# jvasilakes/disentanglement-vae

Measured on NVIDIA B200. Metric: train_tokens_per_sec, higher is better.
Workload: dtype f32

## Files before the change

disentanglement-vae_b200/_lib.py:

```python
import ctypes as C
import os

_HERE = os.path.dirname(os.path.abspath(__file__))
LIB_PATH = os.path.join(_HERE, "libdvae_b200.so")

MAX_SPACES = 8
HEADS_NSCALARS = 3 + 3 * MAX_SPACES


class DvaeError(RuntimeError):
    pass


_p = C.c_void_p
_i = C.c_int
_l = C.c_int64
_f = C.c_float
_u32 = C.c_uint32
_pp = C.POINTER(C.c_void_p)
_ip = C.POINTER(C.c_int)

SIGNATURES = {
    "dvae_last_error_string": (C.c_char_p, []),
    "dvae_version": (_i, []),
    "dvae_launch_count": (_l, []),
    "dvae_weight_planes_floats": (_l, [_i, _i, _i]),
    "dvae_weight_planes_register": (_i, [_p, _i, _i, _p, _p]),
    "dvae_weight_planes_refresh": (_i, [_p]),
    "dvae_weight_planes_refresh_ex": (_i, [_i, _i, _p]),
    "dvae_weight_planes_enable": (_i, [_i]),
    "dvae_weight_planes_clear": (_i, []),
    "dvae_defer_joins": (_i, [_i]),
    "dvae_join_side_streams": (_i, [_p]),
    "dvae_linear": (_i, [_p, _l, _i, _p, _l, _i, _p, _l, _i, _i, _i, _p, _p, _f, _i, _p]),
    "dvae_tc_linear": (_i, [_p, _l, _i, _p, _l, _i, _p, _l, _i, _i, _i, _p, _p, _f, _i, _i, _p]),
    "dvae_tc16_linear": (_i, [_p, _l, _i, _p, _l, _i, _p, _l, _i, _i, _i, _p, _p, _f, _i, _f, _f, _p, _p, _p]),
    "dvae_colsum": (_i, [_p, _l, _i, _i, _p, _f, _p]),
    "dvae_randn": (_i, [_p, _l, _p, _u32, _p]),
    "dvae_embedding_fwd": (_i, [_p, _i, _p, _l, _l, _i, _i, _f, _p, _u32, _l, _i, _p, _p]),
    "dvae_embedding_bwd": (_i, [_p, _i, _p, _l, _l, _i, _i, _f, _p, _u32, _l, _i, _p, _p]),
    "dvae_bow_encoder_fwd": (_i, [_p, _i, _p, _l, _l, _i, _i, _f, _p, _u32, _p, _l, _p, _p]),
    "dvae_bow_encoder_bwd": (_i, [_p, _l, _p, _i, _p, _l, _l, _i, _i, _f, _p, _u32, _p, _p]),
    "dvae_dropout": (_i, [_p, _l, _l, _i, _f, _p, _u32, _p, _l, _l, _p]),
    "dvae_lstm_step": (_i, [_p, _l, _i, _i, _i, _i, _i, _p, _p, _p, _p, _p, _p, _l, _p, _p, _p, _p, _p]),
    "dvae_vocab_sample_step": (_i, [_p, _l, _i, _i, _i, _p, _p, _p, _u32, _p, _l, _p, _p]),
    "dvae_vocab_sample_step_ex": (_i, [_p, _l, _i, _i, _i, _p, _p, _p, _u32, _p, _l, _p, _p, _p]),
    "dvae_vocab_w_planes_floats": (_l, [_i, _i]),
    "dvae_vocab_w_planes": (_i, [_p, _i, _i, _p, _p]),
    "dvae_vocab_sample_step_planes": (_i, [_p, _l, _i, _i, _i, _p, _p, _p, _p, _u32, _p, _l, _p, _p, _p]),
    "dvae_recount_lengths": (_i, [_p, _l, _l, _i, _i, _l, _l, _l, _p, _p]),
    "dvae_bleu_counts": (_i, [_p, _l, _i, _p, _l, _i, _i, _l, _p, _p]),
    "dvae_bleu_score": (_i, [_p, _p, _p]),
    "dvae_lstm_state_ws_floats": (_l, [_i, _i, _i]),
    "dvae_lstm_seq_fwd": (_i, [_p, _l, _i, _i, _i, _i, _i, _pp, _pp, _pp, _pp, _p, _p, _l, _l, _p, _p, _l, _p, _p,
                               _l, _l, _p, _p, _p, _p]),
    "dvae_lstm_input_proj": (_i, [_p, _l, _i, _i, _i, _i, _i, _pp, _pp, _pp, _p, _p]),
    "dvae_lstm_seq_fwd_ex": (_i, [_p, _l, _i, _i, _i, _i, _i, _pp, _pp, _pp, _pp, _p, _p, _l, _l, _p, _p, _l, _p, _p,
                                  _l, _l, _p, _p, _p, _i, _p]),
    "dvae_lstm_seq_bwd": (_i, [_p, _l, _i, _i, _i, _i, _i, _pp, _pp, _p, _p, _l, _l, _p, _p, _l, _p, _p, _p, _l,
                               _p, _p, _l, _l, _p, _l, _pp, _pp, _pp, _pp, _p, _p, _l, _l, _p, _p]),
    "dvae_lstm_bwd_planes_ws_floats": (_l, [_i, _i, _i, _i, _i]),
    "dvae_lstm_seq_bwd_ex": (_i, [_p, _l, _i, _i, _i, _i, _i, _pp, _pp, _p, _p, _l, _l, _p, _p, _l, _p, _p, _p, _l,
                                  _p, _p, _l, _l, _p, _l, _pp, _pp, _pp, _pp, _p, _p, _l, _l, _p, _p, _p]),
    "dvae_counter_increment": (_i, [_p, _p]),
    "dvae_fork_after": (_i, [_i, _p, _p, C.POINTER(C.c_void_p)]),
    "dvae_nvls_barrier_words": (_l, []),
    "dvae_nvls_all_reduce": (_i, [_p, _l, _pp, _i, _i, _p, C.c_uint32, C.c_uint32, _i, C.c_uint64, _p, _p]),
    "dvae_p2p_all_reduce": (_i, [_pp, _l, _pp, _i, _i, _p, C.c_uint32, C.c_uint32, _i, C.c_uint64, _p, _p]),
    "dvae_flag_signal": (_i, [_p, _p, _i, _p, _p]),
    "dvae_flag_wait": (_i, [_p, _p, _p]),
    "dvae_flag_signal_value": (_i, [_p, C.c_uint32, _p]),
    "dvae_flag_wait_value": (_i, [_p, C.c_uint32, _p]),
    "dvae_heads_ws_floats": (_l, [_i, _i]),
    "dvae_latent_heads_fwd": (_i, [_p, _i, _i, _i, _ip, _ip, _p, _p, _p, _p, _p, _p, _p, _p, _p, _i, _p, _p, _p,
                                   _p, _p, _p, _p, _p]),
    "dvae_heads_bwd_ws_floats": (_l, [_i, _i, _i]),
    "dvae_latent_heads_bwd": (_i, [_p, _i, _i, _i, _ip, _ip, _p, _p, _p, _p, _p, _p, _i, _p, _p, _p, _p, _p, _p,
                                   _p, _p, _p, _p, _p, _p, _p, _p, _p, _p, _p, _p, _p]),
    "dvae_dsc_loss": (_i, [_p, _p, _i, _i, _ip, _ip, _p, _p, _p, _p]),
    "dvae_vocab_ce_ws_floats": (_l, [_i, _i, _i]),
    "dvae_vocab_ce_fwd": (_i, [_p, _l, _i, _i, _i, _i, _p, _p, _p, _l, _p, _i, _p, _p, _p, _p, _p, _p]),
    "dvae_vocab_split_w": (_i, [_p, _i, _i, _i, _p, _p]),
    "dvae_vocab_ce_fwd_ex": (_i, [_p, _l, _i, _i, _i, _i, _p, _p, _p, _l, _p, _i, _p, _p, _p, _p, _p, _i, _p]),
    "dvae_vocab_ce_partials": (_i, [_p, _l, _i, _i, _i, _i, _p, _p, _p, _l, _p, _i, _p, _p]),
    "dvae_vocab_ce_bwd_ws_floats": (_l, [_i, _i, _i]),
    "dvae_vocab_ce_bwd": (_i, [_p, _l, _i, _i, _i, _i, _p, _p, _p, _l, _p, _p, _p, _p, _l, _p, _p, _p, _p, _p]),
    "dvae_entropy_loss": (_i, [_p, _i, _i, _p, _p, _p, _p]),
    "dvae_club_mi": (_i, [_p, _p, _p, _i, _i, _p, _p, _p, _p, _p, _p, _p]),
    "dvae_club_nll": (_i, [_p, _p, _p, _i, _i, _p, _p, _p, _p, _p]),
    "dvae_act_bwd": (_i, [_p, _p, _p, _l, _i, _p]),
    "dvae_relu": (_i, [_p, _l, _p]),
    "dvae_grad_sumsq": (_i, [_p, _l, _p, _p, _p]),
    "dvae_clip_adam": (_i, [_p, _p, _p, _p, _l, _p, _f, _f, _p, _i, _p]),
}

_lib = None
planes_owner = None


def load():
    global _lib
    if _lib is not None:
        return _lib
    if not os.path.exists(LIB_PATH):
        raise DvaeError(
            f"{LIB_PATH} not found: build it with `python -c 'import __graft_entry__ as g; g.build()'` "
            "(nvcc, sm_100a).  There is no CPU or PyTorch fallback for this path.")
    lib = C.CDLL(LIB_PATH)
    for name, (res, args) in SIGNATURES.items():
        try:
            fn = getattr(lib, name)
        except AttributeError as e:
            raise DvaeError(f"{LIB_PATH} does not export {name}") from e
        fn.restype = res
        fn.argtypes = args
    _lib = lib
    return lib


def check(rc, what):
    if rc != 0:
        msg = load().dvae_last_error_string()
        raise DvaeError(f"{what} failed ({rc}): {msg.decode() if msg else ''}")


def ptr(t):
    return None if t is None else t.data_ptr()


def ptr_array(tensors):
    arr = (C.c_void_p * max(len(tensors), 1))()
    for i, t in enumerate(tensors):
        arr[i] = None if t is None else t.data_ptr()
    return arr


def int_array(vals):
    arr = (C.c_int * max(len(vals), 1))()
    for i, v in enumerate(vals):
        arr[i] = int(v)
    return arr


def stream_ptr():
    import torch
    return torch.cuda.current_stream().cuda_stream


def launch_count():
    return int(load().dvae_launch_count())
```

disentanglement-vae_b200/csrc/common.cuh:

```cuda
#pragma once
#include <cuda_runtime.h>
#include <stdint.h>
#include <stdio.h>

#include "../../include/dvae_b200.h"

namespace dvae {

void set_error(const char* fmt, ...);
void count_launch(int n = 1);

#define DVAE_REQUIRE(cond, ...)            \
  do {                                     \
    if (!(cond)) {                         \
      ::dvae::set_error(__VA_ARGS__);      \
      return DVAE_EINVAL;                  \
    }                                      \
  } while (0)

#define DVAE_CUDA(call)                                                                  \
  do {                                                                                   \
    cudaError_t e__ = (call);                                                            \
    if (e__ != cudaSuccess) {                                                            \
      ::dvae::set_error("%s failed at %s:%d: %s", #call, __FILE__, __LINE__,             \
                        cudaGetErrorString(e__));                                        \
      return DVAE_ECUDA;                                                                 \
    }                                                                                    \
  } while (0)

#define DVAE_LAUNCH_CHECK()                                                              \
  do {                                                                                   \
    ::dvae::count_launch();                                                              \
    cudaError_t e__ = cudaGetLastError();                                                \
    if (e__ != cudaSuccess) {                                                            \
      ::dvae::set_error("kernel launch failed at %s:%d: %s", __FILE__, __LINE__,         \
                        cudaGetErrorString(e__));                                        \
      return DVAE_ECUDA;                                                                 \
    }                                                                                    \
  } while (0)

static inline int ceil_div(int64_t a, int64_t b) { return (int)((a + b - 1) / b); }

class Fork {
 public:
  explicit Fork(cudaStream_t main);
  cudaStream_t side(int i);
  int join();
  int join_or_defer();
  int mark(int i);
  int wait_mark();
  int chain(int from, int to);
 private:
  cudaStream_t main_;
  bool used_[3] = {false, false, false};
  bool marked_ = false;
  bool ok_;
};

bool defer_joins_enabled();

bool force_simt_gemm();

struct GemmHints {
  const uint32_t* a_amax_bits = nullptr;
  const uint32_t* b_amax_bits = nullptr;
  int a_amax_n = 1, b_amax_n = 1;
  float a_scale = 1.f, b_scale = 1.f;
  bool a_wide = false, b_wide = false;
  const void* b_planes = nullptr;
  int b_tile0 = 0, b_kb0 = 0, b_kbtot = 0;
  int max_ctas = 0;
  bool atomic_out = false;
  bool c_zeroed = false;
  int concurrency = 1;
};
int linear_impl_ex(const float* A, int64_t lda, int trans_a, const float* B, int64_t ldb, int trans_b, float* C,
                   int64_t ldc, int M, int N, int K, const float* bias, const float* bias2, float beta, int act,
                   const GemmHints& hints, cudaStream_t st);

namespace tc {
bool tc_linear_supported(const float* A, int64_t lda, const float* B, int64_t ldb, int M, int N, int K);
int tc_linear_impl(const float* A, int64_t lda, int trans_a, const float* B, int64_t ldb, int trans_b, float* C, int64_t ldc,
                   int M, int N, int K, const float* bias, const float* bias2, float beta, int act, int passes,
                   cudaStream_t st);
int tc_ce_partials(const float* h, int64_t ldh, int N, int B, int H, int V, const float* w, const float* bias,
                   const int64_t* targets, int64_t tgt_stride_b, const int64_t* lengths, int tiles_per_split, int nsplit,
                   float* part, int* part_idx, const uint64_t* gumbel_seed, uint32_t gumbel_salt, cudaStream_t st);
int tc_softmax_grad(const float* h, int64_t ldh, int N, int B, int H, int v0, int vc, const float* w, const float* bias,
                    const int64_t* targets, int64_t tgt_stride_b, const int64_t* lengths, const float* lse,
                    const float* grad_scale, float* P, int64_t ldp, cudaStream_t st);
}

struct Philox {
  static constexpr uint32_t kM0 = 0xD2511F53u, kM1 = 0xCD9E8D57u, kW0 = 0x9E3779B9u, kW1 = 0xBB67AE85u;
  __host__ __device__ static inline void round(uint32_t (&c)[4], uint32_t k0, uint32_t k1) {
#ifdef __CUDA_ARCH__
    uint32_t hi0 = __umulhi(kM0, c[0]), hi1 = __umulhi(kM1, c[2]);
#else
    uint32_t hi0 = (uint32_t)(((uint64_t)kM0 * c[0]) >> 32), hi1 = (uint32_t)(((uint64_t)kM1 * c[2]) >> 32);
#endif
    uint32_t lo0 = kM0 * c[0], lo1 = kM1 * c[2];
    uint32_t n0 = hi1 ^ c[1] ^ k0, n1 = lo1, n2 = hi0 ^ c[3] ^ k1, n3 = lo0;
    c[0] = n0; c[1] = n1; c[2] = n2; c[3] = n3;
  }
  __host__ __device__ static inline void gen(uint64_t seed, uint32_t salt, uint64_t ctr, uint32_t (&out)[4]) {
    uint32_t c[4] = {(uint32_t)ctr, (uint32_t)(ctr >> 32), salt, 0x5eedu};
    uint32_t k0 = (uint32_t)seed, k1 = (uint32_t)(seed >> 32);
#pragma unroll
    for (int i = 0; i < 10; ++i) {
      round(c, k0, k1);
      k0 += kW0;
      k1 += kW1;
    }
    out[0] = c[0]; out[1] = c[1]; out[2] = c[2]; out[3] = c[3];
  }
};

__device__ __forceinline__ void dropout_scale4(uint64_t seed, uint32_t salt, uint64_t idx4, float p,
                                               float inv_keep, float (&s)[4]) {
  uint32_t r[4];
  Philox::gen(seed, salt, idx4, r);
#pragma unroll
  for (int i = 0; i < 4; ++i) s[i] = ((float)r[i] * 2.3283064365386963e-10f >= p) ? inv_keep : 0.f;
}

__device__ __forceinline__ void gumbel4(uint64_t seed, uint32_t salt, int row, int col, int ncol4, float (&g)[4]) {
  uint32_t r[4];
  Philox::gen(seed, salt, (uint64_t)row * ncol4 + (col >> 2), r);
#pragma unroll
  for (int i = 0; i < 4; ++i) {
    const float u = ((float)(r[i] >> 8) + 0.5f) * (1.f / 16777216.f);
    g[i] = -logf(-logf(u));
  }
}

__device__ __forceinline__ float warp_sum(float v) {
#pragma unroll
  for (int o = 16; o > 0; o >>= 1) v += __shfl_xor_sync(0xffffffffu, v, o);
  return v;
}

__device__ __forceinline__ float sigmoidf_(float x) { return 1.f / (1.f + expf(-x)); }

}
```

disentanglement-vae_b200/csrc/embed_optim.cu:

```cuda
#include "common.cuh"

namespace dvae {

constexpr int kSMs = 148;

__global__ void embedding_fwd_kernel(const float* __restrict__ emb, int E, const int64_t* __restrict__ tokens,
                                     int64_t sb, int64_t st_, int T, int B, float p, const uint64_t* seed_dev,
                                     uint32_t salt, int64_t first_token, int t0, float* __restrict__ x) {
  const int64_t total4 = (int64_t)T * B * ((E + 3) / 4);
  const uint64_t seed = (p > 0.f && seed_dev) ? *seed_dev : 0;
  const float inv_keep = p > 0.f ? 1.f / (1.f - p) : 1.f;
  const int e4n = (E + 3) / 4;
  for (int64_t i = (int64_t)blockIdx.x * blockDim.x + threadIdx.x; i < total4; i += (int64_t)gridDim.x * blockDim.x) {
    const int64_t row = i / e4n + (int64_t)t0 * B;
    const int e0 = (int)(i % e4n) * 4;
    const int t = (int)(row / B), b = (int)(row % B);
    const int64_t tok = (t == 0 && first_token >= 0) ? first_token : tokens[b * sb + t * st_];
    const float* src = emb + tok * E + e0;
    float s[4] = {1.f, 1.f, 1.f, 1.f};
    if (p > 0.f && seed_dev) dropout_scale4(seed, salt, (uint64_t)(row * e4n + e0 / 4), p, inv_keep, s);
    float* dst = x + row * E + e0;
#pragma unroll
    for (int j = 0; j < 4; ++j)
      if (e0 + j < E) dst[j] = src[j] * s[j];
// ... 30 lines not shown
                                   float* __restrict__ ctx, int64_t ldctx, int32_t* __restrict__ argmax) {
  const int e4n = (E + 3) / 4;
  const int64_t total = (int64_t)B * e4n;
  const uint64_t seed = (p > 0.f && seed_dev) ? *seed_dev : 0;
  const float inv_keep = p > 0.f ? 1.f / (1.f - p) : 1.f;
  for (int64_t i = (int64_t)blockIdx.x * blockDim.x + threadIdx.x; i < total; i += (int64_t)gridDim.x * blockDim.x) {
    const int b = (int)(i / e4n), e0 = (int)(i % e4n) * 4;
    float best[4] = {-INFINITY, -INFINITY, -INFINITY, -INFINITY};
    int arg[4] = {0, 0, 0, 0};
    for (int t = 0; t < T; ++t) {
      const int64_t tok = tokens[b * sb + t * st_];
      float s[4] = {1.f, 1.f, 1.f, 1.f};
      if (p > 0.f && seed_dev) dropout_scale4(seed, salt, (uint64_t)(((int64_t)t * B + b) * e4n + e0 / 4), p, inv_keep, s);
#pragma unroll
      for (int j = 0; j < 4; ++j)
        if (e0 + j < E) {
          const float v = emb[tok * E + e0 + j] * s[j];
          if (v > best[j]) { best[j] = v; arg[j] = t; }
        }
    }
#pragma unroll
    for (int j = 0; j < 4; ++j)
      if (e0 + j < E) {
        ctx[(int64_t)b * ldctx + e0 + j] = best[j];
        argmax[(int64_t)b * E + e0 + j] = arg[j];
      }
  }
}

__global__ void bow_max_bwd_kernel(const float* __restrict__ d_ctx, int64_t ldd, const int32_t* __restrict__ argmax, int E,
                                   const int64_t* __restrict__ tokens, int64_t sb, int64_t st_, int T, int B, float p,
                                   const uint64_t* seed_dev, uint32_t salt, float* __restrict__ d_emb) {
  const int e4n = (E + 3) / 4;
  const int64_t total = (int64_t)B * E;
  const uint64_t seed = (p > 0.f && seed_dev) ? *seed_dev : 0;
  const float inv_keep = p > 0.f ? 1.f / (1.f - p) : 1.f;
  for (int64_t i = (int64_t)blockIdx.x * blockDim.x + threadIdx.x; i < total; i += (int64_t)gridDim.x * blockDim.x) {
    const int b = (int)(i / E), e = (int)(i % E);
    const int t = argmax[i];
    float s[4] = {1.f, 1.f, 1.f, 1.f};
    if (p > 0.f && seed_dev) dropout_scale4(seed, salt, (uint64_t)(((int64_t)t * B + b) * e4n + e / 4), p, inv_keep, s);
    const float v = d_ctx[(int64_t)b * ldd + e] * s[e & 3];
    if (v != 0.f) atomicAdd(d_emb + tokens[b * sb + t * st_] * E + e, v);
  }
}

__global__ void dropout_kernel(const float* __restrict__ x, int64_t ldx, int64_t rows, int width, float p,
                               const uint64_t* seed_dev, uint32_t salt, float* __restrict__ y, int64_t ldy, int64_t row0) {
  const int w4n = (width + 3) / 4;
  const int64_t total4 = rows * w4n;
  const uint64_t seed = (p > 0.f && seed_dev) ? *seed_dev : 0;
  const float inv_keep = p > 0.f ? 1.f / (1.f - p) : 1.f;
  for (int64_t i = (int64_t)blockIdx.x * blockDim.x + threadIdx.x; i < total4; i += (int64_t)gridDim.x * blockDim.x) {
    const int64_t row = i / w4n + row0;
    const int c0 = (int)(i % w4n) * 4;
    float s[4] = {1.f, 1.f, 1.f, 1.f};
    if (p > 0.f && seed_dev) dropout_scale4(seed, salt, (uint64_t)(row * w4n + c0 / 4), p, inv_keep, s);
#pragma unroll
    for (int j = 0; j < 4; ++j)
      if (c0 + j < width) y[row * ldy + c0 + j] = x[row * ldx + c0 + j] * s[j];
  }
}

__global__ void randn_kernel(float* __restrict__ out, int64_t n, const uint64_t* seed_dev, uint32_t salt) {
  const uint64_t seed = *seed_dev;
  const int64_t n4 = (n + 3) / 4;
  for (int64_t i = (int64_t)blockIdx.x * blockDim.x + threadIdx.x; i < n4; i += (int64_t)gridDim.x * blockDim.x) {
    uint32_t r[4];
    Philox::gen(seed, salt, (uint64_t)i, r);
    float u0 = ((float)r[0] + 1.f) * 2.3283064365386963e-10f, u1 = (float)r[1] * 2.3283064365386963e-10f;
    float u2 = ((float)r[2] + 1.f) * 2.3283064365386963e-10f, u3 = (float)r[3] * 2.3283064365386963e-10f;
    float a = sqrtf(-2.f * logf(u0)), b = sqrtf(-2.f * logf(u2));
    float s0, c0, s1, c1;
    sincospif(2.f * u1, &s0, &c0);
    sincospif(2.f * u3, &s1, &c1);
    float v[4] = {a * c0, a * s0, b * c1, b * s1};
#pragma unroll
    for (int j = 0; j < 4; ++j)
      if (i * 4 + j < n) out[i * 4 + j] = v[j];
  }
}

constexpr int kRedBlocks = 1024;

__global__ void __launch_bounds__(256) sumsq_kernel(const float* __restrict__ g, int64_t n, float* __restrict__ sumsq,
                                                    float* __restrict__ ws) {
  __shared__ float red[8];
  __shared__ int is_last;
  float acc = 0.f;
  const int64_t n4 = n / 4;
  const float4* g4 = reinterpret_cast<const float4*>(g);
  for (int64_t i = (int64_t)blockIdx.x * blockDim.x + threadIdx.x; i < n4; i += (int64_t)gridDim.x * blockDim.x) {
    float4 v = g4[i];
    acc = fmaf(v.x, v.x, acc); acc = fmaf(v.y, v.y, acc); acc = fmaf(v.z, v.z, acc); acc = fmaf(v.w, v.w, acc);
  }
  if (blockIdx.x == 0)
    for (int64_t i = n4 * 4 + threadIdx.x; i < n; i += blockDim.x) acc = fmaf(g[i], g[i], acc);
  acc = warp_sum(acc);
  if ((threadIdx.x & 31) == 0) red[threadIdx.x >> 5] = acc;
  __syncthreads();
  if (threadIdx.x == 0) {
    float t = 0.f;
    for (int i = 0; i < 8; ++i) t += red[i];
    ws[blockIdx.x] = t;
    __threadfence();
    unsigned int* counter = reinterpret_cast<unsigned int*>(ws + kRedBlocks);
    is_last = atomicAdd(counter, 1u) == gridDim.x - 1;
  }
  __syncthreads();
  if (is_last) {
    __threadfence();
    double t = 0.0;
    for (int i = threadIdx.x; i < (int)gridDim.x; i += blockDim.x) t += (double)((volatile float*)ws)[i];
    __shared__ double dred[256];
    dred[threadIdx.x] = t;
    __syncthreads();
    for (int o = 128; o > 0; o >>= 1) {
      if ((int)threadIdx.x < o) dred[threadIdx.x] += dred[threadIdx.x + o];
      __syncthreads();
    }
    if (threadIdx.x == 0) {
      sumsq[0] = (float)dred[0];
      *reinterpret_cast<unsigned int*>(ws + kRedBlocks) = 0u;
    }
  }
}

__global__ void __launch_bounds__(256) clip_adam_kernel(float* __restrict__ p, float* __restrict__ g,
                                                        float* __restrict__ m, float* __restrict__ v, int64_t n,
                                                        const float* __restrict__ sumsq, float max_norm,
                                                        float grad_scale, const float* __restrict__ hyper,
                                                        int zero_grad) {
  const float lr = hyper[0], b1 = hyper[1], b2 = hyper[2], eps = hyper[3], step = hyper[4];
  float coef = grad_scale;
  if (sumsq) {
    const float norm = sqrtf(sumsq[0]) * fabsf(grad_scale);
    coef *= fminf(1.f, max_norm / (norm + 1e-6f));
  }
  const float bc1 = 1.f - powf(b1, step), bc2 = 1.f - powf(b2, step);
  const float step_size = lr / bc1, inv_bc2_sqrt = 1.f / sqrtf(bc2);
  auto update = [&](float& pi, float& gi_io, float& mi_io, float& vi_io) {
    const float gi = gi_io * coef;
    const float mi = fmaf(b1, mi_io, (1.f - b1) * gi);
    const float vi = fmaf(b2, vi_io, (1.f - b2) * gi * gi);
    mi_io = mi; vi_io = vi;
    pi -= step_size * mi / (sqrtf(vi) * inv_bc2_sqrt + eps);
    gi_io = zero_grad ? 0.f : gi;
  };
  const bool vec = (((uintptr_t)p | (uintptr_t)g | (uintptr_t)m | (uintptr_t)v) & 15) == 0;
  const int64_t n4 = vec ? n / 4 : 0;
  float4* p4 = reinterpret_cast<float4*>(p); float4* g4 = reinterpret_cast<float4*>(g);
  float4* m4 = reinterpret_cast<float4*>(m); float4* v4 = reinterpret_cast<float4*>(v);
  const int64_t stride = (int64_t)gridDim.x * blockDim.x;
  for (int64_t i = (int64_t)blockIdx.x * blockDim.x + threadIdx.x; i < n4; i += 2 * stride) {
    const int64_t j = i + stride;
    const bool two = j < n4;
    float4 pa = p4[i], ga = g4[i], ma = m4[i], va = v4[i];
    float4 pb, gb, mb, vb;
    if (two) { pb = p4[j]; gb = g4[j]; mb = m4[j]; vb = v4[j]; }
    update(pa.x, ga.x, ma.x, va.x); update(pa.y, ga.y, ma.y, va.y); update(pa.z, ga.z, ma.z, va.z); update(pa.w, ga.w, ma.w, va.w);
    p4[i] = pa; g4[i] = ga; m4[i] = ma; v4[i] = va;
    if (two) {
      update(pb.x, gb.x, mb.x, vb.x); update(pb.y, gb.y, mb.y, vb.y); update(pb.z, gb.z, mb.z, vb.z); update(pb.w, gb.w, mb.w, vb.w);
      p4[j] = pb; g4[j] = gb; m4[j] = mb; v4[j] = vb;
    }
  }
  for (int64_t i = n4 * 4 + (int64_t)blockIdx.x * blockDim.x + threadIdx.x; i < n; i += stride) update(p[i], g[i], m[i], v[i]);
}

}

using namespace dvae;

static int ew_grid(int64_t work) {
  int64_t blocks = (work + 255) / 256;
  int64_t cap = (int64_t)kSMs * 8;
  return (int)(blocks < 1 ? 1 : (blocks > cap ? cap : blocks));
}

extern "C" int dvae_embedding_fwd(const float* emb, int E, const int64_t* tokens, int64_t sb, int64_t st_, int T,
                                  int B, float p, const uint64_t* seed_dev, uint32_t salt, int64_t first_token, int t0, float* x, void* stream) {
  DVAE_REQUIRE(emb && tokens && x && E > 0 && T > 0 && B > 0 && p >= 0.f && p < 1.f, "dvae_embedding_fwd: bad argument");
  embedding_fwd_kernel<<<ew_grid((int64_t)T * B * ((E + 3) / 4)), 256, 0, (cudaStream_t)stream>>>(emb, E, tokens, sb, st_, T, B, p, seed_dev, salt, first_token, t0, x);
  DVAE_LAUNCH_CHECK();
  return DVAE_OK;
}

extern "C" int dvae_embedding_bwd(const float* d_x, int E, const int64_t* tokens, int64_t sb, int64_t st_, int T,
                                  int B, float p, const uint64_t* seed_dev, uint32_t salt, int64_t first_token, int t0, float* d_emb, void* stream) {
  DVAE_REQUIRE(d_x && tokens && d_emb && E > 0 && T > 0 && B > 0 && p >= 0.f && p < 1.f, "dvae_embedding_bwd: bad argument");
  embedding_bwd_kernel<<<ew_grid((int64_t)T * B * ((E + 3) / 4)), 256, 0, (cudaStream_t)stream>>>(d_x, E, tokens, sb, st_, T, B, p, seed_dev, salt, first_token, t0, d_emb);
  DVAE_LAUNCH_CHECK();
  return DVAE_OK;
}

extern "C" int dvae_bow_encoder_fwd(const float* emb, int E, const int64_t* tokens, int64_t sb, int64_t st_, int T, int B, float p,
                                    const uint64_t* seed_dev, uint32_t salt, float* ctx, int64_t ldctx, int32_t* argmax, void* stream) {
  DVAE_REQUIRE(emb && tokens && ctx && argmax && E > 0 && T > 0 && B > 0 && p >= 0.f && p < 1.f, "dvae_bow_encoder_fwd: bad argument");
  bow_max_fwd_kernel<<<ew_grid((int64_t)B * ((E + 3) / 4)), 256, 0, (cudaStream_t)stream>>>(emb, E, tokens, sb, st_, T, B, p, seed_dev, salt, ctx, ldctx, argmax);
  DVAE_LAUNCH_CHECK();
  return DVAE_OK;
}

extern "C" int dvae_bow_encoder_bwd(const float* d_ctx, int64_t ldd, const int32_t* argmax, int E, const int64_t* tokens, int64_t sb,
                                    int64_t st_, int T, int B, float p, const uint64_t* seed_dev, uint32_t salt, float* d_emb, void* stream) {
  DVAE_REQUIRE(d_ctx && argmax && tokens && d_emb && E > 0 && T > 0 && B > 0 && p >= 0.f && p < 1.f, "dvae_bow_encoder_bwd: bad argument");
  bow_max_bwd_kernel<<<ew_grid((int64_t)B * E), 256, 0, (cudaStream_t)stream>>>(d_ctx, ldd, argmax, E, tokens, sb, st_, T, B, p, seed_dev, salt, d_emb);
  DVAE_LAUNCH_CHECK();
  return DVAE_OK;
}

extern "C" int dvae_dropout(const float* x, int64_t ldx, int64_t rows, int width, float p, const uint64_t* seed_dev,
                            uint32_t salt, float* y, int64_t ldy, int64_t row0, void* stream) {
  DVAE_REQUIRE(x && y && rows > 0 && width > 0 && p >= 0.f && p < 1.f, "dvae_dropout: bad argument");
  dropout_kernel<<<ew_grid(rows * ((width + 3) / 4)), 256, 0, (cudaStream_t)stream>>>(x, ldx, rows, width, p, seed_dev, salt, y, ldy, row0);
  DVAE_LAUNCH_CHECK();
  return DVAE_OK;
}

extern "C" int dvae_randn(float* out, int64_t n, const uint64_t* seed_dev, uint32_t salt, void* stream) {
  DVAE_REQUIRE(out && seed_dev && n > 0, "dvae_randn: bad argument");
  randn_kernel<<<ew_grid((n + 3) / 4), 256, 0, (cudaStream_t)stream>>>(out, n, seed_dev, salt);
  DVAE_LAUNCH_CHECK();
  return DVAE_OK;
}

extern "C" int dvae_grad_sumsq(const float* g, int64_t n, float* sumsq, float* ws, void* stream) {
  DVAE_REQUIRE(g && sumsq && ws && n > 0, "dvae_grad_sumsq: bad argument");
  DVAE_REQUIRE((reinterpret_cast<uintptr_t>(g) & 15) == 0, "dvae_grad_sumsq: gradient buffer must be 16-byte aligned");
  int blocks = ew_grid(n / 4 + 1);
  if (blocks > kRedBlocks) blocks = kRedBlocks;
  sumsq_kernel<<<blocks, 256, 0, (cudaStream_t)stream>>>(g, n, sumsq, ws);
  DVAE_LAUNCH_CHECK();
  return DVAE_OK;
}

extern "C" int dvae_clip_adam(float* p, float* g, float* m, float* v, int64_t n, const float* sumsq, float max_norm,
                              float grad_scale, const float* hyper_dev, int zero_grad, void* stream) {
  DVAE_REQUIRE(p && g && m && v && hyper_dev && n > 0, "dvae_clip_adam: bad argument");
  clip_adam_kernel<<<ew_grid((n + 7) / 8), 256, 0, (cudaStream_t)stream>>>(p, g, m, v, n, sumsq, max_norm, grad_scale, hyper_dev, zero_grad);
  DVAE_LAUNCH_CHECK();
  return DVAE_OK;
}

namespace dvae {
__global__ void recount_lengths_kernel(const int64_t* __restrict__ tokens, int64_t sb, int64_t st_, int B, int T, int64_t eos,
                                       int64_t pad, int64_t min_len, int64_t* __restrict__ lengths_out) {
  const int warp = (blockIdx.x * blockDim.x + threadIdx.x) >> 5, lane = threadIdx.x & 31;
  if (warp >= B) return;
  int n = 0;
  for (int t = lane; t < T; t += 32) {
    const int64_t tok = tokens[warp * sb + t * st_];
    n += (tok == eos || tok == pad) ? 1 : 0;
  }
#pragma unroll
  for (int o = 16; o > 0; o >>= 1) n += __shfl_xor_sync(0xffffffffu, n, o);
  if (lane == 0) {
    const int64_t len = (int64_t)T - n;
    lengths_out[warp] = len < min_len ? min_len : len;
  }
}
}

extern "C" int dvae_recount_lengths(const int64_t* tokens, int64_t tok_stride_b, int64_t tok_stride_t, int B, int T,
                                    int64_t eos, int64_t pad, int64_t min_len, int64_t* lengths_out, void* stream) {
  DVAE_REQUIRE(tokens && lengths_out && B > 0 && T > 0, "dvae_recount_lengths: bad argument");
  const int threads = 128, blocks = dvae::ceil_div((int64_t)B * 32, threads);
  dvae::recount_lengths_kernel<<<blocks, threads, 0, (cudaStream_t)stream>>>(tokens, tok_stride_b, tok_stride_t, B, T, eos, pad,
                                                                            min_len, lengths_out);
  DVAE_LAUNCH_CHECK();
  return DVAE_OK;
}
```

disentanglement-vae_b200/csrc/linear.cu:

```cuda
#include "gemm_simt.cuh"
#include "tc_gemm16.cuh"

namespace dvae {

template <class G>
__global__ void __launch_bounds__(G::NT) linear_kernel(const float* __restrict__ A, int64_t lda,
                                                        const float* __restrict__ B, int64_t ldb,
                                                        float* __restrict__ C, int64_t ldc, int M, int N, int K,
                                                        const float* __restrict__ bias,
                                                        const float* __restrict__ bias2, float beta, int act,
                                                        int k_per_split) {
  __shared__ __align__(16) float smem[G::SMEM_FLOATS];
  const int m0 = blockIdx.y * G::BM, n0 = blockIdx.x * G::BN;
  const int kb = blockIdx.z * k_per_split, ke = min(K, kb + k_per_split);
  float acc[G::TM][G::TN];
#pragma unroll
  for (int i = 0; i < G::TM; ++i)
#pragma unroll
    for (int j = 0; j < G::TN; ++j) acc[i][j] = 0.f;
  G::run(A, lda, m0, M, B, ldb, n0, N, kb, ke, K, smem, acc);
  const int ty = threadIdx.x / G::TX, tx = threadIdx.x % G::TX;
  const bool split = gridDim.z > 1;
#pragma unroll
  for (int i = 0; i < G::TM; ++i) {
    int m = m0 + G::row_of(ty, i);
    if (m >= M) continue;
#pragma unroll
    for (int j = 0; j < G::TN; ++j) {
      int n = n0 + G::col_of(tx, j);
      if (n >= N) continue;
      float v = acc[i][j];
      float* c = C + (int64_t)m * ldc + n;
      if (split) {
        if (blockIdx.z == 0) {
          if (bias) v += bias[n];
          if (bias2) v += bias2[n];
        }
        atomicAdd(c, v);
      } else {
        if (bias) v += bias[n];
        if (bias2) v += bias2[n];
        if (act == 1) v = tanhf(v);
        if (beta != 0.f) v += beta * (*c);
        *c = v;
      }
    }
  }
}

using GBig_NT = GemmTile<128, 128, 16, 8, 8, true, true>;
using GBig_NN = GemmTile<128, 128, 16, 8, 8, true, false>;
using GBig_TN = GemmTile<128, 128, 16, 8, 8, false, false>;
using GBig_TT = GemmTile<128, 128, 16, 8, 8, false, true>;
using GSm_NT = GemmTile<64, 64, 16, 4, 4, true, true>;
using GSm_NN = GemmTile<64, 64, 16, 4, 4, true, false>;
using GSm_TN = GemmTile<64, 64, 16, 4, 4, false, false>;
using GSm_TT = GemmTile<64, 64, 16, 4, 4, false, true>;

template <class G>
static int launch_linear(const float* A, int64_t lda, const float* B, int64_t ldb, float* C, int64_t ldc, int M,
                         int N, int K, const float* bias, const float* bias2, float beta, int act, int splits,
                         cudaStream_t st) {
  int k_per_split = ceil_div(ceil_div(K, splits), G::BK) * G::BK;
  splits = ceil_div(K, k_per_split);
  dim3 grid(ceil_div(N, G::BN), ceil_div(M, G::BM), splits);
  linear_kernel<G><<<grid, G::NT, 0, st>>>(A, lda, B, ldb, C, ldc, M, N, K, bias, bias2, beta, act, k_per_split);
  DVAE_LAUNCH_CHECK();
  return DVAE_OK;
}

__global__ void scale_rows_kernel(float* C, int64_t ldc, int M, int N, float beta) {
  int64_t i = (int64_t)blockIdx.x * blockDim.x + threadIdx.x;
  if (i >= (int64_t)M * N) return;
  float* c = C + (i / N) * ldc + (i % N);
  *c = beta == 0.f ? 0.f : *c * beta;
}

int linear_impl(const float* A, int64_t lda, int trans_a, const float* B, int64_t ldb, int trans_b, float* C,
                int64_t ldc, int M, int N, int K, const float* bias, const float* bias2, float beta, int act,
                cudaStream_t st) {
  return linear_impl_ex(A, lda, trans_a, B, ldb, trans_b, C, ldc, M, N, K, bias, bias2, beta, act, GemmHints(), st);
}

int linear_impl_ex(const float* A, int64_t lda, int trans_a, const float* B, int64_t ldb, int trans_b, float* C,
                   int64_t ldc, int M, int N, int K, const float* bias, const float* bias2, float beta, int act,
                   const GemmHints& hints, cudaStream_t st) {
  DVAE_REQUIRE(A && B && C, "dvae_linear: null pointer");
  DVAE_REQUIRE(M > 0 && N > 0 && K > 0, "dvae_linear: non-positive size M=%d N=%d K=%d", M, N, K);
  DVAE_REQUIRE(act == 0 || act == 1, "dvae_linear: unknown activation %d", act);
  static const double tc_min_mnk = [] {
    const char* e = getenv("DVAE_TC_MIN_LOG2_MNK");
    return (double)(1ll << (e ? atoi(e) : 24));
  }();
  if (!force_simt_gemm() && M >= 64 && N >= 64 && K >= 32 && (double)M * N * K >= tc_min_mnk) {
    const bool unscaled_wide = (hints.a_wide && !hints.a_amax_bits) || (hints.b_wide && !hints.b_amax_bits);
    if (!unscaled_wide && tc16::supported(A, lda, trans_a, B, ldb, trans_b, M, N, K))
      return tc16::linear(A, lda, trans_a, B, ldb, trans_b, C, ldc, M, N, K, bias, bias2, beta, act, hints, st);
    if (tc::tc_linear_supported(A, lda, B, ldb, M, N, K))
      return tc::tc_linear_impl(A, lda, trans_a, B, ldb, trans_b, C, ldc, M, N, K, bias, bias2, beta, act, 3, st);
  }
  const int kSMs = 148;
  int64_t big_tiles = (int64_t)ceil_div(M, 128) * ceil_div(N, 128);
  int64_t small_tiles = (int64_t)ceil_div(M, 64) * ceil_div(N, 64);
  bool big = big_tiles >= kSMs;
  int splits = 1;
  if (!big && small_tiles < kSMs / 2 && K >= 512 && act == 0) {
    { int64_t want = (kSMs + small_tiles - 1) / small_tiles, cap = K / 128; splits = (int)(want < cap ? want : cap); }
    if (splits < 1) splits = 1;
  }
  if (splits > 1) {
    if (beta != 1.f) {
      int64_t n = (int64_t)M * N;
      scale_rows_kernel<<<ceil_div(n, 256), 256, 0, st>>>(C, ldc, M, N, beta);
      DVAE_LAUNCH_CHECK();
    }
  }
#define DVAE_DISPATCH(GB, GS)                                                                                    \
  return big ? launch_linear<GB>(A, lda, B, ldb, C, ldc, M, N, K, bias, bias2, beta, act, 1, st)                 \
             : launch_linear<GS>(A, lda, B, ldb, C, ldc, M, N, K, bias, bias2, beta, act, splits, st)
  if (!trans_a && !trans_b) { DVAE_DISPATCH(GBig_NT, GSm_NT); }
  if (!trans_a && trans_b) { DVAE_DISPATCH(GBig_NN, GSm_NN); }
  if (trans_a && trans_b) { DVAE_DISPATCH(GBig_TN, GSm_TN); }
  DVAE_DISPATCH(GBig_TT, GSm_TT);
#undef DVAE_DISPATCH
}

__global__ void colsum_kernel(const float* __restrict__ X, int64_t ldx, int M, int N, float* __restrict__ out,
                              int rows_per_block) {
  __shared__ float red[8][33];
  const int n = blockIdx.x * 32 + threadIdx.x;
  const int m0 = blockIdx.y * rows_per_block, m1 = min(M, m0 + rows_per_block);
  float s0 = 0.f, s1 = 0.f;
  if (n < N) {
    int m = m0 + threadIdx.y;
    for (; m + 8 < m1; m += 16) { s0 += X[(int64_t)m * ldx + n]; s1 += X[(int64_t)(m + 8) * ldx + n]; }
    if (m < m1) s0 += X[(int64_t)m * ldx + n];
  }
  red[threadIdx.y][threadIdx.x] = s0 + s1;
  __syncthreads();
  if (threadIdx.y == 0 && n < N) {
    float t = 0.f;
#pragma unroll
    for (int i = 0; i < 8; ++i) t += red[i][threadIdx.x];
    atomicAdd(out + n, t);
  }
}

__global__ void scale_vec_kernel(float* out, int N, float beta) {
  int i = blockIdx.x * blockDim.x + threadIdx.x;
  if (i < N) out[i] *= beta;
}

int colsum_impl(const float* X, int64_t ldx, int M, int N, float* out, float beta, cudaStream_t st) {
  DVAE_REQUIRE(X && out && M > 0 && N > 0, "dvae_colsum: bad argument");
  if (beta == 0.f) {
    DVAE_CUDA(cudaMemsetAsync(out, 0, sizeof(float) * N, st));
  } else if (beta != 1.f) {
    scale_vec_kernel<<<ceil_div(N, 256), 256, 0, st>>>(out, N, beta);
    DVAE_LAUNCH_CHECK();
  }
  const int col_blocks = ceil_div(N, 32);
  int row_blocks = ceil_div(2 * 148, col_blocks);
  if (row_blocks > ceil_div(M, 64)) row_blocks = ceil_div(M, 64);
  if (row_blocks < 1) row_blocks = 1;
  const int rows_per_block = ceil_div(M, row_blocks);
  colsum_kernel<<<dim3(col_blocks, ceil_div(M, rows_per_block)), dim3(32, 8), 0, st>>>(X, ldx, M, N, out, rows_per_block);
  DVAE_LAUNCH_CHECK();
  return DVAE_OK;
}

}

extern "C" int dvae_linear(const float* A, int64_t lda, int trans_a, const float* B, int64_t ldb, int trans_b,
                           float* C, int64_t ldc, int M, int N, int K, const float* bias, const float* bias2,
                           float beta, int act, void* stream) {
  dvae::GemmHints hints;
  hints.a_wide = hints.b_wide = true;
  return dvae::linear_impl_ex(A, lda, trans_a, B, ldb, trans_b, C, ldc, M, N, K, bias, bias2, beta, act, hints,
                           (cudaStream_t)stream);
// ... 6 lines not shown
```

disentanglement-vae_b200/csrc/lstm.cu:

```cuda
#include <stdlib.h>

#include <cstring>

#include "common.cuh"
#include "lstm_persist.cuh"
#include "tc_gemm16.cuh"

namespace dvae {

int linear_impl(const float* A, int64_t lda, int trans_a, const float* B, int64_t ldb, int trans_b, float* C,
                int64_t ldc, int M, int N, int K, const float* bias, const float* bias2, float beta, int act,
                cudaStream_t st);
int colsum_impl(const float* X, int64_t ldx, int M, int N, float* out, float beta, cudaStream_t st);

__global__ void copy_state_kernel(const float* __restrict__ src, int64_t lds, int64_t dirs, float* __restrict__ dst,
                                  int64_t ldd, int64_t dird, int D, int B, int H) {
  int64_t i = (int64_t)blockIdx.x * blockDim.x + threadIdx.x;
  if (i >= (int64_t)D * B * H) return;
  int u = i % H, b = (i / H) % B, d = i / ((int64_t)H * B);
  dst[d * dird + b * ldd + u] = src ? src[d * dirs + b * lds + u] : 0.f;
}

__global__ void transpose_kernel(const float* __restrict__ in, float* __restrict__ out, int R, int C) {
  __shared__ float tile[32][33];
// ... 211 lines not shown
int lstm_input_proj_impl(const float* x, int64_t ldx, int T, int B, int I, int H, int D, const float* const* w_ih,
                         const float* const* b_ih, const float* const* b_hh, float* gates, cudaStream_t st) {
  DVAE_REQUIRE(x && gates && w_ih, "dvae_lstm_input_proj: null pointer");
  DVAE_REQUIRE(T > 0 && B > 0 && I > 0 && H > 0 && (D == 1 || D == 2), "dvae_lstm_input_proj: bad shape T=%d B=%d I=%d H=%d D=%d", T, B, I, H, D);
  const int64_t slab = (int64_t)T * B * 4 * H;
  Fork fork(st);
  GemmHints gh;
  gh.concurrency = D;
  for (int d = 0; d < D; ++d) {
    int rc = linear_impl_ex(x, ldx, 0, w_ih[d], I, 0, gates + d * slab, 4 * H, T * B, 4 * H, I, b_ih ? b_ih[d] : nullptr,
                            b_hh ? b_hh[d] : nullptr, 0.f, 0, gh, d == 0 ? st : fork.side(0));
    if (rc) return rc;
  }
  return fork.join();
}

int lstm_seq_fwd_impl(const float* x, int64_t ldx, int T, int B, int I, int H, int D, const float* const* w_ih,
                      const float* const* w_hh, const float* const* b_ih, const float* const* b_hh,
                      const float* h0, const float* c0, int64_t ld0, int64_t dir0, const int64_t* lengths,
                      float* hs, int64_t ldhs, float* hn, float* cn, int64_t ldn, int64_t dirn, float* gates,
                      float* cs, float* ws, bool gates_ready, cudaStream_t st) {
  DVAE_REQUIRE(x && hs && gates && cs && ws && w_ih && w_hh, "dvae_lstm_seq_fwd: null pointer");
  DVAE_REQUIRE(T > 0 && B > 0 && I > 0 && H > 0 && (D == 1 || D == 2), "dvae_lstm_seq_fwd: bad shape T=%d B=%d I=%d H=%d D=%d", T, B, I, H, D);
  DVAE_REQUIRE(!(lengths && h0), "dvae_lstm_seq_fwd: length-masked layers start from the zero state");
  const int64_t sf = (int64_t)D * B * H;
  if (!gates_ready) {
    int rc = lstm_input_proj_impl(x, ldx, T, B, I, H, D, w_ih, b_ih, b_hh, gates, st);
    if (rc) return rc;
  }
  {
    const void* ptrs[] = {x, w_hh[0], w_hh[D - 1], h0, c0, hs, hn, cn, gates, cs, ws};
    const int64_t lds[] = {ld0, dir0, ldhs, ldn, dirn};
    if (!force_step_path() && persist_supported(B, H, D, ptrs, 11, lds, 5)) {
      PersistFwdArgs a;
      a.w_hh[0] = w_hh[0]; a.w_hh[1] = w_hh[D - 1];
      a.gates = gates; a.cs = cs; a.hs = hs; a.ldhs = ldhs; a.h0 = h0; a.c0 = c0; a.ld0 = ld0; a.dir0 = dir0;
      a.hstate = ws; a.hn = hn; a.cn = cn; a.ldn = ldn; a.dirn = dirn; a.lengths = lengths;
      a.T = T; a.B = B; a.D = D; a.n_slices = ceil_div(B, 16); a.d_off = 0;
      a.dbg = nullptr;
      if (const char* e = getenv("DVAE_LSTM_DBG")) a.dbg = reinterpret_cast<unsigned long long*>(strtoull(e, nullptr, 0));
      return persist_fwd(H, a, st);
    }
    if (!force_step_path() && planes_lstm_supported(B, H, D, ptrs, 11, lds, 5) && resident_lstm_supported(B, H))
      return resident_lstm_fwd(T, B, H, D, w_hh, h0, c0, ld0, dir0, lengths, hs, ldhs, hn, cn, ldn, dirn, gates, cs,
                               ws + planes_ws_offset(B, H, D), st);
    if (!force_step_path() && planes_lstm_supported(B, H, D, ptrs, 11, lds, 5))
      return planes_lstm_fwd(T, B, H, D, w_hh, h0, c0, ld0, dir0, lengths, hs, ldhs, hn, cn, ldn, dirn, gates, cs, ws,
                             ws + planes_ws_offset(B, H, D), st);
  }
  float* hbuf[2] = {ws, ws + 2 * sf};
  float* cbuf[2] = {ws + sf, ws + 3 * sf};
  const int nthr = 256, nblk = ceil_div(sf, nthr);
  copy_state_kernel<<<nblk, nthr, 0, st>>>(h0, ld0, dir0, hbuf[0], H, (int64_t)B * H, D, B, H);
  DVAE_LAUNCH_CHECK();
  copy_state_kernel<<<nblk, nthr, 0, st>>>(c0, ld0, dir0, cbuf[0], H, (int64_t)B * H, D, B, H);
  DVAE_LAUNCH_CHECK();
  FwdStepArgs a;
  for (int d = 0; d < 2; ++d) a.w_hh[d] = w_hh[d < D ? d : 0];
  a.gates = gates; a.cs = cs; a.hs = hs; a.ldhs = ldhs; a.lengths = lengths; a.T = T; a.B = B; a.H = H;
  dim3 grid(ceil_div(H, 16), ceil_div(B, kStepRows), D);
  for (int s = 0; s < T; ++s) {
    a.s = s;
    a.h_in = hbuf[s & 1]; a.c_in = cbuf[s & 1]; a.h_out = hbuf[(s + 1) & 1]; a.c_out = cbuf[(s + 1) & 1];
    lstm_step_fwd_kernel<<<grid, kStepThreads, 0, st>>>(a);
    DVAE_LAUNCH_CHECK();
  }
  if (hn) {
    copy_state_kernel<<<nblk, nthr, 0, st>>>(hbuf[T & 1], H, (int64_t)B * H, hn, ldn, dirn, D, B, H);
    DVAE_LAUNCH_CHECK();
  }
  if (cn) {
    copy_state_kernel<<<nblk, nthr, 0, st>>>(cbuf[T & 1], H, (int64_t)B * H, cn, ldn, dirn, D, B, H);
    DVAE_LAUNCH_CHECK();
  }
  return DVAE_OK;
}

int lstm_seq_bwd_impl(const float* x, int64_t ldx, int T, int B, int I, int H, int D, const float* const* w_ih,
                      const float* const* w_hh, const float* h0, const float* c0, int64_t ld0, int64_t dir0,
                      const int64_t* lengths, const float* hs, int64_t ldhs, float* gates, const float* cs,
                      const float* d_hs, int64_t lddhs, const float* d_hn, const float* d_cn, int64_t ldn,
                      int64_t dirn, float* d_x, int64_t lddx, float* const* d_w_ih, float* const* d_w_hh,
                      float* const* d_b_ih, float* const* d_b_hh, float* d_h0, float* d_c0, int64_t ldd0,
                      int64_t dird0, float* ws, float* planes_ws, cudaStream_t st) {
  DVAE_REQUIRE(x && hs && gates && cs && ws && w_ih && w_hh, "dvae_lstm_seq_bwd: null pointer");
  DVAE_REQUIRE(T > 0 && B > 0 && I > 0 && H > 0 && (D == 1 || D == 2), "dvae_lstm_seq_bwd: bad shape");
  DVAE_REQUIRE(!(lengths && h0), "dvae_lstm_seq_bwd: length-masked layers start from the zero state");
  const int64_t slab = (int64_t)T * B * 4 * H, sf = (int64_t)D * B * H;
  bool persisted = false;
  uint32_t* amax = nullptr;
  int amax_n = 1;
  bool dx_zeroed = false;
  {
    const void* ptrs[] = {w_hh[0], w_hh[D - 1], c0, gates, cs, d_hs, d_hn, d_cn, d_h0, d_c0};
    const int64_t lds[] = {ld0, dir0, lddhs, ldn, dirn, ldd0, dird0};
    if (!force_step_path() && persist_supported(B, H, D, ptrs, 10, lds, 7)) {
      PersistBwdArgs a;
      a.w_hh[0] = w_hh[0]; a.w_hh[1] = w_hh[D - 1];
      a.gates = gates; a.cs = cs; a.c0 = c0; a.ld0 = ld0; a.dir0 = dir0; a.d_hs = d_hs; a.lddhs = lddhs;
      a.d_hn = d_hn; a.d_cn = d_cn; a.ldn = ldn; a.dirn = dirn; a.d_h0 = d_h0; a.d_c0 = d_c0; a.ldd0 = ldd0;
      a.dird0 = dird0; a.lengths = lengths; a.T = T; a.B = B; a.D = D; a.n_slices = ceil_div(B, 16); a.d_off = 0;
      a.amax_out = nullptr;
      a.zero_buf = nullptr; a.zero_n4 = 0;
      if (tc_lstm_supported(H)) {
        static thread_local unsigned slot = 0;
        amax = reinterpret_cast<uint32_t*>(ws + state_floats(B, H, D) + 4LL * D * H * H) + amax_slot_entries(B, D) * (slot++ & 7);
        a.amax_out = amax;
        amax_n = tc_lstm_bwd_ctas(B, D);
        if (d_x && lddx == I && (((uintptr_t)d_x) & 15) == 0 && ((int64_t)T * B * I) % 4 == 0 && d_x != d_hs) {
          a.zero_buf = d_x; a.zero_n4 = (int64_t)T * B * I / 4;
          dx_zeroed = true;
        }
      }
      int rc = persist_bwd(H, a, st);
      if (rc) return rc;
      persisted = true;
    } else {
      const void* ptrs2[] = {w_hh[0], w_hh[D - 1], c0, gates, cs, d_hs, d_hn, d_cn, d_h0, d_c0, ws};
      if (!force_step_path() && planes_lstm_supported(B, H, D, ptrs2, 11, lds, 7)) {
        static thread_local unsigned slot2 = 0;
        amax = reinterpret_cast<uint32_t*>(ws + state_floats(B, H, D) + 4LL * D * H * H) + amax_slot_entries(B, D) * (slot2++ & 7);
        amax_n = D;
        int rc = planes_lstm_bwd(T, B, H, D, w_hh, c0, ld0, dir0, lengths, gates, cs, d_hs, lddhs, d_hn, d_cn, ldn, dirn, d_h0,
                                 d_c0, ldd0, dird0, ws, ws + 4 * sf, ws + planes_ws_offset(B, H, D), amax, st);
        if (rc) return rc;
        persisted = true;
      }
    }
  }
  float* carry[2] = {ws, ws + 2 * sf};
  float* dcb[2] = {ws + sf, ws + 3 * sf};
  float* wt = ws + 4 * sf;
  for (int d = 0; d < D && !persisted; ++d) {
    transpose_kernel<<<dim3(ceil_div(H, 32), ceil_div(4 * H, 32)), dim3(32, 8), 0, st>>>(w_hh[d], wt + (int64_t)d * 4 * H * H, 4 * H, H);
    DVAE_LAUNCH_CHECK();
  }
  const int nthr = 256, nblk = ceil_div(sf, nthr);
  if (!persisted) {
    copy_state_kernel<<<nblk, nthr, 0, st>>>(d_hn, ldn, dirn, carry[0], H, (int64_t)B * H, D, B, H);
    DVAE_LAUNCH_CHECK();
    copy_state_kernel<<<nblk, nthr, 0, st>>>(d_cn, ldn, dirn, dcb[0], H, (int64_t)B * H, D, B, H);
    DVAE_LAUNCH_CHECK();
  }
  BwdStepArgs a;
  for (int d = 0; d < 2; ++d) a.w_hh_t[d] = wt + (int64_t)(d < D ? d : 0) * 4 * H * H;
  a.gates = gates; a.cs = cs; a.c0 = c0; a.ld0 = ld0; a.dir0 = dir0; a.d_hs = d_hs; a.lddhs = lddhs;
  a.d_h0 = d_h0; a.d_c0 = d_c0; a.ldd0 = ldd0; a.dird0 = dird0; a.lengths = lengths; a.T = T; a.B = B; a.H = H;
  dim3 grid(ceil_div(H, 32), ceil_div(B, kStepRows), D);
  const int nsteps = persisted ? 0 : T + ((d_h0 || d_c0) ? 1 : 0);
  for (int s = 0; s < nsteps; ++s) {
    a.s = s; a.final_ = (s == T);
    a.carry_in = carry[s & 1]; a.dc_in = dcb[s & 1]; a.carry_out = carry[(s + 1) & 1]; a.dc_out = dcb[(s + 1) & 1];
    if (a.final_) {
    }
    lstm_step_bwd_kernel<<<grid, kStepThreads, 0, st>>>(a);
    DVAE_LAUNCH_CHECK();
  }
  GemmHints gh;
  gh.a_wide = true;
  gh.a_amax_bits = amax;
  gh.a_amax_n = amax_n;
  GemmHints gh_bg = gh;
  {
    static const int cap = [] { const char* e = getenv("DVAE_DW_MAX_CTAS"); return e ? atoi(e) : 48; }();
    gh_bg.max_ctas = (defer_joins_enabled() && tc_lstm_supported(H)) ? cap : 0;
  }
  Fork fork(st);
  const bool dx_pair = d_x && D == 2 && dx_zeroed && !force_simt_gemm() && tc_lstm_supported(H) &&
                       !(getenv("DVAE_DX_PAIR") && getenv("DVAE_DX_PAIR")[0] == '0');
  if (dx_pair) {
    GemmHints ghx = gh;
    ghx.c_zeroed = true; ghx.atomic_out = true; ghx.concurrency = 2;
    int rc = linear_impl_ex(gates + slab, 4 * H, 0, w_ih[1], I, 1, d_x, lddx, T * B, I, 4 * H, nullptr, nullptr, 1.f, 0, ghx, fork.side(2));
    if (rc) return rc;
    if ((rc = fork.mark(2))) return rc;
  }
  const int TB = T * B, KBt = ceil_div(TB, 32);
  const char* dwp_env = getenv("DVAE_DW_PLANES");
  const bool dwp_on = dwp_env ? dwp_env[0] != '0' : (int64_t)4 * H * (I > H ? I : H) * TB >= ((int64_t)1 << 32);
  const bool dw_planes = planes_ws && amax && !force_simt_gemm() && tc16::enabled() && TB >= 128 &&
                         (reinterpret_cast<uintptr_t>(planes_ws) & 15) == 0 && dwp_on;
  const bool hh_planes = dw_planes && T > 1 && B % 32 == 0;
  float *xT = planes_ws, *dGt[2] = {nullptr, nullptr}, *hsT[2] = {nullptr, nullptr};
  if (dw_planes) {
    float* q = xT + tc16::plane_floats(I, TB);
    for (int d = 0; d < D; ++d) { dGt[d] = q; q += tc16::plane_floats(4 * H, TB); }
    for (int d = 0; d < D; ++d) { hsT[d] = q; q += tc16::plane_floats(H, TB); }
    tc16::PlaneTable tab;
    tab.n = 0;
    if (d_w_ih) tab.e[tab.n++] = tc16::PlaneTable::Entry{x, TB, I, nullptr, xT, ldx, nullptr, 0};
    for (int d = 0; d < D; ++d) {
      tab.e[tab.n++] = tc16::PlaneTable::Entry{gates + d * slab, TB, 4 * H, nullptr, dGt[d], 4 * H, amax, amax_n};
      if (hh_planes && d_w_hh) tab.e[tab.n++] = tc16::PlaneTable::Entry{hs + d * H, TB, H, nullptr, hsT[d], ldhs, nullptr, 0};
    }
    int rc = tc16::weight_planes_launch(tab, fork.side(0));
    if (rc) return rc;
    if ((rc = fork.chain(0, 1))) return rc;
  }
  for (int d = 0; d < D; ++d) {
    const float* dG = gates + d * slab;
    int rc;
    if (d_x && !(dx_pair && d == 1)) {
      GemmHints ghx = gh;
      ghx.c_zeroed = dx_zeroed;
      if (dx_pair) { ghx.atomic_out = true; ghx.concurrency = 2; }
      rc = linear_impl_ex(dG, 4 * H, 0, w_ih[d], I, 1, d_x, lddx, T * B, I, 4 * H, nullptr, nullptr, (d == 0 && !dx_pair) ? 0.f : 1.f, 0, ghx, st);
      if (rc) return rc;
      if (dx_pair && (rc = fork.wait_mark())) return rc;
    }
    if (d_w_ih && d_w_ih[d]) {
      if (dw_planes)
        rc = tc16::linear_planes(dGt[d], xT, d_w_ih[d], I, 4 * H, I, TB, nullptr, 0.f, 0, 1.f, 1.f, nullptr, false, 16, fork.side(0), 0, 0,
                                 gh_bg.max_ctas, 0, 0, amax, amax_n);
      else
        rc = linear_impl_ex(dG, 4 * H, 1, x, ldx, 1, d_w_ih[d], I, 4 * H, I, T * B, nullptr, nullptr, 0.f, 0, gh_bg, fork.side(0));
      if (rc) return rc;
    }
    if (d_w_hh && d_w_hh[d]) {
      cudaStream_t s1 = fork.side(1);
      bool wrote = false;
      if (T > 1) {
        const float* dGs = d == 0 ? dG + (int64_t)B * 4 * H : dG;
        const float* hp = d == 0 ? hs + d * H : hs + (int64_t)B * ldhs + d * H;
        if (hh_planes)
          rc = tc16::linear_planes(dGt[d], hsT[d], d_w_hh[d], H, 4 * H, H, (T - 1) * B, nullptr, 0.f, 0, 1.f, 1.f, nullptr, false, 16, s1,
                                   d == 0 ? 0 : B / 32, KBt, gh_bg.max_ctas, d == 0 ? B / 32 : 0, KBt, amax, amax_n);
        else
          rc = linear_impl_ex(dGs, 4 * H, 1, hp, ldhs, 1, d_w_hh[d], H, 4 * H, H, (T - 1) * B, nullptr, nullptr, 0.f, 0, gh_bg, s1);
        if (rc) return rc;
        wrote = true;
      }
      if (h0) {
        const float* dG0 = d == 0 ? dG : dG + (int64_t)(T - 1) * B * 4 * H;
        rc = linear_impl_ex(dG0, 4 * H, 1, h0 + d * dir0, ld0, 1, d_w_hh[d], H, 4 * H, H, B, nullptr, nullptr, wrote ? 1.f : 0.f, 0, gh_bg, s1);
        if (rc) return rc;
        wrote = true;
      }
      if (!wrote) DVAE_CUDA(cudaMemsetAsync(d_w_hh[d], 0, sizeof(float) * 4 * H * H, s1));
    }
    cudaStream_t s2 = fork.side(2);
    if (d_b_ih && d_b_ih[d]) {
      rc = colsum_impl(dG, 4 * H, T * B, 4 * H, d_b_ih[d], 0.f, s2);
      if (rc) return rc;
      if (d_b_hh && d_b_hh[d]) DVAE_CUDA(cudaMemcpyAsync(d_b_hh[d], d_b_ih[d], sizeof(float) * 4 * H, cudaMemcpyDeviceToDevice, s2));
    } else if (d_b_hh && d_b_hh[d]) {
      rc = colsum_impl(dG, 4 * H, T * B, 4 * H, d_b_hh[d], 0.f, s2);
      if (rc) return rc;
    }
  }
  {
    int rc = fork.join_or_defer();
    if (rc) return rc;
  }
  return DVAE_OK;
}

__global__ void lstm_cell_step_kernel(float* __restrict__ gates_t, const float* __restrict__ c_prev, int64_t ldc, float* __restrict__ cs_t,
                                      float* __restrict__ hs_t, int B, int H) {
  const int HQ = H / 4, idx = blockIdx.x * blockDim.x + threadIdx.x;
  if (idx >= B * HQ) return;
  const int b = idx / HQ, u0 = (idx % HQ) * 4;
  float* g = gates_t + (int64_t)b * 4 * H + u0;
  float4 gi = *reinterpret_cast<float4*>(g), gf = *reinterpret_cast<float4*>(g + H), gg = *reinterpret_cast<float4*>(g + 2 * H),
         go = *reinterpret_cast<float4*>(g + 3 * H);
  float4 c = c_prev ? *reinterpret_cast<const float4*>(c_prev + (int64_t)b * ldc + u0) : make_float4(0.f, 0.f, 0.f, 0.f), h;
#define DVAE_CELL(x)                                                                  \
  gi.x = sigmoidf_(gi.x); gf.x = sigmoidf_(gf.x); gg.x = tanhf(gg.x); go.x = sigmoidf_(go.x); \
  c.x = fmaf(gf.x, c.x, gi.x * gg.x); h.x = go.x * tanhf(c.x);
  DVAE_CELL(x) DVAE_CELL(y) DVAE_CELL(z) DVAE_CELL(w)
#undef DVAE_CELL
  *reinterpret_cast<float4*>(g) = gi; *reinterpret_cast<float4*>(g + H) = gf; *reinterpret_cast<float4*>(g + 2 * H) = gg;
  *reinterpret_cast<float4*>(g + 3 * H) = go;
  *reinterpret_cast<float4*>(cs_t + (int64_t)b * H + u0) = c;
  *reinterpret_cast<float4*>(hs_t + (int64_t)b * H + u0) = h;
}

int lstm_step_impl(const float* x, int64_t ldx, int t, int T, int B, int I, int H, const float* w_ih, const float* w_hh,
                   const float* b_ih, const float* b_hh, const float* h0, const float* c0, int64_t ld0, float* hs,
                   float* gates, float* cs, float* ws, cudaStream_t st) {
  DVAE_REQUIRE(x && w_ih && w_hh && hs && gates && cs && ws, "dvae_lstm_step: null pointer");
  DVAE_REQUIRE(t >= 0 && t < T && B > 0 && I > 0 && H > 0, "dvae_lstm_step: bad shape");
  int rc = linear_impl(x + (int64_t)t * B * ldx, ldx, 0, w_ih, I, 0, gates + (int64_t)t * B * 4 * H, 4 * H, B, 4 * H, I, b_ih, b_hh,
                       0.f, 0, st);
  if (rc) return rc;
  const int64_t sf = (int64_t)B * H;
  {
    const void* ptrs[] = {x, w_hh, h0, c0, hs, gates, cs};
    bool aligned = H % 4 == 0 && ld0 % 4 == 0;
    for (const void* q : ptrs) aligned = aligned && ((reinterpret_cast<uintptr_t>(q) & 15) == 0);
    const char* e = getenv("DVAE_LSTM_IMPL");
    if (aligned && B >= 256 && H >= 64 && !force_simt_gemm() && !(e && !strcmp(e, "step"))) {
      float* gates_t = gates + (int64_t)t * B * 4 * H;
      const float* h_prev = t == 0 ? h0 : hs + (int64_t)(t - 1) * sf;
      const float* c_prev = t == 0 ? c0 : cs + (int64_t)(t - 1) * sf;
      if (h_prev && (rc = linear_impl(h_prev, t == 0 ? ld0 : H, 0, w_hh, H, 0, gates_t, 4 * H, B, 4 * H, H, nullptr, nullptr, 1.f, 0, st)))
        return rc;
      lstm_cell_step_kernel<<<ceil_div((int64_t)B * (H / 4), 256), 256, 0, st>>>(gates_t, c_prev, t == 0 ? ld0 : H, cs + (int64_t)t * sf,
                                                                               hs + (int64_t)t * sf, B, H);
      DVAE_LAUNCH_CHECK();
      return DVAE_OK;
    }
  }
  const float *h_in, *c_in;
  if (t == 0) {
    const int nthr = 256, nblk = ceil_div(sf, nthr);
    copy_state_kernel<<<nblk, nthr, 0, st>>>(h0, ld0, 0, ws, H, sf, 1, B, H);
    DVAE_LAUNCH_CHECK();
    copy_state_kernel<<<nblk, nthr, 0, st>>>(c0, ld0, 0, ws + sf, H, sf, 1, B, H);
    DVAE_LAUNCH_CHECK();
    h_in = ws; c_in = ws + sf;
  } else {
    h_in = hs + (int64_t)(t - 1) * sf; c_in = cs + (int64_t)(t - 1) * sf;
  }
  FwdStepArgs a;
  a.w_hh[0] = w_hh; a.w_hh[1] = w_hh;
  a.gates = gates; a.cs = cs; a.hs = hs; a.ldhs = H; a.lengths = nullptr; a.T = T; a.B = B; a.H = H; a.s = t;
  a.h_in = h_in; a.c_in = c_in; a.h_out = ws + 2 * sf; a.c_out = ws + 3 * sf;
  lstm_step_fwd_kernel<<<dim3(ceil_div(H, 16), ceil_div(B, kStepRows), 1), kStepThreads, 0, st>>>(a);
  DVAE_LAUNCH_CHECK();
  return DVAE_OK;
}

}

extern "C" int dvae_lstm_step(const float* x, int64_t ldx, int t, int T, int B, int I, int H, const float* w_ih,
                              const float* w_hh, const float* b_ih, const float* b_hh, const float* h0, const float* c0,
                              int64_t ld0, float* hs, float* gates, float* cs, float* state_ws, void* stream) {
  return dvae::lstm_step_impl(x, ldx, t, T, B, I, H, w_ih, w_hh, b_ih, b_hh, h0, c0, ld0, hs, gates, cs, state_ws,
                              (cudaStream_t)stream);
}

extern "C" int64_t dvae_lstm_state_ws_floats(int B, int H, int D) {
  return dvae::planes_ws_offset(B, H, D) + dvae::planes_lstm_ws_floats(B, H, D);
}

extern "C" int dvae_lstm_seq_fwd(const float* x, int64_t ldx, int T, int B, int I, int H, int D,
                                 const float* const* w_ih, const float* const* w_hh, const float* const* b_ih,
                                 const float* const* b_hh, const float* h0, const float* c0, int64_t ld0,
                                 int64_t dir0, const int64_t* lengths, float* hs, int64_t ldhs, float* hn,
                                 float* cn, int64_t ldn, int64_t dirn, float* gates, float* cs, float* state_ws,
                                 void* stream) {
  return dvae::lstm_seq_fwd_impl(x, ldx, T, B, I, H, D, w_ih, w_hh, b_ih, b_hh, h0, c0, ld0, dir0, lengths, hs,
                                 ldhs, hn, cn, ldn, dirn, gates, cs, state_ws, false, (cudaStream_t)stream);
}

extern "C" int dvae_lstm_input_proj(const float* x, int64_t ldx, int T, int B, int I, int H, int D,
                                    const float* const* w_ih, const float* const* b_ih, const float* const* b_hh,
                                    float* gates, void* stream) {
  return dvae::lstm_input_proj_impl(x, ldx, T, B, I, H, D, w_ih, b_ih, b_hh, gates, (cudaStream_t)stream);
}

extern "C" int dvae_lstm_seq_fwd_ex(const float* x, int64_t ldx, int T, int B, int I, int H, int D,
                                    const float* const* w_ih, const float* const* w_hh, const float* const* b_ih,
                                    const float* const* b_hh, const float* h0, const float* c0, int64_t ld0,
                                    int64_t dir0, const int64_t* lengths, float* hs, int64_t ldhs, float* hn,
                                    float* cn, int64_t ldn, int64_t dirn, float* gates, float* cs, float* state_ws,
                                    int flags, void* stream) {
  return dvae::lstm_seq_fwd_impl(x, ldx, T, B, I, H, D, w_ih, w_hh, b_ih, b_hh, h0, c0, ld0, dir0, lengths, hs,
                                 ldhs, hn, cn, ldn, dirn, gates, cs, state_ws, (flags & 1) != 0, (cudaStream_t)stream);
}

extern "C" int dvae_lstm_seq_bwd(const float* x, int64_t ldx, int T, int B, int I, int H, int D,
                                 const float* const* w_ih, const float* const* w_hh, const float* h0,
                                 const float* c0, int64_t ld0, int64_t dir0, const int64_t* lengths,
                                 const float* hs, int64_t ldhs, float* gates, const float* cs, const float* d_hs,
                                 int64_t lddhs, const float* d_hn, const float* d_cn, int64_t ldn, int64_t dirn,
                                 float* d_x, int64_t lddx, float* const* d_w_ih, float* const* d_w_hh,
                                 float* const* d_b_ih, float* const* d_b_hh, float* d_h0, float* d_c0,
                                 int64_t ldd0, int64_t dird0, float* state_ws, void* stream) {
  return dvae::lstm_seq_bwd_impl(x, ldx, T, B, I, H, D, w_ih, w_hh, h0, c0, ld0, dir0, lengths, hs, ldhs, gates, cs,
                                 d_hs, lddhs, d_hn, d_cn, ldn, dirn, d_x, lddx, d_w_ih, d_w_hh, d_b_ih, d_b_hh,
                                 d_h0, d_c0, ldd0, dird0, state_ws, nullptr, (cudaStream_t)stream);
}

extern "C" int64_t dvae_lstm_bwd_planes_ws_floats(int T, int B, int I, int H, int D) {
  const int TB = T * B;
  return dvae::tc16::plane_floats(I, TB) + (int64_t)D * (dvae::tc16::plane_floats(4 * H, TB) + dvae::tc16::plane_floats(H, TB));
}

extern "C" int dvae_lstm_seq_bwd_ex(const float* x, int64_t ldx, int T, int B, int I, int H, int D,
                                    const float* const* w_ih, const float* const* w_hh, const float* h0,
                                    const float* c0, int64_t ld0, int64_t dir0, const int64_t* lengths,
                                    const float* hs, int64_t ldhs, float* gates, const float* cs, const float* d_hs,
                                    int64_t lddhs, const float* d_hn, const float* d_cn, int64_t ldn, int64_t dirn,
                                    float* d_x, int64_t lddx, float* const* d_w_ih, float* const* d_w_hh,
                                    float* const* d_b_ih, float* const* d_b_hh, float* d_h0, float* d_c0,
                                    int64_t ldd0, int64_t dird0, float* state_ws, float* planes_ws, void* stream) {
  return dvae::lstm_seq_bwd_impl(x, ldx, T, B, I, H, D, w_ih, w_hh, h0, c0, ld0, dir0, lengths, hs, ldhs, gates, cs,
                                 d_hs, lddhs, d_hn, d_cn, ldn, dirn, d_x, lddx, d_w_ih, d_w_hh, d_b_ih, d_b_hh,
                                 d_h0, d_c0, ldd0, dird0, state_ws, planes_ws, (cudaStream_t)stream);
}
```

disentanglement-vae_b200/csrc/tc_gemm16.cu:

```cuda
#include <cuda_fp16.h>
#include <stdlib.h>
#include <string.h>

#include "tc_gemm.cuh"
#include "tc_gemm16.cuh"
#include "tc_planes.cuh"

namespace dvae {
namespace tc16 {

using namespace tc;

constexpr int BM = 128, BN = 128, BK = 32;
constexpr int STAGES = 6, MAX_STAGES = 14;
constexpr int RAW_TILE = BM * BK * 4;
constexpr int STAGE_BYTES = 2 * RAW_TILE;
constexpr int PS_PLANE = BM * BK * 2, PS_TILE = 2 * PS_PLANE;
constexpr int PS_LBO = 128, PS_SBO = 512;
static_assert(PS_TILE == RAW_TILE, "in-place conversion: fp16 hi + lo planes occupy exactly the landed fp32 tile");
constexpr int EPI_WARPS = 8, MMA_WARP = 4, TMA_WARP = 5, PROD_WARP0 = 6, PROD_WARPS = 16, EPI2_WARP0 = PROD_WARP0 + PROD_WARPS;
constexpr int NUM_THREADS = (EPI2_WARP0 + 4) * 32;
constexpr int CONV_BARRIER = 1;
constexpr int EPI_SCRATCH_BYTES = 8 * 32 * 32 * 4;
#ifndef DVAE_AS_KB
// ... 81 lines not shown
__device__ __forceinline__ uint32_t cluster_rank() {
  uint32_t r;
  asm volatile("mov.u32 %0, %%cluster_ctarank;" : "=r"(r));
  return r;
}
__device__ __forceinline__ void cluster_sync_all() {
  asm volatile("barrier.cluster.arrive.release.aligned;\n\tbarrier.cluster.wait.acquire.aligned;" ::: "memory");
}
__device__ __forceinline__ void bulk_load_multicast(uint32_t smem_dst, const void* src, uint32_t bytes, uint64_t* bar, uint16_t mask) {
  asm volatile("cp.async.bulk.shared::cluster.global.mbarrier::complete_tx::bytes.multicast::cluster [%0], [%1], %2, [%3], %4;" ::"r"(smem_dst),
               "l"(src), "r"(bytes), "r"(smem_u32(bar)), "h"(mask)
               : "memory");
}
__device__ __forceinline__ void tc_commit_multicast(uint64_t* bar, uint16_t mask) {
  asm volatile("tcgen05.commit.cta_group::1.mbarrier::arrive::one.shared::cluster.multicast::cluster.b64 [%0], %1;" ::"r"(smem_u32(bar)),
               "h"(mask)
               : "memory");
}

__device__ __forceinline__ void bulk_load(uint32_t smem_dst, const void* src, uint32_t bytes, uint64_t* bar) {
  asm volatile("cp.async.bulk.shared::cluster.global.mbarrier::complete_tx::bytes [%0], [%1], %2, [%3];" ::"r"(smem_dst), "l"(src),
               "r"(bytes), "r"(smem_u32(bar))
               : "memory");
}

__global__ void split_planes_kernel(const float* __restrict__ X, int64_t ld, int R, int K, float scale, float lo_scale,
                                    uint8_t* __restrict__ planes) {
  const int KB = (K + BK - 1) / BK, KC = KB * (BK / 8), RP = (R + BM - 1) / BM * BM;
  const int64_t total = (int64_t)RP * KC;
  for (int64_t i = (int64_t)blockIdx.x * blockDim.x + threadIdx.x; i < total; i += (int64_t)gridDim.x * blockDim.x) {
    const int kc = (int)(i % KC), r = (int)(i / KC);
    float v[8];
#pragma unroll
    for (int e = 0; e < 8; ++e) v[e] = (r < R && kc * 8 + e < K) ? __ldg(X + (int64_t)r * ld + kc * 8 + e) : 0.f;
    uint4 h, l;
    h.x = pack_hi_lo(v[0], v[1], scale, l.x, lo_scale); h.y = pack_hi_lo(v[2], v[3], scale, l.y, lo_scale);
    h.z = pack_hi_lo(v[4], v[5], scale, l.z, lo_scale); h.w = pack_hi_lo(v[6], v[7], scale, l.w, lo_scale);
    const int64_t off = ((int64_t)(r >> 7) * KB + (kc >> 2)) * (2 * PS_PLANE) + ((r & 127) >> 3) * PS_SBO + (kc & 3) * PS_LBO + (r & 7) * 16;
    *reinterpret_cast<uint4*>(planes + off) = h;
    *reinterpret_cast<uint4*>(planes + off + PS_PLANE) = l;
  }
}

__global__ void weight_planes_kernel(PlaneTable tab) {
  const PlaneTable::Entry e = tab.e[blockIdx.y >> 1];
  const int tr = blockIdx.y & 1;
  uint8_t* out = reinterpret_cast<uint8_t*>(tr ? e.planes_t : e.planes);
  if (!out) return;
  const int R = tr ? e.C : e.R, K = tr ? e.R : e.C;
  const int64_t ld = e.ld ? e.ld : e.C;
  const float sc = scale_from_amax(e.amax, e.amax_n, 1.f);
  const int KB = (K + BK - 1) / BK, KC = KB * (BK / 8), RP = (R + BM - 1) / BM * BM;
  const int64_t total = (int64_t)RP * KC;
  for (int64_t i = (int64_t)blockIdx.x * blockDim.x + threadIdx.x; i < total; i += (int64_t)gridDim.x * blockDim.x) {
    int kc, r;
    if (!tr) { kc = (int)(i % KC); r = (int)(i / KC); }
    else { r = (int)(i % RP); kc = (int)(i / RP); }
    float v[8];
#pragma unroll
    for (int j = 0; j < 8; ++j) {
      const int k = kc * 8 + j;
      v[j] = (r < R && k < K) ? __ldg(tr ? e.w + (int64_t)k * ld + r : e.w + (int64_t)r * ld + k) : 0.f;
    }
    uint4 h, l;
    h.x = pack_hi_lo(v[0], v[1], sc, l.x); h.y = pack_hi_lo(v[2], v[3], sc, l.y);
    h.z = pack_hi_lo(v[4], v[5], sc, l.z); h.w = pack_hi_lo(v[6], v[7], sc, l.w);
    const int64_t off = ((int64_t)(r >> 7) * KB + (kc >> 2)) * (2 * PS_PLANE) + ((r & 127) >> 3) * PS_SBO + (kc & 3) * PS_LBO + (r & 7) * 16;
    *reinterpret_cast<uint4*>(out + off) = h;
    *reinterpret_cast<uint4*>(out + off + PS_PLANE) = l;
  }
}

int weight_planes_launch(const PlaneTable& tab, cudaStream_t st) {
  if (tab.n <= 0) return DVAE_OK;
  int64_t most = 1;
  for (int i = 0; i < tab.n; ++i) most = max(most, (int64_t)tab.e[i].R * tab.e[i].C / 8);
  int bx = ceil_div(most, 256 * 4);
  bx = bx < 8 ? 8 : (bx > 4 * 148 ? 4 * 148 : bx);
  weight_planes_kernel<<<dim3(bx, 2 * tab.n), 256, 0, st>>>(tab);
  DVAE_LAUNCH_CHECK();
  return DVAE_OK;
}

__global__ void __launch_bounds__(NUM_THREADS, 1)
tc16_gemm_kernel(const __grid_constant__ CUtensorMap tmA, const __grid_constant__ CUtensorMap tmB, Params p) {
  extern __shared__ __align__(1024) uint8_t smem[];
  if (p.skip_flag && *p.skip_flag) return;
  uint64_t* bars = reinterpret_cast<uint64_t*>(smem + OFF_BAR);
  uint64_t* full = bars;
  uint64_t* empty = bars + MAX_STAGES;
  uint64_t* raw_full = bars + 2 * MAX_STAGES;
  uint64_t* tmem_full = raw_full + MAX_STAGES;
  uint64_t* tmem_empty = tmem_full + 2;
  uint64_t* a_full = tmem_empty + 2;
  uint32_t* tmem_slot = reinterpret_cast<uint32_t*>(a_full + 1);

  const int tid = threadIdx.x, warp = tid >> 5, lane = tid & 31;
  const bool wide_epi = p.presplit && p.mode != 0;
  const uint32_t csize = p.mcast ? cluster_size() : 1, crank = p.mcast ? cluster_rank() : 0;
  const uint16_t cmask = (uint16_t)((1u << csize) - 1);
  const bool conv_as_epi = wide_epi && warp >= PROD_WARP0 && warp < PROD_WARP0 + EPI_WARPS;
  asm volatile("griddepcontrol.launch_dependents;" ::: "memory");
  if (tid == 0) DBG16(0);
  if (p.zero_buf) {
    float4* z4 = reinterpret_cast<float4*>(p.zero_buf);
    const int64_t nblk = (int64_t)gridDim.x * gridDim.y * gridDim.z;
    const int64_t blk = ((int64_t)blockIdx.z * gridDim.y + blockIdx.y) * gridDim.x + blockIdx.x;
    for (int64_t i = blk * NUM_THREADS + tid; i < p.zero_n4; i += nblk * NUM_THREADS) z4[i] = make_float4(0.f, 0.f, 0.f, 0.f);
    if (p.zero_buf2) {
      float4* y4 = reinterpret_cast<float4*>(p.zero_buf2);
      for (int64_t i = blk * NUM_THREADS + tid; i < p.zero2_n4; i += nblk * NUM_THREADS) y4[i] = make_float4(0.f, 0.f, 0.f, 0.f);
    }
  }
  const int m0 = blockIdx.x * BM;
  const int nt0 = blockIdx.y * p.tiles_per_cta;
  const int n_tiles = (p.N + BN - 1) / BN;
  const int nt1 = min(n_tiles, nt0 + p.tiles_per_cta);
  const int nkb_total = (p.K + BK - 1) / BK;
  const int kb0 = blockIdx.z * p.kb_per_split;
  const int nkb = max(0, min(nkb_total, kb0 + p.kb_per_split) - kb0);
  const int b_tile0 = p.b_row0 / BN;

  if (tid == 0) {
    if (smem_u32(smem) & 1023) {
      printf("dvae tc16_gemm: dynamic shared memory base is not 1024-byte aligned\n");
      __trap();
    }
    for (int s = 0; s < MAX_STAGES; ++s) {
      mbar_init(&full[s], p.presplit ? 1 : PROD_WARPS / 2 + (p.b_presplit ? 1 : 0));
      mbar_init(&empty[s], p.mcast ? csize : 1);
      mbar_init(&raw_full[s], 1);
    }
    for (int a = 0; a < 2; ++a) {
      mbar_init(&tmem_full[a], 1);
      mbar_init(&tmem_empty[a], wide_epi ? 2 * EPI_WARPS : EPI_WARPS);
    }
    mbar_init(a_full, 2 * EPI_WARPS);
    fence_barrier_init();
  }
  if (warp == TMA_WARP && lane == 0 && !p.presplit) {
    tma_prefetch_desc(&tmA);
    tma_prefetch_desc(&tmB);
  }
  const bool a_stat = p.presplit && !p.no_astat && nkb_total <= AS_MAX_KB && gridDim.z == 1;
  const int nstages = a_stat ? (p.mode == 1 ? AS_STAGES_NOSCRATCH : AS_STAGES) : STAGES;
  const uint32_t stage_bytes = a_stat ? AS_STAGE_BYTES : STAGE_BYTES;
  const int a_blk = min((int)blockIdx.x, (p.M + BM - 1) / BM - 1);
  if (warp == MMA_WARP) tmem_alloc(tmem_slot, TMEM_COLS);
  tc_fence_before();
  __syncthreads();
  if (p.mcast) cluster_sync_all();
  tc_fence_after();
  const uint32_t tmem_base = *tmem_slot;
  const uint32_t smem_u = smem_u32(smem);

  if (warp == TMA_WARP) {
    if (DVAE_TC16_FLAG(16)) {
    } else if (lane == 0 && a_stat) {
      const uint8_t* b_planes = reinterpret_cast<const uint8_t*>(p.b_planes);
      int stage = 0, phase = 0;
      for (int nt = nt0; nt < nt1; ++nt) {
        for (int kb = 0; kb < nkb; kb += AS_KB_PER_STAGE) {
          DVAE_TC16_MARK(nt == nt0 + 1 && kb < 8, 32 + 2 * kb);
          if (!DVAE_TC16_FLAG(8)) mbar_wait(&empty[stage], phase ^ 1);
          else mbar_wait(&full[stage], phase ^ 1);
          DVAE_TC16_MARK(nt == nt0 + 1 && kb < 8, 33 + 2 * kb);
// ... 281 lines not shown
              float tv[16], ssum = 0.f;
#pragma unroll
              for (int k = 0; k < 16; ++k) {
                const int r = rg * 16 + k;
                tv[k] = lds32(sc + (r * 16 + (cc ^ ((r >> 1) & 15))) * 4);
                ssum += tv[k];
              }
              ssum += __shfl_xor_sync(0xffffffffu, ssum, 16);
              if (colw < p.N) {
                if (rg == 0 && p.p_colsum) atomicAdd(p.p_colsum + colw, ssum);
                const float lo8[8] = {tv[0], tv[1], tv[2], tv[3], tv[4], tv[5], tv[6], tv[7]};
                const float hi8[8] = {tv[8], tv[9], tv[10], tv[11], tv[12], tv[13], tv[14], tv[15]};
                if (r0 + rg * 16 < p.p_kb_t * BK) store_plane_chunk(p.p_planes_t, colw, r0 + rg * 16, p.p_kb_t, lo8, p.p_scale);
                if (r0 + rg * 16 + 8 < p.p_kb_t * BK) store_plane_chunk(p.p_planes_t, colw, r0 + rg * 16 + 8, p.p_kb_t, hi8, p.p_scale);
              }
              __syncwarp();
              continue;
            }
            const int colw = col0 + hh * 16 + (lane & 15);
            float* cp = p.C + (int64_t)(r0 + (lane >> 4)) * p.ldc + colw;
            if (colw < p.N) {
#pragma unroll
              for (int k = 0; k < 16; ++k) {
                const float val = lds32(sc + ((2 * k + (lane >> 4)) * 16 + ((lane & 15) ^ k)) * 4);
                if (2 * k + (lane >> 4) < nr) cp[(int64_t)(2 * k) * p.ldc] = val;
              }
            }
            __syncwarp();
          }
          DVAE_TC16_MARK(tid == 0 && tile == 2, 105);
          continue;
        }
        if (p.mode != 1) {
          const uint32_t sc = smem_u + OFF_SCRATCH + ew * (32 * 32 * 4);
          DVAE_TC16_MARK(tid == 0 && tile == 2, 104 + 3 * (c - c_lo));
#pragma unroll
          for (int hh = 0; hh < 2; ++hh) {
            float v[16], w[16];
            tmem_ld16_pair(ta + hh * 16, ta + 128 + hh * 16, v, w);
            float x[16];
#pragma unroll
            for (int j = 0; j < 16; ++j) x[j] = fmaf(w[j], kLoInv, v[j]) * oscale;
            if (p.mode == 2) {
              float bv[16];
#pragma unroll
              for (int q = 0; q < 4; ++q) {
                const uint4 t = lds128(sbias_u + ((c - c_lo) * 32 + hh * 16 + 4 * q) * 4);
                bv[4 * q] = __uint_as_float(t.x); bv[4 * q + 1] = __uint_as_float(t.y);
                bv[4 * q + 2] = __uint_as_float(t.z); bv[4 * q + 3] = __uint_as_float(t.w);
              }
              const bool dead = row_scale == 0.f;
#pragma unroll
              for (int j = 0; j < 16; ++j) {
                const int col = col0 + hh * 16 + j;
                const float e = ex2_ftz(fmaf(x[j] + bv[j], kLog2e, row_nlse2));
                x[j] = (dead || col >= p.N) ? 0.f : (e - (col == tgt ? 1.f : 0.f)) * row_scale;
              }
            }
#pragma unroll
            for (int j = 0; j < 16; ++j) sts32(sc + (lane * 32 + ((hh * 16 + j) ^ lane)) * 4, x[j]);
          }
          DVAE_TC16_MARK(tid == 0 && tile == 2, 105 + 3 * (c - c_lo));
          __syncwarp();
          const int col = col0 + lane;
          const int r0 = m0 + quarter * 32;
          const int nr = min(32, p.M - r0);
          if (col < p.N && nr > 0) {
            const bool split = gridDim.z > 1 || p.atomic_out;
            float badd = 0.f;
            if (p.mode == 0 && (!split || blockIdx.z == 0)) {
              if (p.bias) badd += __ldg(p.bias + col);
              if (p.bias2) badd += __ldg(p.bias2 + col);
            }
            float* cp = p.C + (int64_t)r0 * p.ldc + col;
            const int64_t ldc = p.ldc;
            auto chunk_at = [&](int rr) { return lds32(sc + (uint32_t)(rr * 32 + (lane ^ rr)) * 4); };
            if (p.mode == 2 || (!split && p.act == 0 && p.beta == 0.f)) {
              if (nr == 32) {
#pragma unroll
                for (int rr = 0; rr < 32; ++rr) cp[rr * ldc] = chunk_at(rr) + badd;
              } else {
                for (int rr = 0; rr < nr; ++rr) cp[rr * ldc] = chunk_at(rr) + badd;
              }
            } else if (split) {
              for (int rr = 0; rr < nr; ++rr) atomicAdd(cp + rr * ldc, chunk_at(rr) + badd);
            } else {
              const float beta = p.beta;
              const bool do_tanh = p.act == 1;
              if (nr == 32 && beta != 0.f) {
#pragma unroll 1
                for (int r8 = 0; r8 < 32; r8 += 8) {
                  float old[8];
#pragma unroll
                  for (int rr = 0; rr < 8; ++rr) old[rr] = cp[(r8 + rr) * ldc];
#pragma unroll
                  for (int rr = 0; rr < 8; ++rr) {
                    float x = chunk_at(r8 + rr) + badd;
                    if (do_tanh) x = tanhf(x);
                    cp[(r8 + rr) * ldc] = fmaf(beta, old[rr], x);
                  }
                }
              } else {
                for (int rr = 0; rr < nr; ++rr) {
                  float x = chunk_at(rr) + badd;
                  if (do_tanh) x = tanhf(x);
                  if (beta != 0.f) x = fmaf(beta, cp[rr * ldc], x);
                  cp[rr * ldc] = x;
                }
              }
            }
          }
          DVAE_TC16_MARK(tid == 0 && tile == 2, 106 + 3 * (c - c_lo));
          __syncwarp();
          continue;
        }
        const bool sample = p.gumbel_seed != nullptr;
        const uint64_t gseed = sample ? *p.gumbel_seed : 0;
#pragma unroll
        for (int hh = 0; hh < 2; ++hh) {
          float v[16], w[16];
          DVAE_TC16_MARK(tid == 0 && tile == 2, 98 + 3 * hh);
          if (a_stat) {
            tmem_ld16(ta + hh * 16, v);
#pragma unroll
            for (int j = 0; j < 16; ++j) w[j] = 0.f;
          } else {
            tmem_ld16_pair(ta + hh * 16, ta + 128 + hh * 16, v, w);
          }
          DVAE_TC16_MARK(tid == 0 && tile == 2, 99 + 3 * hh);
          if (!row_ok) continue;
          const int base = col0 + hh * 16;
          float x[16], xs[16];
          {
            const uint32_t ba = sbias_u + ((c - c_lo) * 32 + hh * 16) * 4;
            float bv[16];
#pragma unroll
            for (int q = 0; q < 4; ++q) {
              const uint4 t = lds128(ba + q * 16);
              bv[4 * q] = __uint_as_float(t.x); bv[4 * q + 1] = __uint_as_float(t.y);
              bv[4 * q + 2] = __uint_as_float(t.z); bv[4 * q + 3] = __uint_as_float(t.w);
            }
#pragma unroll
            for (int j = 0; j < 16; ++j) x[j] = fmaf(fmaf(w[j], kLoInv, v[j]), oscale, bv[j]);
            if (base + 16 > p.N) {
#pragma unroll
              for (int j = 0; j < 16; ++j)
                if (base + j >= p.N) x[j] = -INFINITY;
            }
          }
          if (sample) {
#pragma unroll
            for (int j4 = 0; j4 < 16; j4 += 4) {
              float g[4];
              gumbel4(gseed, p.gumbel_salt, row, base + j4, (p.N + 3) >> 2, g);
#pragma unroll
              for (int jj = 0; jj < 4; ++jj) xs[j4 + jj] = x[j4 + jj] + g[jj];
            }
          } else {
#pragma unroll
            for (int j = 0; j < 16; ++j) xs[j] = x[j];
          }
          float m8[8], m4[4];
#pragma unroll
          for (int j = 0; j < 8; ++j) m8[j] = fmaxf(xs[2 * j], xs[2 * j + 1]);
#pragma unroll
          for (int j = 0; j < 4; ++j) m4[j] = fmaxf(m8[2 * j], m8[2 * j + 1]);
// ... 82 lines not shown
  CUresult r = fn(m, CU_TENSOR_MAP_DATA_TYPE_FLOAT32, 2, const_cast<float*>(base), dims, strides, box, estr,
                  CU_TENSOR_MAP_INTERLEAVE_NONE, mn_major ? CU_TENSOR_MAP_SWIZZLE_NONE : CU_TENSOR_MAP_SWIZZLE_128B,
                  CU_TENSOR_MAP_L2_PROMOTION_L2_128B, CU_TENSOR_MAP_FLOAT_OOB_FILL_NONE);
  DVAE_REQUIRE(r == CUDA_SUCCESS, "tc16_gemm: cuTensorMapEncodeTiled failed (%d) rows=%d K=%d ld=%lld", (int)r, rows, K, (long long)ld);
  return DVAE_OK;
}

int64_t plane_floats(int R, int K) { return (int64_t)ceil_div(R, BM) * BM * ceil_div(K, BK) * BK; }

bool presplit_enabled() {
  const char* e = getenv("DVAE_VOCAB_PRESPLIT");
  return !(e && e[0] == '0');
}

bool single_acc_planes(int K) { return ceil_div(K, BK) <= AS_MAX_KB; }

int split_planes(const float* X, int64_t ld, int R, int K, float scale, void* planes, cudaStream_t st, bool force_dual) {
  const bool single = !force_dual && single_acc_planes(K);
  const float lo_scale = single ? 1.f : kLoScale;
  if (single) scale *= kSingleScale;
  DVAE_REQUIRE(X && planes && R > 0 && K > 0, "tc16 split_planes: bad argument");
  const int64_t work = (int64_t)ceil_div(R, BM) * BM * ceil_div(K, BK) * (BK / 8);
  int blocks = ceil_div(work, 256);
  if (blocks > 148 * 8) blocks = 148 * 8;
  split_planes_kernel<<<blocks, 256, 0, st>>>(X, ld, R, K, scale, lo_scale, reinterpret_cast<uint8_t*>(planes));
  DVAE_LAUNCH_CHECK();
  return DVAE_OK;
}

static int launch(const Params& p_in, dim3 grid, cudaStream_t st) {
  Params p = p_in;
  if (p.dbg)
    if (const char* e = getenv("DVAE_TC_DBG_MODE"))
      if (atoi(e) != p.mode) p.dbg = nullptr;
  static bool ready = false;
  if (!ready) {
    DVAE_CUDA(cudaFuncSetAttribute(tc16_gemm_kernel, cudaFuncAttributeMaxDynamicSharedMemorySize, SMEM_BYTES));
    ready = true;
  }
  CUtensorMap ma, mb;
  int rc;
  if (p.presplit) {
    memset(&ma, 0, sizeof(ma));
    memset(&mb, 0, sizeof(mb));
  } else {
    if ((rc = make_map(&ma, p.A, p.lda, p.a_mn, p.M, p.K))) return rc;
    if (p.b_presplit) memset(&mb, 0, sizeof(mb));
    else if ((rc = make_map(&mb, p.Bm, p.ldb, p.b_mn, p.N, p.K))) return rc;
  }
  const char* mc_env = getenv("DVAE_TC16_MCAST");
  const bool mcast_on = mc_env && mc_env[0] == '1';
  if (mcast_on && p.presplit && ceil_div(p.K, BK) <= AS_MAX_KB && grid.z == 1 && grid.x >= 2) {
    p.mcast = 1;
    grid.x = (grid.x + 1) / 2 * 2;
    cudaLaunchConfig_t cfg = {};
    cfg.gridDim = grid; cfg.blockDim = dim3(NUM_THREADS); cfg.dynamicSmemBytes = SMEM_BYTES; cfg.stream = st;
    cudaLaunchAttribute attr[1];
    attr[0].id = cudaLaunchAttributeClusterDimension;
    attr[0].val.clusterDim.x = 2; attr[0].val.clusterDim.y = 1; attr[0].val.clusterDim.z = 1;
    cfg.attrs = attr; cfg.numAttrs = 1;
    DVAE_CUDA(cudaLaunchKernelEx(&cfg, tc16_gemm_kernel, ma, mb, p));
    DVAE_LAUNCH_CHECK();
    return DVAE_OK;
  }
  tc16_gemm_kernel<<<grid, NUM_THREADS, SMEM_BYTES, st>>>(ma, mb, p);
  DVAE_LAUNCH_CHECK();
  return DVAE_OK;
}

__global__ void tc16_scale_rows_kernel(float* C, int64_t ldc, int M, int N, float beta) {
  int64_t i = (int64_t)blockIdx.x * blockDim.x + threadIdx.x;
  if (i >= (int64_t)M * N) return;
  float* c = C + (i / N) * ldc + (i % N);
  *c = beta == 0.f ? 0.f : *c * beta;
}

static void apply_hints(Params& p, const GemmHints& h) {
  if (const char* e = getenv("DVAE_TC_DBG")) p.dbg = reinterpret_cast<unsigned long long*>(strtoull(e, nullptr, 0));
  if (const char* e = getenv("DVAE_TC_SKIP_EPILOGUE")) p.dbg_skip_epilogue = atoi(e);
  p.a_amax = h.a_amax_bits; p.b_amax = h.b_amax_bits; p.a_amax_n = h.a_amax_n; p.b_amax_n = h.b_amax_n;
  p.a_scale = h.a_scale; p.b_scale = h.b_scale;
  p.alpha = 1.f; p.alpha_dev = nullptr;
  p.atomic_out = h.atomic_out ? 1 : 0;
}

int linear(const float* A, int64_t lda, int trans_a, const float* B, int64_t ldb, int trans_b, float* C, int64_t ldc, int M,
           int N, int K, const float* bias, const float* bias2, float beta, int act, const GemmHints& hints, cudaStream_t st) {
  Params p = {};
  p.A = A; p.lda = lda; p.Bm = B; p.ldb = ldb;
  p.M = M; p.N = N; p.K = K; p.a_mn = trans_a ? 1 : 0; p.b_mn = trans_b ? 1 : 0; p.tiles_per_cta = 1;
  p.C = C; p.ldc = ldc; p.bias = bias; p.bias2 = bias2; p.beta = beta; p.act = act; p.mode = 0;
  apply_hints(p, hints);
  PlaneHit hit;
  if (hints.b_planes) {
    p.b_presplit = 1; p.b_planes = hints.b_planes; p.b_row0 = hints.b_tile0 * BN; p.b_kb0 = hints.b_kb0; p.b_kbtot = hints.b_kbtot;
  } else if (!hints.b_amax_bits && hints.b_scale == 1.f && find_weight_planes(B, ldb, trans_b, N, K, &hit)) {
    p.b_presplit = 1; p.b_planes = hit.planes; p.b_row0 = hit.tile0 * BN; p.b_kb0 = hit.kb0; p.b_kbtot = hit.kbtot;
  }
  const int tiles = ceil_div(M, BM) * ceil_div(N, BN), nkb = ceil_div(K, BK);
  int splits = 1;
  if (act == 0 && nkb >= 16) {
    const float t_kb = p.b_presplit ? 0.33f + 0.15f * p.a_mn : 0.5f + 0.2f * (p.a_mn + p.b_mn);
    float best = 1e30f;
    for (int s2 = 1; s2 <= 16 && s2 <= nkb / 4; ++s2) {
      const int kbs = ceil_div(nkb, s2), se = ceil_div(nkb, kbs);
      if (se != s2) continue;
      if (hints.max_ctas > 0 && s2 > 1 && tiles * se > hints.max_ctas) break;
      const int waves = ceil_div(tiles * se, 148);
      const float t = waves * (kbs * t_kb + (se > 1 ? 6.f : 4.f)) + (se > 1 ? 2.f : 0.f);
      if (t < best * 0.95f) { best = t; splits = se; }
    }
  }
  if (const char* e = getenv("DVAE_TC16_SPLITS_BIG_MN"))
    if (p.a_mn && p.b_mn && tiles >= 64 && act == 0) splits = atoi(e);
  p.kb_per_split = ceil_div(nkb, splits);
  splits = ceil_div(nkb, p.kb_per_split);
  if (splits > 1 && beta != 1.f && !(beta == 0.f && hints.c_zeroed)) {
    if (beta == 0.f && ldc == N) {
      DVAE_CUDA(cudaMemsetAsync(C, 0, sizeof(float) * (size_t)M * N, st));
    } else {
      tc16_scale_rows_kernel<<<ceil_div((int64_t)M * N, 256), 256, 0, st>>>(C, ldc, M, N, beta);
      DVAE_LAUNCH_CHECK();
    }
  }
  const int conc = hints.concurrency > 1 ? hints.concurrency : 1;
  const int sm_budget = hints.max_ctas > 0 ? hints.max_ctas : 148;
  if (splits == 1 && tiles * conc > sm_budget && ceil_div(N, BN) >= 2) {
    int tpc = ceil_div(tiles * conc, sm_budget);
    if (tpc < 2) tpc = 2;
    if (tpc > ceil_div(N, BN)) tpc = ceil_div(N, BN);
    p.tiles_per_cta = tpc;
  }
  return launch(p, dim3(ceil_div(M, BM), ceil_div(ceil_div(N, BN), p.tiles_per_cta), splits), st);
}

int linear_planes(const void* a_planes, const void* b_planes, float* C, int64_t ldc, int M, int N, int K, const float* bias,
                  float beta, int act, float a_scale, float b_scale, const float* c_row_scale, bool c_zeroed, int max_splits,
                  cudaStream_t st, int b_kb0, int b_kbtot, int max_ctas, int a_kb0, int a_kbtot, const uint32_t* a_amax, int a_amax_n) {
  DVAE_REQUIRE(a_planes && b_planes && C && M > 0 && N > 0 && K > 0, "tc16 linear_planes: bad argument");
  Params p = {};
  p.presplit = 1; p.no_astat = 1; p.a_planes = a_planes; p.b_planes = b_planes; p.a_rows = M; p.b_rows = N;
  p.M = M; p.N = N; p.K = K; p.tiles_per_cta = 1; p.C = C; p.ldc = ldc; p.bias = bias; p.beta = beta; p.act = act; p.mode = 0;
  apply_hints(p, GemmHints());
  p.a_scale = a_scale; p.b_scale = b_scale; p.c_row_scale = c_row_scale;
  p.b_kb0 = b_kb0; p.b_kbtot = b_kbtot;
  p.a_kb0 = a_kb0; p.a_kbtot = a_kbtot;
  if (a_amax) { p.a_amax = a_amax; p.a_amax_n = a_amax_n; }
  const int tiles = ceil_div(M, BM) * ceil_div(N, BN), nkb = ceil_div(K, BK);
  int splits = 1;
  if (act == 0 && nkb >= 8) {
    const float t_kb = 0.27f;
    float best = 1e30f;
    for (int s2 = 1; s2 <= max_splits && s2 <= nkb / 4; ++s2) {
      const int kbs = ceil_div(nkb, s2), se = ceil_div(nkb, kbs);
      if (se != s2) continue;
      if (max_ctas > 0 && s2 > 1 && tiles * se > max_ctas) break;
      const int waves = ceil_div(tiles * se, 148);
      const float t = waves * (kbs * t_kb + (se > 1 ? 5.f : 4.f)) + (se > 1 ? 1.5f : 0.f);
      if (t < best * 0.95f) { best = t; splits = se; }
    }
  }
  p.kb_per_split = ceil_div(nkb, splits);
  splits = ceil_div(nkb, p.kb_per_split);
  if (splits > 1 && beta != 1.f && !(beta == 0.f && c_zeroed)) {
    if (beta == 0.f && ldc == N) {
      DVAE_CUDA(cudaMemsetAsync(C, 0, sizeof(float) * (size_t)M * N, st));
// ... 75 lines not shown
```

disentanglement-vae_b200/csrc/tc_gemm16.cuh:

```cuda
#pragma once
#include "common.cuh"

namespace dvae {
namespace tc16 {

struct Params {
  const float* A; int64_t lda;
  const float* Bm; int64_t ldb;
  int M, N, K;
  int a_mn, b_mn;
  int tiles_per_cta;
  float* C; int64_t ldc;
  const float* bias; const float* bias2;
  float beta; int act;
  int mode;
  int kb_per_split;
  const uint32_t* a_amax; const uint32_t* b_amax; float a_scale, b_scale; int a_amax_n, b_amax_n;
  float alpha; const float* alpha_dev;
  const int64_t* targets; int64_t tgt_stride_b; const int64_t* lengths; int B;
  float* part; int* part_idx;
  const float* lse; const float* grad_scale; int v0;
  const uint64_t* gumbel_seed; uint32_t gumbel_salt;
  float* zero_buf; int64_t zero_n4;
  float* zero_buf2; int64_t zero2_n4;
  int mcast;
  int a_kbtot; int a_kb0;
  int b_presplit; int b_kbtot; int b_kb0;
  int atomic_out;
  int no_astat;
  const float* c_row_scale;
  int presplit; int b_row0;
  const void* a_planes; const void* b_planes; int a_rows, b_rows;
  uint8_t* p_planes_a; uint8_t* p_planes_t; float* p_colsum; float p_scale; int p_kb_a, p_kb_t;
  const int* skip_flag;
  int dbg_skip_epilogue;
  unsigned long long* dbg;
};

bool enabled();
bool shape_ok(const float* A, int64_t lda, int trans_a, const float* B, int64_t ldb, int trans_b, int M, int N, int K);
bool supported(const float* A, int64_t lda, int trans_a, const float* B, int64_t ldb, int trans_b, int M, int N, int K);
int linear(const float* A, int64_t lda, int trans_a, const float* B, int64_t ldb, int trans_b, float* C, int64_t ldc, int M,
           int N, int K, const float* bias, const float* bias2, float beta, int act, const GemmHints& hints, cudaStream_t st);
int64_t plane_floats(int R, int K);
int split_planes(const float* X, int64_t ld, int R, int K, float scale, void* planes, cudaStream_t st, bool force_dual = false);
int linear_planes(const void* a_planes, const void* b_planes, float* C, int64_t ldc, int M, int N, int K, const float* bias,
                  float beta, int act, float a_scale, float b_scale, const float* c_row_scale, bool c_zeroed, int max_splits,
                  cudaStream_t st, int b_kb0 = 0, int b_kbtot = 0, int max_ctas = 0, int a_kb0 = 0, int a_kbtot = 0,
                  const uint32_t* a_amax = nullptr, int a_amax_n = 1);
constexpr int kMaxPlaneEntries = 24;
struct PlaneTable {
  struct Entry { const float* w; int R, C; void* planes; void* planes_t; int64_t ld; const uint32_t* amax; int amax_n; };
  Entry e[kMaxPlaneEntries];
  int n;
};
int weight_planes_launch(const PlaneTable& tab, cudaStream_t st);
struct PlaneHit { const void* planes; int tile0, kb0, kbtot; };
bool find_weight_planes(const float* B, int64_t ldb, int trans_b, int N, int K, PlaneHit* hit);
bool presplit_enabled();
int ce_partials(const float* h, int64_t ldh, int N, int B, int H, int V, const float* w, const float* bias,
                const int64_t* targets, int64_t tgt_stride_b, const int64_t* lengths, int tiles_per_split, int nsplit,
                float* part, int* part_idx, const uint64_t* gumbel_seed, uint32_t gumbel_salt, const void* h_planes,
                const void* w_planes, const int* skip_flag, cudaStream_t st);
int softmax_grad(const float* h, int64_t ldh, int N, int B, int H, int V, int v0, int vc, const float* w, const float* bias,
                 const int64_t* targets, int64_t tgt_stride_b, const int64_t* lengths, const float* lse,
                 const float* grad_scale, float* P, int64_t ldp, const void* h_planes, const void* w_planes, float* zero_buf,
                 int64_t zero_n4, float* zero_buf2, int64_t zero2_n4, cudaStream_t st, void* p_planes_a = nullptr,
                 void* p_planes_t = nullptr, float* p_colsum = nullptr, float p_scale = 1.f);

}
}
```

disentanglement-vae_b200/engine.py:

```python
import os
import random

import torch
import torch.distributed as dist

from . import _lib
from ._lib import ptr, check
from .plan import StepPlan
from .losses import get_cyclic_kl_weight
from .dist import all_reduce_views_


def d_bow(plan):
    return bool(plan.d.bow)


class TrainEngine:
    NSLOT = max(3, int(os.environ.get("DVAE_ENGINE_SLOTS", "4")))

    def __init__(self, model, params, B, T, lr=None, total_steps=None, use_graph=True, max_norm=5.0,
                 process_group=None, seed=None, teacher_forcing_prob=None):
        model._require_cuda()
        self.model, self.params, self.B, self.T = model, params, B, T
        self.lib = _lib.load()
        self.device = model._flat.device
        self.plan = StepPlan(model, B, T, self.device)
        self.d = d = self.plan.d
        self.world = dist.get_world_size(process_group) if (dist.is_available() and dist.is_initialized()) else 1
        self.rank = dist.get_rank(process_group) if self.world > 1 else 0
        self.pg = process_group
        self.max_norm = max_norm
        self.lr = float(params["learn_rate"] if lr is None else lr)
        self.total_steps = total_steps
        self.lambdas = params["lambdas"]
        if total_steps is None and any(v == "cyclic" for v in self.lambdas.values()):
            raise ValueError("a \"cyclic\" lambda needs total_steps (= epochs * len(dataloader), run.py:215-216)")
        self.tf_prob = float(params.get("teacher_forcing_prob", 1.0) if teacher_forcing_prob is None else teacher_forcing_prob)
        self.sampled = self.tf_prob < 1.0
        self.aux = bool(len(model.adversaries) or len(model.mi_estimators))
        if self.aux and self.world > 1:
            raise NotImplementedError("adversarial_loss / mi_loss models train on one GPU through the engine (their private "
                                      "optimizers are not all-reduced)")
        self.n = model._flat_numel
        f32 = dict(device=self.device, dtype=torch.float32)
        self.flat = model._flat[:self.n]
        self.use_graph = use_graph
        self._nvls = None
        if self.world > 1 and use_graph and not self.aux and os.environ.get("DVAE_DP_NVLS", "1") != "0":
            self._setup_nvls()
        if self._nvls is None:
            self.grad = torch.zeros(self.n, **f32)
        self.m = torch.zeros(self.n, **f32)
        self.v = torch.zeros(self.n, **f32)
        self.G = model.grad_views(self.grad)
        named = dict(model.named_parameters())
        for n in model._layout:
            named[n].grad = self.G[n]
        self.n_dsc = max(sum(1 for o in d.dsc_out if o > 0), 1)
        self.hyper = torch.zeros(8, **f32)
        self.kl_w = torch.zeros(max(d.S, 1), **f32)
        self.sumsq = torch.zeros(1, **f32)
        self.red_ws = torch.zeros(1032, **f32)
        T1 = max(T - 1, 1)
        lay, off = {}, 0
        for name, nbytes in (("inputs", B * T * 8), ("lengths", B * 8), ("seed", 8), ("labels", self.n_dsc * B * 4),
                             ("scal", (8 + max(d.S, 1)) * 4), ("coins", T1 * 4)):
            lay[name] = (off, nbytes)
            off = (off + nbytes + 15) // 16 * 16
        self._stage_bytes, self._stage_lay = off, lay
        self.d_stage = torch.zeros(off, device=self.device, dtype=torch.uint8)

        def view(buf, name, dtype, *shape):
            o, n = lay[name]
            return buf[o:o + n].view(dtype).view(*shape)
        self.inputs = view(self.d_stage, "inputs", torch.int64, B, T)
        self.lengths = view(self.d_stage, "lengths", torch.int64, B)
        self.labels = view(self.d_stage, "labels", torch.float32, self.n_dsc, B)
        self.d_scal = view(self.d_stage, "scal", torch.float32, 8 + max(d.S, 1))
        self.coins = view(self.d_stage, "coins", torch.int32, T1)
        self.coins.fill_(1)
        self.plan.seed_dev = view(self.d_stage, "seed", torch.int64, 1)
        self.preds = torch.zeros(B, T, device=self.device, dtype=torch.int64) if self.sampled else None
        ns = self.NSLOT
        self.h_stage = torch.zeros(ns, off, dtype=torch.uint8).pin_memory()
        self.h_outs = torch.zeros(ns, self.plan.out.numel(), dtype=torch.float32).pin_memory()
        self._hv = [{k: view(self.h_stage[i], k, dt, *shp).numpy() for k, dt, shp in
                     (("inputs", torch.int64, (B, T)), ("lengths", torch.int64, (B,)), ("seed", torch.int64, (1,)),
                      ("labels", torch.float32, (self.n_dsc, B)), ("scal", torch.float32, (8 + max(d.S, 1),)),
                      ("coins", torch.int32, (T1,)))} for i in range(ns)]
        for hv in self._hv:
            hv["coins"][:] = 1
            hv["lengths"][:] = 1
        self.h_out = self.h_outs[0]
        self._slot_ev = [None] * ns
        self._slot = -1
        self.step_idx = 0
        self.adam_step = 0
        base = int(params.get("random_seed", 10)) if seed is None else int(seed)
        if seed is None:
            base += 7919 * self.rank
        self._gen = torch.Generator().manual_seed(base)
        self._pyrand = random.Random(base)
        self._eval_gen = torch.Generator().manual_seed(base + 0x5EED)
        self._eval_pyrand = random.Random(base + 0x5EED)
        self._eval = None
        self.use_graph = use_graph and not self.aux
        self._graphs = None
        self._buckets = None
        self._comm = None
        self._flag_mode = False
        self._dp_step = 0
        self._dp_ctr = torch.zeros(1, dtype=torch.int32, device=self.device)
        self._dp_flags = torch.zeros(8, dtype=torch.int32, device=self.device)
        self._side = None
        self.label_names = [n for n, o in zip(d.space_names, d.dsc_out) if o > 0]
        self.last_aux = {}
        self.fixed_eps = None
        self._wplanes, self._plane_token = [], object()
        if os.environ.get("DVAE_WEIGHT_PLANES", "1") != "0" and not d.bow:
            self._alloc_weight_planes()

    def _alloc_weight_planes(self):
        lib, P = self.lib, self.model._P
        names = [n for n in P if (".recurrent.weight_ih_" in n)]
        todo = [(n, True, True) for n in names] + [("decoder.linear.weight", False, True)]
        for n, normal, transposed in todo:
            w = P[n]
            R, C = w.shape
            if R * C < (1 << 14) or (w.data_ptr() & 15):
                continue
            mk = lambda tr: torch.empty(lib.dvae_weight_planes_floats(R, C, tr), device=self.device, dtype=torch.float32)
            self._wplanes.append((w, mk(0) if normal else None, mk(1) if transposed else None))

    def _register_weight_planes(self):
        if not self._wplanes or _lib.planes_owner is self._plane_token:
            return
        check(self.lib.dvae_weight_planes_clear(), "dvae_weight_planes_clear")
        for w, pl, plt in self._wplanes:
            check(self.lib.dvae_weight_planes_register(ptr(w), w.size(0), w.size(1), ptr(pl), ptr(plt)), "dvae_weight_planes_register")
        _lib.planes_owner = self._plane_token

    def _forward(self, fork_ok=True, train=True, sampled=None, preds=None):
        pl, P, m = self.plan, self.model._P, self.model
        sampled = self.sampled if sampled is None else sampled
        preds = self.preds if preds is None else preds
        n_pl = len(self._wplanes)
        n_ih = sum(1 for w, a, b in self._wplanes if a is not None)
        if n_pl:
            check(self.lib.dvae_weight_planes_refresh_ex(0, n_ih, _lib.stream_ptr()), "dvae_weight_planes_refresh")
        self.hyper[:5].copy_(self.d_scal[:5])
        self.kl_w.copy_(self.d_scal[8:8 + self.kl_w.numel()])
        if self.fixed_eps is not None:
            pl.eps.copy_(self.fixed_eps)
        else:
            pl.randn_eps()
        cur = torch.cuda.current_stream()
        hoist = fork_ok and os.environ.get("DVAE_HOIST", "1") != "0" and not d_bow(pl) and not sampled
        refresh_wt = n_pl > n_ih and train
        fork_prep = None
        if hoist:
            if self._side is None:
                self._side = torch.cuda.Stream(device=self.device)

            def fork_prep():
                self._side.wait_stream(cur)
                with torch.cuda.stream(self._side):
                    pl.decode_prepare(P, self.inputs, m.sos_token_idx, train)
                    if refresh_wt:
                        check(self.lib.dvae_weight_planes_refresh_ex(n_ih, n_pl - n_ih, _lib.stream_ptr()), "dvae_weight_planes_refresh")
        if refresh_wt and not hoist:
            check(self.lib.dvae_weight_planes_refresh_ex(n_ih, n_pl - n_ih, _lib.stream_ptr()), "dvae_weight_planes_refresh")
        pl.encode(P, self.inputs, self.lengths, train, after_l0_proj=fork_prep)
        pl.heads(P, pl.ctx, pl.eps, self.labels, self.kl_w)
        if hoist:
            cur.wait_stream(self._side)
        if sampled:
            preds.copy_(self.inputs)
            preds[:, 0].fill_(m.sos_token_idx)
            h_top = pl.decode_sampled(P, preds, self.coins, train)
        else:
            h_top = pl.decode_forced(P, self.inputs, m.sos_token_idx, train)
        pl.vocab_ce(P, h_top, self.inputs, self.lengths)
        return h_top, hoist

    def _fwd_bwd(self, part=None, g_z=None):
        pl, P, G, m = self.plan, self.model._P, self.G, self.model
        st = _lib.stream_ptr()
        cur = torch.cuda.current_stream()
        flags = self._flag_mode and part is None
        if flags:
            check(self.lib.dvae_counter_increment(ptr(self._dp_ctr), st), "dvae_counter_increment")
        if part == 0 or part is None or (part == 1 and not self._three_buckets()):
            h_top, hoist = self._forward()
            if callable(g_z):
                g_z = g_z()
            self._g_z = g_z
            self._g_top = pl.vocab_ce_bwd(P, G, h_top, self.inputs, self.lengths, None)
            self._hoist = hoist
            if part == 0:
                check(self.lib.dvae_join_side_streams(st), "dvae_join_side_streams")
                return
            if flags:
                self._signal(0, True)
        if part in (None, 1):
            g_top, hoist = self._g_top, self._hoist
            check(self.lib.dvae_defer_joins(1), "dvae_defer_joins")
            try:
                pl.decode_bwd(P, G, g_top, emb_grad="decoder.embedding.weight" in m._layout,
                              aux_stream=self._side if hoist else None)
            finally:
                if part == 1:
                    check(self.lib.dvae_join_side_streams(st), "dvae_join_side_streams")
                    if hoist:
                        cur.wait_stream(self._side)
            self._aux_pending = hoist and part is None
            if flags:
                self._signal(1, True, self._side if hoist else None)
        emb_enc = "encoder.embedding.weight" in m._layout
        if part in (None, 2):
            check(self.lib.dvae_defer_joins(1), "dvae_defer_joins")
            try:
                g_ctx = pl.heads_bwd(P, G, pl.ctx, pl.eps, self.labels, self.kl_w, pl.g_hid, g_z=getattr(self, "_g_z", None))
                if getattr(self, "_aux_pending", False):
                    torch.cuda.current_stream().wait_stream(self._side)
                    self._aux_pending = False
                self._g_ctx = g_ctx
                split = part == 2 and self._three_buckets()
                if flags:
                    pl.encode_bwd(P, G, self.inputs, self.lengths, g_ctx, emb_grad=emb_enc, layers=(pl.d.Le - 1, 1))
                    self._signal(2, True)
                    pl.encode_bwd(P, G, self.inputs, self.lengths, g_ctx, emb_grad=emb_enc, layers=(0, 0))
                    if len(self._buckets) == 5:
                        self._signal(3, False)
                        self._signal(4, True)
                    else:
                        self._signal(3, True)
                else:
                    pl.encode_bwd(P, G, self.inputs, self.lengths, g_ctx, emb_grad=emb_enc, layers=(pl.d.Le - 1, 1) if split else None)
            finally:
                check(self.lib.dvae_join_side_streams(st), "dvae_join_side_streams")
            if flags and self._nvls is None:
                check(self.lib.dvae_flag_wait(ptr(self._dp_flags[7:]), ptr(self._dp_ctr), st), "dvae_flag_wait")
        if part == 3:
            check(self.lib.dvae_defer_joins(1), "dvae_defer_joins")
            try:
                pl.encode_bwd(P, G, self.inputs, self.lengths, self._g_ctx, emb_grad=emb_enc, layers=(0, 0))
            finally:
                check(self.lib.dvae_join_side_streams(st), "dvae_join_side_streams")

    def _setup_nvls(self):
        import sys
        import ctypes as C

        def agreed(ok, why, phase):
            flag = torch.tensor([1 if ok else 0], dtype=torch.int32, device=self.device)
            torch.cuda.synchronize()
            dist.all_reduce(flag, op=dist.ReduceOp.MIN, group=self.pg)
            if int(flag.item()) == 1:
                return True
            print(f"[dvae_b200] rank {self.rank}: in-graph gradient exchange unavailable ({phase}: {why or 'another rank failed'}); "
                  "using NCCL all-reduce between stage graphs", file=sys.stderr, flush=True)
            return False

        mode = os.environ.get("DVAE_DP_XCHG", "p2p" if self.world == 2 else "nvls")
        n_pad = (self.n + 3) // 4 * 4
        ok, why, st = True, "", {}
        try:
            import torch.distributed._symmetric_memory as symm
            grp = self.pg if self.pg is not None else dist.group.WORLD
            buf = symm.empty(n_pad, dtype=torch.float32, device=self.device)
            hb = symm.rendezvous(buf, group=grp)
            bar = symm.empty(int(self.lib.dvae_nvls_barrier_words()), dtype=torch.int32, device=self.device)
            bar.zero_()
            hbar = symm.rendezvous(bar, group=grp)
            if mode != "p2p" and not hb.multicast_ptr:
                raise RuntimeError("no multicast address (NVSwitch multicast unavailable)")
# ... 3 lines not shown
                      buf_ptrs=[int(p) for p in hb.buffer_ptrs])
        except Exception as e:
            ok, why = False, repr(e)[:200]
        if not agreed(ok, why, "symmetric memory"):
            return
        try:
            one = torch.ones(1, dtype=torch.int32, device=self.device)
            err = torch.zeros(1, dtype=torch.int32, device=self.device)
            if mode == "p2p":
                peers = (C.c_void_p * self.world)(*st["buf_ptrs"])
                check(self.lib.dvae_p2p_all_reduce(peers, n_pad, st["bar_ptrs"], self.rank, self.world, ptr(one), 1, 0, 0,
                                                   5_000_000_000, ptr(err), _lib.stream_ptr()), "dvae_p2p_all_reduce")
            else:
                check(self.lib.dvae_nvls_all_reduce(st["mc"], n_pad, st["bar_ptrs"], self.rank, self.world, ptr(one), 1, 0, 0,
                                                    5_000_000_000, ptr(err), _lib.stream_ptr()), "dvae_nvls_all_reduce")
            torch.cuda.synchronize()
            want = float(self.world * (self.world + 1) // 2)
            if int(err.item()) != 0 or not bool((st["buf"] == want).all()):
                raise RuntimeError("timeout or wrong sums")
        except Exception as e:
            ok, why = False, repr(e)[:200]
        if not agreed(ok, why, "self-test"):
            return
        st["buf"].zero_()
        if not agreed(True, "", "zero"):
            return
        self.grad = st["buf"][:self.n]
        self._nvls = st

    def _signal(self, k, include_sides, extra=None):
        if self._nvls is not None:
            import ctypes as C
            out = C.c_void_p()
            check(self.lib.dvae_fork_after(1 if include_sides else 0, extra.cuda_stream if extra is not None else None,
                                           _lib.stream_ptr(), C.byref(out)), "dvae_fork_after")
            nv = self._nvls
            ctas = [int(c) for c in os.environ.get("DVAE_XCHG_CTAS", "16,16,32,64,64").split(",")][min(k, 4)]
            if len(self._buckets) == 4 and k == 3:
                ctas = max(ctas, 64)
            for j, v in enumerate(self._buckets[k]):
                off = v.data_ptr() - nv["buf"].data_ptr()
                n = (v.numel() + 3) // 4 * 4
                if nv["mode"] == "p2p":
                    peers = (C.c_void_p * self.world)(*[bp + off for bp in nv["buf_ptrs"]])
                    check(self.lib.dvae_p2p_all_reduce(peers, n, nv["bar_ptrs"], self.rank, self.world, ptr(self._dp_ctr),
                                                       16, 2 * k + j + 1, ctas, 0, None, out.value), "dvae_p2p_all_reduce")
                else:
                    check(self.lib.dvae_nvls_all_reduce(nv["mc"] + off, n, nv["bar_ptrs"], self.rank, self.world, ptr(self._dp_ctr),
                                                        16, 2 * k + j + 1, ctas, 0, None, out.value), "dvae_nvls_all_reduce")
            return
        check(self.lib.dvae_flag_signal(ptr(self._dp_flags[k:]), ptr(self._dp_ctr), 1 if include_sides else 0,
                                        extra.cuda_stream if extra is not None else None, _lib.stream_ptr()), "dvae_flag_signal")

    def _one_graph_dp(self):
        if not (self._three_buckets() and self.use_graph and not self.aux):
            return False
        return self._nvls is not None or os.environ.get("DVAE_DP_FLAGS", "0") == "1"

    @property
    def exchange_mode(self):
        if self.world == 1:
            return "none"
        if self._nvls is not None and self._one_graph_dp():
            return self._nvls["mode"]
        return "nccl+flags" if self._one_graph_dp() else "nccl+stages"

    def _ensure_buckets(self):
        if self._buckets is None:
            from .dist import grad_buckets4, grad_buckets3, grad_buckets5
            if self._three_buckets() and self._nvls is not None and os.environ.get("DVAE_DP_BUCKETS", "4") == "5":
                self._buckets = grad_buckets5(self.model, self.grad)
            elif self._three_buckets():
                self._buckets = grad_buckets4(self.model, self.grad)
            else:
                b3 = grad_buckets3(self.model, self.grad)
                self._buckets = [b3[0], b3[1] + b3[2]]
            self._comm = torch.cuda.Stream(device=self.device)

    def _three_buckets(self):
        return (self.world > 1 and not self.plan.d.bow and self.plan.d.Le >= 2 and os.environ.get("DVAE_DP_BUCKETS", "4") != "2")

    def _optim(self):
        st = _lib.stream_ptr()
        check(self.lib.dvae_grad_sumsq(ptr(self.grad), self.n, ptr(self.sumsq), ptr(self.red_ws), st), "dvae_grad_sumsq")
        check(self.lib.dvae_clip_adam(ptr(self.flat), ptr(self.grad), ptr(self.m), ptr(self.v), self.n, ptr(self.sumsq),
                                      self.max_norm, 1.0 / self.world, ptr(self.hyper), 1, st), "dvae_clip_adam")

    def _latents(self, z):
        from .model import Params
        pl, d, lat, off = self.plan, self.d, {}, 0
        for n, zs in zip(d.space_names, d.space_dims):
            lat[n] = Params(z[:, off:off + zs], pl.mu[:, off:off + zs], pl.logvar[:, off:off + zs])
            off += zs
        return lat

    def _run_aux(self):
        from . import losses
        from .functions import adversary_logits
        m, pl = self.model, self.plan
        box = {}

        def aux_grad():
            z = pl.z.detach().clone().requires_grad_(True)
            lat = self._latents(z)
            Y = {n: self.labels[i].reshape(-1, 1) for i, n in enumerate(self.label_names)}
            A = losses.compute_adversarial_losses(m, adversary_logits(m, lat), Y)
            M = losses.compute_mi_losses(m, lat, beta=0.01)
            aux = A["total_adv_loss"] + M["total_mi"]
            if aux.requires_grad:
                aux.backward(retain_graph=True)
            box.update(A=A, M=M, z=z)
            return z.grad.contiguous() if z.grad is not None else None

        self._fwd_bwd(None, g_z=aux_grad)
        A, M, z = box["A"], box["M"], box["z"]
        for name, dsc_loss in A["idv_adv_dsc_losses"].items():
            m.adversaries[name].optimizer_step(dsc_loss)
        self._optim()
        est_losses = {}
        for pair in M["idv_mi_estimates"]:
            est = m.mi_estimators[pair]
            n1, n2 = pair.split('-')
            lat = self._latents(z.detach())
            mi_loss = est.learning_loss(lat[n1].z, lat[n2].z)
            est.optimizer_step(mi_loss)
            est_losses[pair] = mi_loss
        self.last_aux = {"total_adv_loss": A["total_adv_loss"], "total_mi": M["total_mi"],
                         "idv_adv_losses": A["idv_adv_losses"], "idv_adv_dsc_accs": A["idv_adv_dsc_accs"],
                         "idv_mi_estimates": M["idv_mi_estimates"], "mi_estimator_loss": est_losses}

    def _grad_buckets(self):
        from .dist import grad_buckets
        return grad_buckets(self.model, self.grad)

    def weight_planes(self):
        import contextlib

        @contextlib.contextmanager
        def cm():
            self._register_weight_planes()
            if self._wplanes:
                check(self.lib.dvae_weight_planes_refresh(_lib.stream_ptr()), "dvae_weight_planes_refresh")
                check(self.lib.dvae_weight_planes_enable(1), "dvae_weight_planes_enable")
            try:
                yield self
            finally:
                if self._wplanes:
                    check(self.lib.dvae_weight_planes_enable(0), "dvae_weight_planes_enable")
        return cm()

    def _run(self, body=None):
        self._register_weight_planes()
        if self._wplanes:
            check(self.lib.dvae_weight_planes_enable(1), "dvae_weight_planes_enable")
        try:
            return (body or self._run_inner)()
        finally:
            if self._wplanes:
                check(self.lib.dvae_weight_planes_enable(0), "dvae_weight_planes_enable")

    def _run_inner(self):
        if self.aux:
            return self._run_aux()
        if self.world == 1:
            if not self.use_graph:
                self._fwd_bwd()
# ... 373 lines not shown
```

disentanglement-vae_b200/plan.py:

```python
import torch

from . import _lib
from ._lib import ptr, ptr_array, int_array, check

SALT_ENC_EMB, SALT_DEC_EMB, SALT_ENC_LAYER, SALT_DEC_LAYER, SALT_EPS, SALT_SAMPLE = 1, 3, 16, 32, 64, 4096


class Dims:

    def __init__(self, model):
        enc, dec = model.encoder, model.decoder
        self.V, self.E = enc.embedding.weight.shape
        self.H = enc.hidden_size
        self.Hd = dec.hidden_size
        self.bow = not hasattr(enc, "recurrent")
        self.D = enc.num_directions
        self.Le = 0 if not hasattr(enc, "recurrent") else enc.num_layers
        self.Ld = dec.num_layers
        self.C = self.H * enc.num_layers * self.D
        self.space_names = list(model.context2params.keys())
        self.space_dims = [model.context2params[n].out_features // 2 for n in self.space_names]
        self.S = len(self.space_names)
        self.Z = sum(self.space_dims)
        self.dsc_out = [model.discriminators[n].output_dim if n in model.discriminators else 0
# ... 237 lines not shown
        self._ce_planes_valid = (h_top.data_ptr(), P["decoder.linear.weight"].data_ptr())
        return self.recon

    def vocab_ce_bwd(self, P, G, h_top, targets, lengths, grad_scale_dev):
        self._alloc_bwd()
        lib, d, st = self.lib, self.d, _lib.stream_ptr()
        reuse = getattr(self, "_ce_planes_valid", None) == (h_top.data_ptr(), P["decoder.linear.weight"].data_ptr())
        self._ce_planes_valid = None
        check(lib.dvae_vocab_ce_bwd(ptr(h_top), d.Hd, self.T1, self.B, d.Hd, d.V, ptr(P["decoder.linear.weight"]),
                                    ptr(P["decoder.linear.bias"]), ptr(targets), targets.stride(0), ptr(lengths),
                                    ptr(self.lse), ptr(grad_scale_dev), ptr(self.g_top), d.Hd,
                                    ptr(G["decoder.linear.weight"]), ptr(G["decoder.linear.bias"]),
                                    ptr(self.ce_ws) if reuse else None, ptr(self.ce_bwd_ws), st),
              "dvae_vocab_ce_bwd")
        return self.g_top

    def decode_bwd(self, P, G, g_top, emb_grad=True, aux_stream=None):
        self._alloc_bwd()
        lib, d, st = self.lib, self.d, _lib.stream_ptr()
        B, T1 = self.B, self.T1
        hid = self._dec_hid
        g_in, p = g_top, self._dec_p
        for l in range(d.Ld - 1, -1, -1):
            I = d.E if l == 0 else d.Hd
            x = self.x_dec if l == 0 else (self.d_xin[l] if p > 0.0 else self.d_hs[l - 1])
            g_out = self.g_dx[l % 2]
            w_ih, w_hh, _, _ = self._dec_w(P, l)
            gw_ih, gw_hh, gb_ih, gb_hh = self._dec_w(G, l)
            need_dx = l > 0 or emb_grad
            check(lib.dvae_lstm_seq_bwd_ex(ptr(x), I, T1, B, I, d.Hd, 1, ptr_array(w_ih), ptr_array(w_hh),
                                        hid.data_ptr() + 4 * l * d.Hd, hid.data_ptr() + 4 * (d.Ld + l) * d.Hd,
                                        d.H2L, 0, None, ptr(self.d_hs[l]), d.Hd, ptr(self.d_gates[l]),
                                        ptr(self.d_cs[l]), ptr(g_in), d.Hd, None, None, 0, 0,
                                        ptr(g_out) if need_dx else None, I, ptr_array(gw_ih), ptr_array(gw_hh),
                                        ptr_array(gb_ih), ptr_array(gb_hh), self.g_hid.data_ptr() + 4 * l * d.Hd,
                                        self.g_hid.data_ptr() + 4 * (d.Ld + l) * d.Hd, d.H2L, 0,
                                        ptr(self.state_ws), ptr(self.lstm_bwd_planes), st), "dvae_lstm_seq_bwd(dec)")
            if l > 0 and p > 0.0:
                check(lib.dvae_dropout(ptr(g_out), I, T1 * B, I, p, ptr(self.seed_dev), SALT_DEC_LAYER + l,
                                       ptr(g_out), I, 0, st), "dvae_dropout(bwd)")
            g_in = g_out
        if emb_grad:
            tok = self._dec_tokens
            if aux_stream is not None:
                aux_stream.wait_stream(torch.cuda.current_stream())
                st = aux_stream.cuda_stream
            check(lib.dvae_embedding_bwd(ptr(g_in), d.E, ptr(tok), tok.stride(0), tok.stride(1), T1, B, p,
                                         ptr(self.seed_dev), SALT_DEC_EMB, self._dec_first, 0,
                                         ptr(G["decoder.embedding.weight"]), st), "dvae_embedding_bwd")
        return self.g_hid

    def heads_bwd(self, P, G, ctx, eps, labels, kl_w, g_hid, g_z=None, g_mu=None, g_logvar=None, g_logits=None):
        self._alloc_bwd()
        lib, d, st = self.lib, self.d, _lib.stream_ptr()
        check(lib.dvae_latent_heads_bwd(ptr(ctx), self.B, d.C, d.S, self._space_dims, self._dsc_out,
                                        ptr(P["_c2p.weight"]), ptr(eps), ptr(P.get("_dsc.weight")), ptr(labels),
                                        ptr(kl_w), ptr(P["z2hidden.weight"]), d.H2L, ptr(self.z), ptr(self.mu),
                                        ptr(self.logvar), ptr(self.hid), ptr(self.dsc_logits), ptr(g_hid),
                                        ptr(g_z), ptr(g_mu), ptr(g_logvar), ptr(g_logits), ptr(G["_c2p.weight"]),
                                        ptr(G["_c2p.bias"]), ptr(G.get("_dsc.weight")), ptr(G.get("_dsc.bias")),
                                        ptr(G["z2hidden.weight"]), ptr(G["z2hidden.bias"]), ptr(self.g_ctx),
                                        ptr(self.heads_bwd_ws), st), "dvae_latent_heads_bwd")
        return self.g_ctx

    def encode_bwd(self, P, G, inputs, lengths, g_ctx, emb_grad=True, layers=None):
        self._alloc_bwd()
        lib, d, st = self.lib, self.d, _lib.stream_ptr()
        B, T = self.B, self.T
        p = self._enc_p
        if d.bow:
            if emb_grad:
                check(lib.dvae_bow_encoder_bwd(ptr(g_ctx), d.C, ptr(self.bow_argmax), d.E, ptr(inputs), inputs.stride(0),
                                               inputs.stride(1), T, B, p, ptr(self.seed_dev), SALT_ENC_EMB,
                                               ptr(G["encoder.embedding.weight"]), st), "dvae_bow_encoder_bwd")
            return
        first, last = (d.Le - 1, 0) if layers is None else layers
        g_in = None if first == d.Le - 1 else self._enc_g_in
        for l in range(first, last - 1, -1):
            I = d.E if l == 0 else d.D * d.H
            x = self.x_enc if l == 0 else (self.e_xin[l] if p > 0.0 else self.e_hs[l - 1])
            g_out = self.g_dx[l % 2]
            w_ih, w_hh, _, _ = self._enc_w(P, l, d.D)
            gw_ih, gw_hh, gb_ih, gb_hh = self._enc_w(G, l, d.D)
            need_dx = l > 0 or emb_grad
            off = l * d.D * d.H
            check(lib.dvae_lstm_seq_bwd_ex(ptr(x), I, T, B, I, d.H, d.D, ptr_array(w_ih), ptr_array(w_hh), None, None,
                                        0, 0, ptr(lengths), ptr(self.e_hs[l]), d.D * d.H, ptr(self.e_gates[l]),
                                        ptr(self.e_cs[l]), ptr(g_in), d.D * d.H, g_ctx.data_ptr() + 4 * off, None,
                                        d.C, d.H, ptr(g_out) if need_dx else None, I, ptr_array(gw_ih),
                                        ptr_array(gw_hh), ptr_array(gb_ih), ptr_array(gb_hh), None, None, 0, 0,
                                        ptr(self.state_ws), ptr(self.lstm_bwd_planes), st), "dvae_lstm_seq_bwd(enc)")
            if l > 0 and p > 0.0:
                check(lib.dvae_dropout(ptr(g_out), I, T * B, I, p, ptr(self.seed_dev), SALT_ENC_LAYER + l,
                                       ptr(g_out), I, 0, st), "dvae_dropout(bwd)")
            g_in = g_out
        self._enc_g_in = g_in
        if emb_grad and last == 0:
            check(lib.dvae_embedding_bwd(ptr(g_in), d.E, ptr(inputs), inputs.stride(0), inputs.stride(1), T, B, p,
                                         ptr(self.seed_dev), SALT_ENC_EMB, -1, 0, ptr(G["encoder.embedding.weight"]),
                                         st), "dvae_embedding_bwd")

    def randn_eps(self, salt_offset=0):
        check(self.lib.dvae_randn(ptr(self.eps), self.eps.numel(), ptr(self.seed_dev), SALT_EPS + salt_offset,
                                  _lib.stream_ptr()), "dvae_randn")
        return self.eps

    def recount_lengths(self, tokens, lengths_out, eos, pad=0, min_len=1):
        check(self.lib.dvae_recount_lengths(ptr(tokens), tokens.stride(0), tokens.stride(1), tokens.size(0), tokens.size(1),
                                            eos, pad, min_len, ptr(lengths_out), _lib.stream_ptr()), "dvae_recount_lengths")
        return lengths_out
```

include/dvae_b200.h:

```cpp
#ifndef DVAE_B200_H_
#define DVAE_B200_H_

#include <stdint.h>

#ifdef __cplusplus
extern "C" {
#endif

#define DVAE_OK 0
#define DVAE_EINVAL (-1)
#define DVAE_ECUDA (-2)
#define DVAE_EWORKSPACE (-3)

#define DVAE_MAX_SPACES 8

const char* dvae_last_error_string(void);
int dvae_version(void);
int64_t dvae_launch_count(void);

int dvae_linear(const float* A, int64_t lda, int trans_a, const float* B, int64_t ldb, int trans_b,
                float* C, int64_t ldc, int M, int N, int K, const float* bias, const float* bias2,
                float beta, int act, void* stream);

int dvae_tc_linear(const float* A, int64_t lda, int trans_a, const float* B, int64_t ldb, int trans_b,
// ... 23 lines not shown

int dvae_defer_joins(int on);
int dvae_join_side_streams(void* stream);

int dvae_counter_increment(uint32_t* counter, void* stream);
int dvae_fork_after(int include_sides, void* extra_stream, void* stream, void** forked_stream_out);
int dvae_flag_signal(uint32_t* flag, const uint32_t* counter, int include_sides, void* extra_stream, void* stream);
int dvae_flag_wait(const uint32_t* flag, const uint32_t* counter, void* stream);
int dvae_flag_signal_value(uint32_t* flag, uint32_t value, void* stream);
int dvae_flag_wait_value(const uint32_t* flag, uint32_t value, void* stream);

int64_t dvae_nvls_barrier_words(void);
int dvae_p2p_all_reduce(float* const* peer_ptrs_host, int64_t n, uint32_t* const* barrier_ptrs_host, int rank, int world,
                        const uint32_t* counter_dev, uint32_t epoch_mul, uint32_t epoch_add, int ctas,
                        uint64_t soft_timeout_ns, uint32_t* err_dev, void* stream);
int dvae_nvls_all_reduce(float* mc_ptr, int64_t n, uint32_t* const* barrier_ptrs_host, int rank, int world,
                         const uint32_t* counter_dev, uint32_t epoch_mul, uint32_t epoch_add, int ctas,
                         uint64_t soft_timeout_ns, uint32_t* err_dev, void* stream);

int dvae_colsum(const float* X, int64_t ldx, int M, int N, float* out, float beta, void* stream);

int dvae_randn(float* out, int64_t n, const uint64_t* seed_dev, uint32_t salt, void* stream);
int dvae_embedding_fwd(const float* emb, int E, const int64_t* tokens, int64_t tok_stride_b,
                       int64_t tok_stride_t, int T, int B, float p, const uint64_t* seed_dev,
                       uint32_t salt, int64_t first_token, int t0, float* x, void* stream);
int dvae_embedding_bwd(const float* d_x, int E, const int64_t* tokens, int64_t tok_stride_b,
                       int64_t tok_stride_t, int T, int B, float p, const uint64_t* seed_dev,
                       uint32_t salt, int64_t first_token, int t0, float* d_emb, void* stream);
int dvae_bow_encoder_fwd(const float* emb, int E, const int64_t* tokens, int64_t tok_stride_b, int64_t tok_stride_t,
                         int T, int B, float p, const uint64_t* seed_dev, uint32_t salt, float* ctx, int64_t ldctx,
                         int32_t* argmax, void* stream);
int dvae_bow_encoder_bwd(const float* d_ctx, int64_t ldd, const int32_t* argmax, int E, const int64_t* tokens,
                         int64_t tok_stride_b, int64_t tok_stride_t, int T, int B, float p, const uint64_t* seed_dev,
                         uint32_t salt, float* d_emb, void* stream);
int dvae_dropout(const float* x, int64_t ldx, int64_t rows, int width, float p,
                 const uint64_t* seed_dev, uint32_t salt, float* y, int64_t ldy, int64_t row0,
                 void* stream);

int64_t dvae_lstm_state_ws_floats(int B, int H, int D);
int dvae_lstm_seq_fwd(const float* x, int64_t ldx, int T, int B, int I, int H, int D,
                      const float* const* w_ih_host, const float* const* w_hh_host,
                      const float* const* b_ih_host, const float* const* b_hh_host,
                      const float* h0, const float* c0, int64_t ld0, int64_t dir0,
                      const int64_t* lengths, float* hs, int64_t ldhs, float* hn, float* cn,
                      int64_t ldn, int64_t dirn, float* gates, float* cs, float* state_ws,
                      void* stream);

int dvae_lstm_step(const float* x, int64_t ldx, int t, int T, int B, int I, int H, const float* w_ih,
                   const float* w_hh, const float* b_ih, const float* b_hh, const float* h0,
                   const float* c0, int64_t ld0, float* hs, float* gates, float* cs, float* state_ws,
                   void* stream);

int dvae_lstm_input_proj(const float* x, int64_t ldx, int T, int B, int I, int H, int D,
                         const float* const* w_ih, const float* const* b_ih, const float* const* b_hh,
                         float* gates, void* stream);
int dvae_lstm_seq_fwd_ex(const float* x, int64_t ldx, int T, int B, int I, int H, int D,
                         const float* const* w_ih, const float* const* w_hh, const float* const* b_ih,
                         const float* const* b_hh, const float* h0, const float* c0, int64_t ld0,
                         int64_t dir0, const int64_t* lengths, float* hs, int64_t ldhs, float* hn,
                         float* cn, int64_t ldn, int64_t dirn, float* gates, float* cs, float* state_ws,
                         int flags, void* stream);

int dvae_lstm_seq_bwd(const float* x, int64_t ldx, int T, int B, int I, int H, int D,
                      const float* const* w_ih_host, const float* const* w_hh_host,
                      const float* h0, const float* c0, int64_t ld0, int64_t dir0,
                      const int64_t* lengths, const float* hs, int64_t ldhs, float* gates,
                      const float* cs, const float* d_hs, int64_t lddhs, const float* d_hn,
                      const float* d_cn, int64_t ldn, int64_t dirn, float* d_x, int64_t lddx,
                      float* const* d_w_ih_host, float* const* d_w_hh_host,
                      float* const* d_b_ih_host, float* const* d_b_hh_host, float* d_h0,
                      float* d_c0, int64_t ldd0, int64_t dird0, float* state_ws, void* stream);

int64_t dvae_lstm_bwd_planes_ws_floats(int T, int B, int I, int H, int D);
int dvae_lstm_seq_bwd_ex(const float* x, int64_t ldx, int T, int B, int I, int H, int D,
                         const float* const* w_ih_host, const float* const* w_hh_host,
                         const float* h0, const float* c0, int64_t ld0, int64_t dir0,
                         const int64_t* lengths, const float* hs, int64_t ldhs, float* gates,
                         const float* cs, const float* d_hs, int64_t lddhs, const float* d_hn,
                         const float* d_cn, int64_t ldn, int64_t dirn, float* d_x, int64_t lddx,
                         float* const* d_w_ih_host, float* const* d_w_hh_host,
                         float* const* d_b_ih_host, float* const* d_b_hh_host, float* d_h0,
                         float* d_c0, int64_t ldd0, int64_t dird0, float* state_ws, float* planes_ws,
                         void* stream);

#define DVAE_HEADS_NSCALARS (3 + 3 * DVAE_MAX_SPACES)
int64_t dvae_heads_ws_floats(int B, int S);
int dvae_latent_heads_fwd(const float* ctx, int B, int C, int S, const int* space_dims_host,
                          const int* dsc_out_host, const float* w_c2p, const float* b_c2p,
                          const float* eps, const float* w_dsc, const float* b_dsc,
                          const float* labels, const float* kl_w_dev, const float* w_z2h,
                          const float* b_z2h, int H2L, float* z, float* mu, float* logvar,
                          float* hid, float* dsc_logits, float* scalars, float* ws, void* stream);

int64_t dvae_heads_bwd_ws_floats(int B, int Z, int H2L);
int dvae_latent_heads_bwd(const float* ctx, int B, int C, int S, const int* space_dims_host,
                          const int* dsc_out_host, const float* w_c2p, const float* eps,
                          const float* w_dsc, const float* labels, const float* kl_w_dev,
                          const float* w_z2h, int H2L, const float* z, const float* mu,
                          const float* logvar, const float* hid, const float* dsc_logits,
                          const float* d_hid, const float* d_z_extra, const float* d_mu_extra,
                          const float* d_logvar_extra, const float* d_logits_extra, float* d_w_c2p,
                          float* d_b_c2p, float* d_w_dsc, float* d_b_dsc, float* d_w_z2h,
                          float* d_b_z2h, float* d_ctx, float* ws, void* stream);

int dvae_dsc_loss(const float* dsc_logits, const float* labels, int B, int S,
                  const int* space_dims_host, const int* dsc_out_host, float* out,
                  const float* d_out, float* d_logits, void* stream);

int64_t dvae_vocab_ce_ws_floats(int N, int V, int H);
int dvae_vocab_ce_fwd(const float* h, int64_t ldh, int T1, int B, int H, int V, const float* w,
                      const float* bias, const int64_t* targets, int64_t tgt_stride_b,
                      const int64_t* lengths, int sos, float* lse, float* nll, int32_t* argmax,
                      float* loss, float* ws, void* stream);

int dvae_vocab_split_w(const float* w, int N, int V, int H, float* ws, void* stream);
int dvae_vocab_ce_fwd_ex(const float* h, int64_t ldh, int T1, int B, int H, int V, const float* w,
                         const float* bias, const int64_t* targets, int64_t tgt_stride_b,
                         const int64_t* lengths, int sos, float* lse, float* nll, int32_t* argmax,
                         float* loss, float* ws, int flags, void* stream);

int dvae_vocab_ce_partials(const float* h, int64_t ldh, int T1, int B, int H, int V, const float* w,
                           const float* bias, const int64_t* targets, int64_t tgt_stride_b,
                           const int64_t* lengths, int sos, float* ws, void* stream);

int dvae_vocab_sample_step(const float* h, int64_t ldh, int B, int H, int V, const float* w,
                           const float* bias, const uint64_t* seed_dev, uint32_t salt, int64_t* tokens_out,
                           int64_t tok_stride, float* ws, void* stream);

int dvae_vocab_sample_step_ex(const float* h, int64_t ldh, int B, int H, int V, const float* w,
                              const float* bias, const uint64_t* seed_dev, uint32_t salt, int64_t* tokens_out,
                              int64_t tok_stride, const int32_t* forced_flag_dev, float* ws, void* stream);

int64_t dvae_vocab_w_planes_floats(int V, int H);
int dvae_vocab_w_planes(const float* w, int V, int H, float* planes, void* stream);
int dvae_vocab_sample_step_planes(const float* h, int64_t ldh, int B, int H, int V, const float* w,
                                  const float* bias, const float* w_planes, const uint64_t* seed_dev, uint32_t salt,
                                  int64_t* tokens_out, int64_t tok_stride, const int32_t* forced_flag_dev, float* ws,
                                  void* stream);

int dvae_recount_lengths(const int64_t* tokens, int64_t tok_stride_b, int64_t tok_stride_t, int B, int T,
                         int64_t eos, int64_t pad, int64_t min_len, int64_t* lengths_out, void* stream);

#define DVAE_BLEU_MAX_T 256
int dvae_bleu_counts(const int64_t* ref, int64_t ref_stride, int T_ref, const int64_t* cand, int64_t cand_stride,
                     int T_cand, int B, int64_t eos, int64_t* counts, void* stream);
int dvae_bleu_score(const int64_t* counts, float* score_out, void* stream);

int64_t dvae_vocab_ce_bwd_ws_floats(int N, int V, int H);
int dvae_vocab_ce_bwd(const float* h, int64_t ldh, int T1, int B, int H, int V, const float* w,
                      const float* bias, const int64_t* targets, int64_t tgt_stride_b,
                      const int64_t* lengths, const float* lse, const float* grad_scale_dev,
                      float* d_h, int64_t lddh, float* d_w, float* d_bias, const float* fwd_ws, float* ws,
                      void* stream);

int dvae_grad_sumsq(const float* g, int64_t n, float* sumsq, float* ws, void* stream);
int dvae_clip_adam(float* p, float* g, float* m, float* v, int64_t n, const float* sumsq,
                   float max_norm, float grad_scale, const float* hyper_dev, int zero_grad,
                   void* stream);

#ifdef __cplusplus
}
#endif
#endif
```

Baseline: 1.156 million.

## Skip untouched embedding rows in optimizer and fuse embedding grad into LSTM backward

Marks the embedding rows referenced by the batch's tokens in a bitmask. The grad-norm and clip-Adam kernels then skip rows that were not touched. The untouched rows get their zero-gradient Adam update (moment decay) in a separate kernel on a side stream, which overlaps with the forward/backward pass. The encoder's first-layer LSTM backward now scatters the input gradient straight into the embedding gradient through a fused GEMM epilogue, replacing the separate embedding_bwd pass. This adds a side stream, bitmask bookkeeping and more complex kernels, and the exact-Adam semantics must hold for the untouched rows.

Result: slower. 1.127 million (median of 6 runs) (-2.6%).

```diff
diff --git a/disentanglement-vae_b200/_lib.py b/disentanglement-vae_b200/_lib.py
--- a/disentanglement-vae_b200/_lib.py
+++ b/disentanglement-vae_b200/_lib.py
@@ -62,6 +62,8 @@
     "dvae_lstm_bwd_planes_ws_floats": (_l, [_i, _i, _i, _i, _i]),
     "dvae_lstm_seq_bwd_ex": (_i, [_p, _l, _i, _i, _i, _i, _i, _pp, _pp, _p, _p, _l, _l, _p, _p, _l, _p, _p, _p, _l,
                                   _p, _p, _l, _l, _p, _l, _pp, _pp, _pp, _pp, _p, _p, _l, _l, _p, _p, _p]),
+    "dvae_lstm_seq_bwd_emb": (_i, [_p, _l, _i, _i, _i, _i, _i, _pp, _pp, _p, _p, _l, _p, _p, _p, _l, _p, _p, _l, _l,
+                                   _p, _pp, _pp, _pp, _pp, _p, _p, _p, _l, _l, _f, _p, _u32, _p, _p]),
     "dvae_counter_increment": (_i, [_p, _p]),
     "dvae_fork_after": (_i, [_i, _p, _p, C.POINTER(C.c_void_p)]),
     "dvae_nvls_barrier_words": (_l, []),
@@ -92,6 +94,10 @@
     "dvae_relu": (_i, [_p, _l, _p]),
     "dvae_grad_sumsq": (_i, [_p, _l, _p, _p, _p]),
     "dvae_clip_adam": (_i, [_p, _p, _p, _p, _l, _p, _f, _f, _p, _i, _p]),
+    "dvae_mark_rows": (_i, [_p, _l, _l, _i, _i, _l, _p, _p]),
+    "dvae_adam_untouched": (_i, [_p, _p, _p, _i, _p, _p, _p, _pp, _f, _p, _p]),
+    "dvae_grad_sumsq_skip": (_i, [_p, _l, _p, _p, _i, _p, _p, _p, _pp, _p]),
+    "dvae_clip_adam_skip": (_i, [_p, _p, _p, _p, _l, _p, _f, _f, _p, _i, _p, _p, _p, _pp, _p]),
 }
 
 _lib = None
diff --git a/disentanglement-vae_b200/csrc/common.cuh b/disentanglement-vae_b200/csrc/common.cuh
--- a/disentanglement-vae_b200/csrc/common.cuh
+++ b/disentanglement-vae_b200/csrc/common.cuh
@@ -61,6 +61,15 @@
 
 bool force_simt_gemm();
 
+struct EmbScatter {
+  const int64_t* tokens = nullptr;
+  int64_t sb = 0, st = 0;
+  int B = 0;
+  float p = 0.f;
+  const uint64_t* seed_dev = nullptr;
+  uint32_t salt = 0;
+};
+
 struct GemmHints {
   const uint32_t* a_amax_bits = nullptr;
   const uint32_t* b_amax_bits = nullptr;
@@ -73,10 +82,13 @@
   bool atomic_out = false;
   bool c_zeroed = false;
   int concurrency = 1;
+  EmbScatter scatter;
 };
 int linear_impl_ex(const float* A, int64_t lda, int trans_a, const float* B, int64_t ldb, int trans_b, float* C,
                    int64_t ldc, int M, int N, int K, const float* bias, const float* bias2, float beta, int act,
                    const GemmHints& hints, cudaStream_t st);
+bool linear_scatter_supported(const float* A, int64_t lda, int trans_a, const float* B, int64_t ldb, int trans_b, int M,
+                              int N, int K, const GemmHints& hints);
 
 namespace tc {
 bool tc_linear_supported(const float* A, int64_t lda, const float* B, int64_t ldb, int M, int N, int K);
diff --git a/disentanglement-vae_b200/csrc/embed_optim.cu b/disentanglement-vae_b200/csrc/embed_optim.cu
--- a/disentanglement-vae_b200/csrc/embed_optim.cu
+++ b/disentanglement-vae_b200/csrc/embed_optim.cu
@@ -136,15 +136,37 @@
 }
 
 constexpr int kRedBlocks = 1024;
+constexpr int kMaxSkipSegs = 2;
+
+struct RowSkip {
+  int64_t off[kMaxSkipSegs], rows[kMaxSkipSegs];
+  int E[kMaxSkipSegs];
+  const uint32_t* bits[kMaxSkipSegs];
+  int n;
+};
+
+__device__ __forceinline__ bool untouched4(RowSkip s, int64_t e) {
+#pragma unroll
+  for (int k = 0; k < kMaxSkipSegs; ++k) {
+    if (k >= s.n) break;
+    const int64_t r = e - s.off[k];
+    if (r >= 0 && r < s.rows[k] * s.E[k]) {
+      const int64_t row = r / s.E[k];
+      return !((__ldg(s.bits[k] + (row >> 5)) >> (row & 31)) & 1u);
+    }
+  }
+  return false;
+}
 
 __global__ void __launch_bounds__(256) sumsq_kernel(const float* __restrict__ g, int64_t n, float* __restrict__ sumsq,
-                                                    float* __restrict__ ws) {
+                                                    float* __restrict__ ws, RowSkip skip) {
   __shared__ float red[8];
   __shared__ int is_last;
   float acc = 0.f;
   const int64_t n4 = n / 4;
   const float4* g4 = reinterpret_cast<const float4*>(g);
   for (int64_t i = (int64_t)blockIdx.x * blockDim.x + threadIdx.x; i < n4; i += (int64_t)gridDim.x * blockDim.x) {
+    if (skip.n && untouched4(skip, 4 * i)) continue;
     float4 v = g4[i];
     acc = fmaf(v.x, v.x, acc); acc = fmaf(v.y, v.y, acc); acc = fmaf(v.z, v.z, acc); acc = fmaf(v.w, v.w, acc);
   }
@@ -180,27 +202,39 @@
   }
 }
 
-__global__ void __launch_bounds__(256) clip_adam_kernel(float* __restrict__ p, float* __restrict__ g,
-                                                        float* __restrict__ m, float* __restrict__ v, int64_t n,
-                                                        const float* __restrict__ sumsq, float max_norm,
-                                                        float grad_scale, const float* __restrict__ hyper,
-                                                        int zero_grad) {
-  const float lr = hyper[0], b1 = hyper[1], b2 = hyper[2], eps = hyper[3], step = hyper[4];
-  float coef = grad_scale;
-  if (sumsq) {
-    const float norm = sqrtf(sumsq[0]) * fabsf(grad_scale);
-    coef *= fminf(1.f, max_norm / (norm + 1e-6f));
-  }
-  const float bc1 = 1.f - powf(b1, step), bc2 = 1.f - powf(b2, step);
-  const float step_size = lr / bc1, inv_bc2_sqrt = 1.f / sqrtf(bc2);
-  auto update = [&](float& pi, float& gi_io, float& mi_io, float& vi_io) {
+struct AdamStep {
+  float coef, b1, b2, eps, step_size, inv_bc2_sqrt;
+  __device__ __forceinline__ AdamStep(const float* hyper, const float* sumsq, float max_norm, float grad_scale) {
+    const float lr = hyper[0], step = hyper[4];
+    b1 = hyper[1]; b2 = hyper[2]; eps = hyper[3];
+    coef = grad_scale;
+    if (sumsq) {
+      const float norm = sqrtf(sumsq[0]) * fabsf(grad_scale);
+      coef *= fminf(1.f, max_norm / (norm + 1e-6f));
+    }
+    const float bc1 = 1.f - powf(b1, step), bc2 = 1.f - powf(b2, step);
+    step_size = lr / bc1; inv_bc2_sqrt = 1.f / sqrtf(bc2);
+  }
+  __device__ __forceinline__ void update(float& pi, float& gi_io, float& mi_io, float& vi_io, int zero_grad) const {
     const float gi = gi_io * coef;
     const float mi = fmaf(b1, mi_io, (1.f - b1) * gi);
     const float vi = fmaf(b2, vi_io, (1.f - b2) * gi * gi);
     mi_io = mi; vi_io = vi;
     pi -= step_size * mi / (sqrtf(vi) * inv_bc2_sqrt + eps);
     gi_io = zero_grad ? 0.f : gi;
-  };
+  }
+  __device__ __forceinline__ void update4(float4& p, float4& g, float4& m, float4& v, int zero_grad) const {
+    update(p.x, g.x, m.x, v.x, zero_grad); update(p.y, g.y, m.y, v.y, zero_grad);
+    update(p.z, g.z, m.z, v.z, zero_grad); update(p.w, g.w, m.w, v.w, zero_grad);
+  }
+};
+
+__global__ void __launch_bounds__(256, 3) clip_adam_kernel(float* __restrict__ p, float* __restrict__ g,
+                                                        float* __restrict__ m, float* __restrict__ v, int64_t n,
+                                                        const float* __restrict__ sumsq, float max_norm,
+                                                        float grad_scale, const float* __restrict__ hyper,
+                                                        int zero_grad, RowSkip skip) {
+  const AdamStep a(hyper, sumsq, max_norm, grad_scale);
   const bool vec = (((uintptr_t)p | (uintptr_t)g | (uintptr_t)m | (uintptr_t)v) & 15) == 0;
   const int64_t n4 = vec ? n / 4 : 0;
   float4* p4 = reinterpret_cast<float4*>(p); float4* g4 = reinterpret_cast<float4*>(g);
@@ -208,18 +242,52 @@
   const int64_t stride = (int64_t)gridDim.x * blockDim.x;
   for (int64_t i = (int64_t)blockIdx.x * blockDim.x + threadIdx.x; i < n4; i += 2 * stride) {
     const int64_t j = i + stride;
-    const bool two = j < n4;
-    float4 pa = p4[i], ga = g4[i], ma = m4[i], va = v4[i];
-    float4 pb, gb, mb, vb;
-    if (two) { pb = p4[j]; gb = g4[j]; mb = m4[j]; vb = v4[j]; }
-    update(pa.x, ga.x, ma.x, va.x); update(pa.y, ga.y, ma.y, va.y); update(pa.z, ga.z, ma.z, va.z); update(pa.w, ga.w, ma.w, va.w);
-    p4[i] = pa; g4[i] = ga; m4[i] = ma; v4[i] = va;
-    if (two) {
-      update(pb.x, gb.x, mb.x, vb.x); update(pb.y, gb.y, mb.y, vb.y); update(pb.z, gb.z, mb.z, vb.z); update(pb.w, gb.w, mb.w, vb.w);
+    const bool da = !(skip.n && untouched4(skip, 4 * i));
+    const bool db = j < n4 && !(skip.n && untouched4(skip, 4 * j));
+    float4 pa, ga, ma, va, pb, gb, mb, vb;
+    if (da) { pa = p4[i]; ga = g4[i]; ma = m4[i]; va = v4[i]; }
+    if (db) { pb = p4[j]; gb = g4[j]; mb = m4[j]; vb = v4[j]; }
+    if (da) {
+      a.update4(pa, ga, ma, va, zero_grad);
+      p4[i] = pa; g4[i] = ga; m4[i] = ma; v4[i] = va;
+    }
+    if (db) {
+      a.update4(pb, gb, mb, vb, zero_grad);
       p4[j] = pb; g4[j] = gb; m4[j] = mb; v4[j] = vb;
     }
   }
-  for (int64_t i = n4 * 4 + (int64_t)blockIdx.x * blockDim.x + threadIdx.x; i < n; i += stride) update(p[i], g[i], m[i], v[i]);
+  for (int64_t i = n4 * 4 + (int64_t)blockIdx.x * blockDim.x + threadIdx.x; i < n; i += stride) a.update(p[i], g[i], m[i], v[i], zero_grad);
+}
+
+__global__ void __launch_bounds__(256) adam_untouched_kernel(float* __restrict__ p, float* __restrict__ m, float* __restrict__ v,
+                                                             RowSkip skip, float grad_scale, const float* __restrict__ hyper,
+                                                             float zero) {
+  const AdamStep a(hyper, nullptr, 0.f, grad_scale);
+  const bool k1 = blockIdx.y == 1;
+  const int64_t rows = k1 ? skip.rows[1] : skip.rows[0], off = k1 ? skip.off[1] : skip.off[0];
+  const int e4 = (k1 ? skip.E[1] : skip.E[0]) / 4;
+  const uint32_t* bits = k1 ? skip.bits[1] : skip.bits[0];
+  const int64_t n4 = rows * e4;
+  float4* p4 = reinterpret_cast<float4*>(p + off);
+  float4* m4 = reinterpret_cast<float4*>(m + off);
+  float4* v4 = reinterpret_cast<float4*>(v + off);
+  for (int64_t i = (int64_t)blockIdx.x * blockDim.x + threadIdx.x; i < n4; i += (int64_t)gridDim.x * blockDim.x) {
+    const int64_t row = i / e4;
+    if ((__ldg(bits + (row >> 5)) >> (row & 31)) & 1u) continue;
+    float4 pa = p4[i], ma = m4[i], va = v4[i], ga = make_float4(zero, zero, zero, zero);
+    a.update4(pa, ga, ma, va, 0);
+    p4[i] = pa; m4[i] = ma; v4[i] = va;
+  }
+}
+
+__global__ void mark_rows_kernel(const int64_t* __restrict__ tokens, int64_t sb, int64_t st_, int T, int B, int64_t extra,
+                                 uint32_t* __restrict__ bits) {
+  const int64_t i = (int64_t)blockIdx.x * blockDim.x + threadIdx.x;
+  if (i == 0 && extra >= 0) atomicOr(bits + (extra >> 5), 1u << (extra & 31));
+  if (i >= (int64_t)T * B) return;
+  const int t = (int)(i / B), b = (int)(i % B);
+  const int64_t tok = tokens[b * sb + t * st_];
+  atomicOr(bits + (tok >> 5), 1u << (tok & 31));
 }
 
 }
@@ -279,22 +347,88 @@
   return DVAE_OK;
 }
 
-extern "C" int dvae_grad_sumsq(const float* g, int64_t n, float* sumsq, float* ws, void* stream) {
+static int make_skip(int nseg, const int64_t* seg_off, const int64_t* seg_rows, const int* seg_E, const uint32_t* const* bits,
+                     int64_t n, RowSkip* s) {
+  s->n = 0;
+  DVAE_REQUIRE(nseg >= 0 && nseg <= kMaxSkipSegs, "row skip: at most %d segments", kMaxSkipSegs);
+  for (int k = 0; k < nseg; ++k) {
+    DVAE_REQUIRE(bits[k] && seg_E[k] > 0 && seg_E[k] % 4 == 0 && seg_off[k] >= 0 && seg_off[k] % 4 == 0 && seg_rows[k] > 0 &&
+                 seg_off[k] + seg_rows[k] * seg_E[k] <= n / 4 * 4, "row skip: bad segment %d", k);
+    s->off[k] = seg_off[k]; s->rows[k] = seg_rows[k]; s->E[k] = seg_E[k]; s->bits[k] = bits[k];
+  }
+  s->n = nseg;
+  return DVAE_OK;
+}
+
+static int sumsq_launch(const float* g, int64_t n, float* sumsq, float* ws, const RowSkip& skip, void* stream) {
   DVAE_REQUIRE(g && sumsq && ws && n > 0, "dvae_grad_sumsq: bad argument");
   DVAE_REQUIRE((reinterpret_cast<uintptr_t>(g) & 15) == 0, "dvae_grad_sumsq: gradient buffer must be 16-byte aligned");
   int blocks = ew_grid(n / 4 + 1);
   if (blocks > kRedBlocks) blocks = kRedBlocks;
-  sumsq_kernel<<<blocks, 256, 0, (cudaStream_t)stream>>>(g, n, sumsq, ws);
-  DVAE_LAUNCH_CHECK();
-  return DVAE_OK;
+  sumsq_kernel<<<blocks, 256, 0, (cudaStream_t)stream>>>(g, n, sumsq, ws, skip);
+  DVAE_LAUNCH_CHECK();
+  return DVAE_OK;
+}
+
+static int clip_adam_launch(float* p, float* g, float* m, float* v, int64_t n, const float* sumsq, float max_norm,
+                            float grad_scale, const float* hyper_dev, int zero_grad, const RowSkip& skip, void* stream) {
+  DVAE_REQUIRE(p && g && m && v && hyper_dev && n > 0, "dvae_clip_adam: bad argument");
+  DVAE_REQUIRE(skip.n == 0 || ((((uintptr_t)p | (uintptr_t)g | (uintptr_t)m | (uintptr_t)v) & 15) == 0 && zero_grad),
+               "dvae_clip_adam: skipped rows need 16-byte aligned buffers and zero_grad");
+  clip_adam_kernel<<<ew_grid((n + 7) / 8), 256, 0, (cudaStream_t)stream>>>(p, g, m, v, n, sumsq, max_norm, grad_scale, hyper_dev, zero_grad, skip);
+  DVAE_LAUNCH_CHECK();
+  return DVAE_OK;
+}
+
+extern "C" int dvae_grad_sumsq(const float* g, int64_t n, float* sumsq, float* ws, void* stream) {
+  RowSkip none = {};
+  return sumsq_launch(g, n, sumsq, ws, none, stream);
 }
 
 extern "C" int dvae_clip_adam(float* p, float* g, float* m, float* v, int64_t n, const float* sumsq, float max_norm,
                               float grad_scale, const float* hyper_dev, int zero_grad, void* stream) {
-  DVAE_REQUIRE(p && g && m && v && hyper_dev && n > 0, "dvae_clip_adam: bad argument");
-  clip_adam_kernel<<<ew_grid((n + 7) / 8), 256, 0, (cudaStream_t)stream>>>(p, g, m, v, n, sumsq, max_norm, grad_scale, hyper_dev, zero_grad);
-  DVAE_LAUNCH_CHECK();
-  return DVAE_OK;
+  RowSkip none = {};
+  return clip_adam_launch(p, g, m, v, n, sumsq, max_norm, grad_scale, hyper_dev, zero_grad, none, stream);
+}
+
+extern "C" int dvae_mark_rows(const int64_t* tokens, int64_t sb, int64_t st_, int T, int B, int64_t extra, uint32_t* bits,
+                              void* stream) {
+  DVAE_REQUIRE(tokens && bits && T > 0 && B > 0, "dvae_mark_rows: bad argument");
+  mark_rows_kernel<<<ceil_div((int64_t)T * B, 256), 256, 0, (cudaStream_t)stream>>>(tokens, sb, st_, T, B, extra, bits);
+  DVAE_LAUNCH_CHECK();
+  return DVAE_OK;
+}
+
+extern "C" int dvae_adam_untouched(float* p, float* m, float* v, int nseg, const int64_t* seg_off, const int64_t* seg_rows,
+                                   const int* seg_E, const uint32_t* const* bits, float grad_scale, const float* hyper_dev,
+                                   void* stream) {
+  DVAE_REQUIRE(p && m && v && hyper_dev && nseg > 0, "dvae_adam_untouched: bad argument");
+  DVAE_REQUIRE((((uintptr_t)p | (uintptr_t)m | (uintptr_t)v) & 15) == 0, "dvae_adam_untouched: buffers must be 16-byte aligned");
+  RowSkip s;
+  int rc = make_skip(nseg, seg_off, seg_rows, seg_E, bits, INT64_MAX, &s);
+  if (rc) return rc;
+  int64_t most = 0;
+  for (int k = 0; k < nseg; ++k) most = seg_rows[k] * seg_E[k] / 4 > most ? seg_rows[k] * seg_E[k] / 4 : most;
+  adam_untouched_kernel<<<dim3(ew_grid(most), nseg), 256, 0, (cudaStream_t)stream>>>(p, m, v, s, grad_scale, hyper_dev, 0.f);
+  DVAE_LAUNCH_CHECK();
+  return DVAE_OK;
+}
+
+extern "C" int dvae_grad_sumsq_skip(const float* g, int64_t n, float* sumsq, float* ws, int nseg, const int64_t* seg_off,
+                                    const int64_t* seg_rows, const int* seg_E, const uint32_t* const* bits, void* stream) {
+  RowSkip s;
+  int rc = make_skip(nseg, seg_off, seg_rows, seg_E, bits, n, &s);
+  if (rc) return rc;
+  return sumsq_launch(g, n, sumsq, ws, s, stream);
+}
+
+extern "C" int dvae_clip_adam_skip(float* p, float* g, float* m, float* v, int64_t n, const float* sumsq, float max_norm,
+                                   float grad_scale, const float* hyper_dev, int nseg, const int64_t* seg_off,
+                                   const int64_t* seg_rows, const int* seg_E, const uint32_t* const* bits, void* stream) {
+  RowSkip s;
+  int rc = make_skip(nseg, seg_off, seg_rows, seg_E, bits, n, &s);
+  if (rc) return rc;
+  return clip_adam_launch(p, g, m, v, n, sumsq, max_norm, grad_scale, hyper_dev, 1, s, stream);
 }
 
 namespace dvae {
diff --git a/disentanglement-vae_b200/csrc/linear.cu b/disentanglement-vae_b200/csrc/linear.cu
--- a/disentanglement-vae_b200/csrc/linear.cu
+++ b/disentanglement-vae_b200/csrc/linear.cu
@@ -82,19 +82,39 @@
   return linear_impl_ex(A, lda, trans_a, B, ldb, trans_b, C, ldc, M, N, K, bias, bias2, beta, act, GemmHints(), st);
 }
 
+static bool tc_shape(int M, int N, int K) {
+  static const double tc_min_mnk = [] {
+    const char* e = getenv("DVAE_TC_MIN_LOG2_MNK");
+    return (double)(1ll << (e ? atoi(e) : 24));
+  }();
+  return !force_simt_gemm() && M >= 64 && N >= 64 && K >= 32 && (double)M * N * K >= tc_min_mnk;
+}
+
+static bool takes_tc16(const float* A, int64_t lda, int trans_a, const float* B, int64_t ldb, int trans_b, int M, int N,
+                       int K, const GemmHints& hints) {
+  const bool unscaled_wide = (hints.a_wide && !hints.a_amax_bits) || (hints.b_wide && !hints.b_amax_bits);
+  return tc_shape(M, N, K) && !unscaled_wide && tc16::supported(A, lda, trans_a, B, ldb, trans_b, M, N, K);
+}
+
+bool linear_scatter_supported(const float* A, int64_t lda, int trans_a, const float* B, int64_t ldb, int trans_b, int M,
+                              int N, int K, const GemmHints& hints) {
+  return N % 32 == 0 && takes_tc16(A, lda, trans_a, B, ldb, trans_b, M, N, K, hints);
+}
+
 int linear_impl_ex(const float* A, int64_t lda, int trans_a, const float* B, int64_t ldb, int trans_b, float* C,
                    int64_t ldc, int M, int N, int K, const float* bias, const float* bias2, float beta, int act,
                    const GemmHints& hints, cudaStream_t st) {
   DVAE_REQUIRE(A && B && C, "dvae_linear: null pointer");
   DVAE_REQUIRE(M > 0 && N > 0 && K > 0, "dvae_linear: non-positive size M=%d N=%d K=%d", M, N, K);
   DVAE_REQUIRE(act == 0 || act == 1, "dvae_linear: unknown activation %d", act);
-  static const double tc_min_mnk = [] {
-    const char* e = getenv("DVAE_TC_MIN_LOG2_MNK");
-    return (double)(1ll << (e ? atoi(e) : 24));
-  }();
-  if (!force_simt_gemm() && M >= 64 && N >= 64 && K >= 32 && (double)M * N * K >= tc_min_mnk) {
-    const bool unscaled_wide = (hints.a_wide && !hints.a_amax_bits) || (hints.b_wide && !hints.b_amax_bits);
-    if (!unscaled_wide && tc16::supported(A, lda, trans_a, B, ldb, trans_b, M, N, K))
+  if (hints.scatter.tokens) {
+    DVAE_REQUIRE(linear_scatter_supported(A, lda, trans_a, B, ldb, trans_b, M, N, K, hints) && !bias && !bias2 && act == 0 &&
+                 beta == 1.f && hints.scatter.B > 0 && M % hints.scatter.B == 0,
+                 "dvae_linear: embedding scatter needs the fp16-split kernel (M=%d N=%d K=%d)", M, N, K);
+    return tc16::linear(A, lda, trans_a, B, ldb, trans_b, C, ldc, M, N, K, nullptr, nullptr, 1.f, 0, hints, st);
+  }
+  if (tc_shape(M, N, K)) {
+    if (takes_tc16(A, lda, trans_a, B, ldb, trans_b, M, N, K, hints))
       return tc16::linear(A, lda, trans_a, B, ldb, trans_b, C, ldc, M, N, K, bias, bias2, beta, act, hints, st);
     if (tc::tc_linear_supported(A, lda, B, ldb, M, N, K))
       return tc::tc_linear_impl(A, lda, trans_a, B, ldb, trans_b, C, ldc, M, N, K, bias, bias2, beta, act, 3, st);
diff --git a/disentanglement-vae_b200/csrc/lstm.cu b/disentanglement-vae_b200/csrc/lstm.cu
--- a/disentanglement-vae_b200/csrc/lstm.cu
+++ b/disentanglement-vae_b200/csrc/lstm.cu
@@ -317,8 +317,10 @@
                       const float* d_hs, int64_t lddhs, const float* d_hn, const float* d_cn, int64_t ldn,
                       int64_t dirn, float* d_x, int64_t lddx, float* const* d_w_ih, float* const* d_w_hh,
                       float* const* d_b_ih, float* const* d_b_hh, float* d_h0, float* d_c0, int64_t ldd0,
-                      int64_t dird0, float* ws, float* planes_ws, cudaStream_t st) {
+                      int64_t dird0, float* ws, float* planes_ws, const EmbScatter* emb, float* d_emb, cudaStream_t st) {
   DVAE_REQUIRE(x && hs && gates && cs && ws && w_ih && w_hh, "dvae_lstm_seq_bwd: null pointer");
+  DVAE_REQUIRE(!emb || (emb->tokens && d_emb && d_x && lddx == I), "dvae_lstm_seq_bwd: the embedding scatter needs tokens, "
+               "d_emb and a dense d_x workspace");
   DVAE_REQUIRE(T > 0 && B > 0 && I > 0 && H > 0 && (D == 1 || D == 2), "dvae_lstm_seq_bwd: bad shape");
   DVAE_REQUIRE(!(lengths && h0), "dvae_lstm_seq_bwd: length-masked layers start from the zero state");
   const int64_t slab = (int64_t)T * B * 4 * H, sf = (int64_t)D * B * H;
@@ -326,6 +328,7 @@
   uint32_t* amax = nullptr;
   int amax_n = 1;
   bool dx_zeroed = false;
+  bool scatter = false;
   {
     const void* ptrs[] = {w_hh[0], w_hh[D - 1], c0, gates, cs, d_hs, d_hn, d_cn, d_h0, d_c0};
     const int64_t lds[] = {ld0, dir0, lddhs, ldn, dirn, ldd0, dird0};
@@ -342,7 +345,14 @@
         amax = reinterpret_cast<uint32_t*>(ws + state_floats(B, H, D) + 4LL * D * H * H) + amax_slot_entries(B, D) * (slot++ & 7);
         a.amax_out = amax;
         amax_n = tc_lstm_bwd_ctas(B, D);
-        if (d_x && lddx == I && (((uintptr_t)d_x) & 15) == 0 && ((int64_t)T * B * I) % 4 == 0 && d_x != d_hs) {
+        if (emb && !force_simt_gemm()) {
+          GemmHints gs;
+          gs.a_wide = true; gs.a_amax_bits = amax; gs.a_amax_n = amax_n;
+          scatter = true;
+          for (int d = 0; d < D; ++d)
+            scatter = scatter && linear_scatter_supported(gates + d * slab, 4 * H, 0, w_ih[d], I, 1, T * B, I, 4 * H, gs);
+        }
+        if (!scatter && d_x && lddx == I && (((uintptr_t)d_x) & 15) == 0 && ((int64_t)T * B * I) % 4 == 0 && d_x != d_hs) {
           a.zero_buf = d_x; a.zero_n4 = (int64_t)T * B * I / 4;
           dx_zeroed = true;
         }
@@ -401,12 +411,15 @@
     gh_bg.max_ctas = (defer_joins_enabled() && tc_lstm_supported(H)) ? cap : 0;
   }
   Fork fork(st);
-  const bool dx_pair = d_x && D == 2 && dx_zeroed && !force_simt_gemm() && tc_lstm_supported(H) &&
+  const bool dx_pair = d_x && D == 2 && (dx_zeroed || scatter) && !force_simt_gemm() && tc_lstm_supported(H) &&
                        !(getenv("DVAE_DX_PAIR") && getenv("DVAE_DX_PAIR")[0] == '0');
+  float* dx_out = scatter ? d_emb : d_x;
+  const int64_t lddx_out = scatter ? I : lddx;
+  if (scatter) gh.scatter = *emb;
   if (dx_pair) {
     GemmHints ghx = gh;
     ghx.c_zeroed = true; ghx.atomic_out = true; ghx.concurrency = 2;
-    int rc = linear_impl_ex(gates + slab, 4 * H, 0, w_ih[1], I, 1, d_x, lddx, T * B, I, 4 * H, nullptr, nullptr, 1.f, 0, ghx, fork.side(2));
+    int rc = linear_impl_ex(gates + slab, 4 * H, 0, w_ih[1], I, 1, dx_out, lddx_out, T * B, I, 4 * H, nullptr, nullptr, 1.f, 0, ghx, fork.side(2));
     if (rc) return rc;
     if ((rc = fork.mark(2))) return rc;
   }
@@ -439,7 +452,8 @@
       GemmHints ghx = gh;
       ghx.c_zeroed = dx_zeroed;
       if (dx_pair) { ghx.atomic_out = true; ghx.concurrency = 2; }
-      rc = linear_impl_ex(dG, 4 * H, 0, w_ih[d], I, 1, d_x, lddx, T * B, I, 4 * H, nullptr, nullptr, (d == 0 && !dx_pair) ? 0.f : 1.f, 0, ghx, st);
+      rc = linear_impl_ex(dG, 4 * H, 0, w_ih[d], I, 1, dx_out, lddx_out, T * B, I, 4 * H, nullptr, nullptr,
+                          (d == 0 && !dx_pair && !scatter) ? 0.f : 1.f, 0, ghx, st);
       if (rc) return rc;
       if (dx_pair && (rc = fork.wait_mark())) return rc;
     }
@@ -482,6 +496,10 @@
       rc = colsum_impl(dG, 4 * H, T * B, 4 * H, d_b_hh[d], 0.f, s2);
       if (rc) return rc;
     }
+  }
+  if (emb && !scatter) {
+    int rc = dvae_embedding_bwd(d_x, I, emb->tokens, emb->sb, emb->st, T, B, emb->p, emb->seed_dev, emb->salt, -1, 0, d_emb, st);
+    if (rc) return rc;
   }
   {
     int rc = fork.join_or_defer();
@@ -605,7 +623,7 @@
                                  int64_t ldd0, int64_t dird0, float* state_ws, void* stream) {
   return dvae::lstm_seq_bwd_impl(x, ldx, T, B, I, H, D, w_ih, w_hh, h0, c0, ld0, dir0, lengths, hs, ldhs, gates, cs,
                                  d_hs, lddhs, d_hn, d_cn, ldn, dirn, d_x, lddx, d_w_ih, d_w_hh, d_b_ih, d_b_hh,
-                                 d_h0, d_c0, ldd0, dird0, state_ws, nullptr, (cudaStream_t)stream);
+                                 d_h0, d_c0, ldd0, dird0, state_ws, nullptr, nullptr, nullptr, (cudaStream_t)stream);
 }
 
 extern "C" int64_t dvae_lstm_bwd_planes_ws_floats(int T, int B, int I, int H, int D) {
@@ -623,5 +641,21 @@
                                     int64_t ldd0, int64_t dird0, float* state_ws, float* planes_ws, void* stream) {
   return dvae::lstm_seq_bwd_impl(x, ldx, T, B, I, H, D, w_ih, w_hh, h0, c0, ld0, dir0, lengths, hs, ldhs, gates, cs,
                                  d_hs, lddhs, d_hn, d_cn, ldn, dirn, d_x, lddx, d_w_ih, d_w_hh, d_b_ih, d_b_hh,
-                                 d_h0, d_c0, ldd0, dird0, state_ws, planes_ws, (cudaStream_t)stream);
-}
+                                 d_h0, d_c0, ldd0, dird0, state_ws, planes_ws, nullptr, nullptr, (cudaStream_t)stream);
+}
+
+extern "C" int dvae_lstm_seq_bwd_emb(const float* x, int64_t ldx, int T, int B, int I, int H, int D,
+                                     const float* const* w_ih, const float* const* w_hh, const int64_t* lengths,
+                                     const float* hs, int64_t ldhs, float* gates, const float* cs, const float* d_hs,
+                                     int64_t lddhs, const float* d_hn, const float* d_cn, int64_t ldn, int64_t dirn,
+                                     float* d_x, float* const* d_w_ih, float* const* d_w_hh, float* const* d_b_ih,
+                                     float* const* d_b_hh, float* state_ws, float* planes_ws, const int64_t* tokens,
+                                     int64_t tok_stride_b, int64_t tok_stride_t, float p, const uint64_t* seed_dev,
+                                     uint32_t salt, float* d_emb, void* stream) {
+  dvae::EmbScatter e;
+  e.tokens = tokens; e.sb = tok_stride_b; e.st = tok_stride_t; e.B = B; e.p = p; e.seed_dev = seed_dev; e.salt = salt;
+  DVAE_REQUIRE(!d_emb || (p >= 0.f && p < 1.f), "dvae_lstm_seq_bwd_emb: bad dropout probability");
+  return dvae::lstm_seq_bwd_impl(x, ldx, T, B, I, H, D, w_ih, w_hh, nullptr, nullptr, 0, 0, lengths, hs, ldhs, gates, cs,
+                                 d_hs, lddhs, d_hn, d_cn, ldn, dirn, d_emb ? d_x : nullptr, I, d_w_ih, d_w_hh, d_b_ih, d_b_hh,
+                                 nullptr, nullptr, 0, 0, state_ws, planes_ws, d_emb ? &e : nullptr, d_emb, (cudaStream_t)stream);
+}
diff --git a/disentanglement-vae_b200/csrc/tc_gemm16.cu b/disentanglement-vae_b200/csrc/tc_gemm16.cu
--- a/disentanglement-vae_b200/csrc/tc_gemm16.cu
+++ b/disentanglement-vae_b200/csrc/tc_gemm16.cu
@@ -187,6 +187,41 @@
   return DVAE_OK;
 }
 
+__device__ __noinline__ void scatter_chunk(EmbScatter s, float* C, int64_t ldc, int N, int r0, int nr, int col0, uint32_t sc,
+                                           int lane) {
+  const bool drop = s.p > 0.f && s.seed_dev;
+  const uint64_t seed = drop ? *s.seed_dev : 0;
+  const float inv_keep = drop ? 1.f / (1.f - s.p) : 1.f;
+  const int e4n = N / 4, col = col0 + lane;
+  int64_t my_tok = 0;
+  if (lane < nr) {
+    const int row = r0 + lane;
+    my_tok = s.tokens[(row % s.B) * s.sb + (row / s.B) * s.st];
+  }
+  int64_t run_tok = -1;
+  float run = 0.f;
+  for (int r4 = 0; r4 < nr; r4 += 4) {
+    uint32_t keep = 0xfu;
+    if (drop) {
+      float k[4];
+      dropout_scale4(seed, s.salt, (uint64_t)((int64_t)(r0 + r4 + (lane & 3)) * e4n + (col0 >> 2) + (lane >> 2)), s.p, inv_keep, k);
+      keep = (k[0] != 0.f ? 1u : 0u) | (k[1] != 0.f ? 2u : 0u) | (k[2] != 0.f ? 4u : 0u) | (k[3] != 0.f ? 8u : 0u);
+    }
+    for (int j = 0; j < 4 && r4 + j < nr; ++j) {
+      const uint32_t m = __shfl_sync(0xffffffffu, keep, (lane & ~3) | j);
+      const int rr = r4 + j;
+      const int64_t tok = __shfl_sync(0xffffffffu, my_tok, rr);
+      if (tok != run_tok) {
+        if (run != 0.f) atomicAdd(C + run_tok * ldc + col, run);
+        run = 0.f;
+        run_tok = tok;
+      }
+      if ((m >> (lane & 3)) & 1u) run += lds32(sc + (uint32_t)(rr * 32 + (lane ^ rr)) * 4) * inv_keep;
+    }
+  }
+  if (run != 0.f) atomicAdd(C + run_tok * ldc + col, run);
+}
+
 __global__ void __launch_bounds__(NUM_THREADS, 1)
 tc16_gemm_kernel(const __grid_constant__ CUtensorMap tmA, const __grid_constant__ CUtensorMap tmB, Params p) {
   extern __shared__ __align__(1024) uint8_t smem[];
@@ -634,6 +669,8 @@
               } else {
                 for (int rr = 0; rr < nr; ++rr) cp[rr * ldc] = chunk_at(rr) + badd;
               }
+            } else if (p.scatter.tokens) {
+              scatter_chunk(p.scatter, p.C, ldc, p.N, r0, nr, col0, sc, lane);
             } else if (split) {
               for (int rr = 0; rr < nr; ++rr) atomicAdd(cp + rr * ldc, chunk_at(rr) + badd);
             } else {
@@ -882,6 +919,7 @@
   p.a_scale = h.a_scale; p.b_scale = h.b_scale;
   p.alpha = 1.f; p.alpha_dev = nullptr;
   p.atomic_out = h.atomic_out ? 1 : 0;
+  p.scatter = h.scatter;
 }
 
 int linear(const float* A, int64_t lda, int trans_a, const float* B, int64_t ldb, int trans_b, float* C, int64_t ldc, int M,
diff --git a/disentanglement-vae_b200/csrc/tc_gemm16.cuh b/disentanglement-vae_b200/csrc/tc_gemm16.cuh
--- a/disentanglement-vae_b200/csrc/tc_gemm16.cuh
+++ b/disentanglement-vae_b200/csrc/tc_gemm16.cuh
@@ -27,6 +27,7 @@
   int a_kbtot; int a_kb0;
   int b_presplit; int b_kbtot; int b_kb0;
   int atomic_out;
+  EmbScatter scatter;
   int no_astat;
   const float* c_row_scale;
   int presplit; int b_row0;
diff --git a/disentanglement-vae_b200/engine.py b/disentanglement-vae_b200/engine.py
--- a/disentanglement-vae_b200/engine.py
+++ b/disentanglement-vae_b200/engine.py
@@ -1,3 +1,4 @@
+import ctypes as C
 import os
 import random
 
@@ -113,6 +114,8 @@
         self._dp_ctr = torch.zeros(1, dtype=torch.int32, device=self.device)
         self._dp_flags = torch.zeros(8, dtype=torch.int32, device=self.device)
         self._side = None
+        self._rows = self._row_segments() if self.world == 1 and not self.aux else None
+        self._rows_pending = False
         self.label_names = [n for n, o in zip(d.space_names, d.dsc_out) if o > 0]
         self.last_aux = {}
         self.fixed_eps = None
@@ -139,6 +142,50 @@
         for w, pl, plt in self._wplanes:
             check(self.lib.dvae_weight_planes_register(ptr(w), w.size(0), w.size(1), ptr(pl), ptr(plt)), "dvae_weight_planes_register")
         _lib.planes_owner = self._plane_token
+
+    def _row_segments(self):
+        lay, segs = self.model._layout, []
+        for name in ("encoder.embedding.weight", "decoder.embedding.weight"):
+            if name not in lay:
+                continue
+            V, E = self.model._P[name].shape
+            off = lay[name]
+            if off % 4 == 0 and E % 4 == 0 and off + V * E <= self.n // 4 * 4:
+                segs.append((name, off, V, E))
+        if not segs:
+            return None
+        k = len(segs)
+        bits = torch.zeros(k, max((V + 31) // 32 for _, _, V, _ in segs), dtype=torch.int32, device=self.device)
+        return {"decoder": [name.startswith("decoder.") for name, _, _, _ in segs], "bits": bits, "n": k,
+                "off": (C.c_int64 * k)(*[s[1] for s in segs]), "rows": (C.c_int64 * k)(*[s[2] for s in segs]),
+                "E": (C.c_int * k)(*[s[3] for s in segs]), "bitp": _lib.ptr_array([bits[i] for i in range(k)]),
+                "stream": None}
+
+    def _seg_args(self):
+        r = self._rows
+        return (r["n"], C.cast(r["off"], C.c_void_p), C.cast(r["rows"], C.c_void_p), C.cast(r["E"], C.c_void_p), r["bitp"])
+
+    def _untouched_adam(self):
+        r, lib = self._rows, self.lib
+        cur = torch.cuda.current_stream()
+        if r["stream"] is None:
+            r["stream"] = torch.cuda.Stream(device=self.device)
+        r["stream"].wait_stream(cur)
+        with torch.cuda.stream(r["stream"]):
+            st = _lib.stream_ptr()
+            r["bits"].zero_()
+            x = self.inputs
+            for k, dec in enumerate(r["decoder"]):
+                b = ptr(r["bits"][k])
+                check(lib.dvae_mark_rows(ptr(x), x.stride(0), x.stride(1), x.size(1), x.size(0),
+                                         self.model.sos_token_idx if dec else -1, b, st), "dvae_mark_rows")
+                if dec and self.sampled:
+                    p = self.preds
+                    check(lib.dvae_mark_rows(ptr(p), p.stride(0), p.stride(1), p.size(1), p.size(0), -1, b, st),
+                          "dvae_mark_rows")
+            check(lib.dvae_adam_untouched(ptr(self.flat), ptr(self.m), ptr(self.v), *self._seg_args(), 1.0 / self.world,
+                                          ptr(self.hyper), st), "dvae_adam_untouched")
+        self._rows_pending = True
 
     def _forward(self, fork_ok=True, train=True, sampled=None, preds=None):
         pl, P, m = self.plan, self.model._P, self.model
@@ -192,6 +239,8 @@
             check(self.lib.dvae_counter_increment(ptr(self._dp_ctr), st), "dvae_counter_increment")
         if part == 0 or part is None or (part == 1 and not self._three_buckets()):
             h_top, hoist = self._forward()
+            if part is None and self._rows is not None:
+                self._untouched_adam()
             if callable(g_z):
                 g_z = g_z()
             self._g_z = g_z
@@ -361,6 +410,15 @@
 
     def _optim(self):
         st = _lib.stream_ptr()
+        if self._rows_pending:
+            self._rows_pending = False
+            torch.cuda.current_stream().wait_stream(self._rows["stream"])
+            check(self.lib.dvae_grad_sumsq_skip(ptr(self.grad), self.n, ptr(self.sumsq), ptr(self.red_ws), *self._seg_args(), st),
+                  "dvae_grad_sumsq_skip")
+            check(self.lib.dvae_clip_adam_skip(ptr(self.flat), ptr(self.grad), ptr(self.m), ptr(self.v), self.n, ptr(self.sumsq),
+                                               self.max_norm, 1.0 / self.world, ptr(self.hyper), *self._seg_args(), st),
+                  "dvae_clip_adam_skip")
+            return
         check(self.lib.dvae_grad_sumsq(ptr(self.grad), self.n, ptr(self.sumsq), ptr(self.red_ws), st), "dvae_grad_sumsq")
         check(self.lib.dvae_clip_adam(ptr(self.flat), ptr(self.grad), ptr(self.m), ptr(self.v), self.n, ptr(self.sumsq),
                                       self.max_norm, 1.0 / self.world, ptr(self.hyper), 1, st), "dvae_clip_adam")
diff --git a/disentanglement-vae_b200/plan.py b/disentanglement-vae_b200/plan.py
--- a/disentanglement-vae_b200/plan.py
+++ b/disentanglement-vae_b200/plan.py
@@ -343,12 +343,22 @@
             g_out = self.g_dx[l % 2]
             w_ih, w_hh, _, _ = self._enc_w(P, l, d.D)
             gw_ih, gw_hh, gb_ih, gb_hh = self._enc_w(G, l, d.D)
-            need_dx = l > 0 or emb_grad
             off = l * d.D * d.H
+            if l == 0:
+                check(lib.dvae_lstm_seq_bwd_emb(ptr(x), I, T, B, I, d.H, d.D, ptr_array(w_ih), ptr_array(w_hh),
+                                                ptr(lengths), ptr(self.e_hs[l]), d.D * d.H, ptr(self.e_gates[l]),
+                                                ptr(self.e_cs[l]), ptr(g_in), d.D * d.H, g_ctx.data_ptr() + 4 * off, None,
+                                                d.C, d.H, ptr(g_out), ptr_array(gw_ih), ptr_array(gw_hh),
+                                                ptr_array(gb_ih), ptr_array(gb_hh), ptr(self.state_ws),
+                                                ptr(self.lstm_bwd_planes), ptr(inputs), inputs.stride(0), inputs.stride(1),
+                                                p, ptr(self.seed_dev), SALT_ENC_EMB,
+                                                ptr(G["encoder.embedding.weight"]) if emb_grad else None, st),
+                      "dvae_lstm_seq_bwd_emb(enc)")
+                continue
             check(lib.dvae_lstm_seq_bwd_ex(ptr(x), I, T, B, I, d.H, d.D, ptr_array(w_ih), ptr_array(w_hh), None, None,
                                         0, 0, ptr(lengths), ptr(self.e_hs[l]), d.D * d.H, ptr(self.e_gates[l]),
                                         ptr(self.e_cs[l]), ptr(g_in), d.D * d.H, g_ctx.data_ptr() + 4 * off, None,
-                                        d.C, d.H, ptr(g_out) if need_dx else None, I, ptr_array(gw_ih),
+                                        d.C, d.H, ptr(g_out), I, ptr_array(gw_ih),
                                         ptr_array(gw_hh), ptr_array(gb_ih), ptr_array(gb_hh), None, None, 0, 0,
                                         ptr(self.state_ws), ptr(self.lstm_bwd_planes), st), "dvae_lstm_seq_bwd(enc)")
             if l > 0 and p > 0.0:
@@ -356,10 +366,6 @@
                                        ptr(g_out), I, 0, st), "dvae_dropout(bwd)")
             g_in = g_out
         self._enc_g_in = g_in
-        if emb_grad and last == 0:
-            check(lib.dvae_embedding_bwd(ptr(g_in), d.E, ptr(inputs), inputs.stride(0), inputs.stride(1), T, B, p,
-                                         ptr(self.seed_dev), SALT_ENC_EMB, -1, 0, ptr(G["encoder.embedding.weight"]),
-                                         st), "dvae_embedding_bwd")
 
     def randn_eps(self, salt_offset=0):
         check(self.lib.dvae_randn(ptr(self.eps), self.eps.numel(), ptr(self.seed_dev), SALT_EPS + salt_offset,
diff --git a/include/dvae_b200.h b/include/dvae_b200.h
--- a/include/dvae_b200.h
+++ b/include/dvae_b200.h
@@ -129,6 +129,16 @@
                          float* const* d_b_ih_host, float* const* d_b_hh_host, float* d_h0,
                          float* d_c0, int64_t ldd0, int64_t dird0, float* state_ws, float* planes_ws,
                          void* stream);
+int dvae_lstm_seq_bwd_emb(const float* x, int64_t ldx, int T, int B, int I, int H, int D,
+                          const float* const* w_ih_host, const float* const* w_hh_host,
+                          const int64_t* lengths, const float* hs, int64_t ldhs, float* gates,
+                          const float* cs, const float* d_hs, int64_t lddhs, const float* d_hn,
+                          const float* d_cn, int64_t ldn, int64_t dirn, float* d_x,
+                          float* const* d_w_ih_host, float* const* d_w_hh_host,
+                          float* const* d_b_ih_host, float* const* d_b_hh_host, float* state_ws,
+                          float* planes_ws, const int64_t* tokens, int64_t tok_stride_b,
+                          int64_t tok_stride_t, float p, const uint64_t* seed_dev, uint32_t salt,
+                          float* d_emb, void* stream);
 
 #define DVAE_HEADS_NSCALARS (3 + 3 * DVAE_MAX_SPACES)
 int64_t dvae_heads_ws_floats(int B, int S);
@@ -204,6 +214,16 @@
 int dvae_clip_adam(float* p, float* g, float* m, float* v, int64_t n, const float* sumsq,
                    float max_norm, float grad_scale, const float* hyper_dev, int zero_grad,
                    void* stream);
+int dvae_mark_rows(const int64_t* tokens, int64_t tok_stride_b, int64_t tok_stride_t, int T, int B, int64_t extra,
+                   uint32_t* bits, void* stream);
+int dvae_adam_untouched(float* p, float* m, float* v, int nseg, const int64_t* seg_off, const int64_t* seg_rows,
+                        const int* seg_E, const uint32_t* const* bits, float grad_scale, const float* hyper_dev,
+                        void* stream);
+int dvae_grad_sumsq_skip(const float* g, int64_t n, float* sumsq, float* ws, int nseg, const int64_t* seg_off,
+                         const int64_t* seg_rows, const int* seg_E, const uint32_t* const* bits, void* stream);
+int dvae_clip_adam_skip(float* p, float* g, float* m, float* v, int64_t n, const float* sumsq, float max_norm,
+                        float grad_scale, const float* hyper_dev, int nseg, const int64_t* seg_off,
+                        const int64_t* seg_rows, const int* seg_E, const uint32_t* const* bits, void* stream);
 
 #ifdef __cplusplus
 }
```
